# thetisproject/thetis

Hardware: AMD Instinct MI355X
Metric: DG element-updates/sec, 2D SWE DG-P1 SSPRK33 (higher is better)
Workload: dtype f64

## Files before the change

include/swe2d.h:

```cpp
#ifndef SWE2D_H
#define SWE2D_H

#include <stddef.h>
#include <stdint.h>

#ifdef __cplusplus
extern "C" {
#endif

#define SWE2D_ABI_VERSION 12
#define SWE2D_MAX_MARKERS 16

typedef enum {
    SWE2D_OK = 0,
    SWE2D_ERR_INVALID_ARGUMENT = -1,
    SWE2D_ERR_NO_DEVICE = -2,
    SWE2D_ERR_HIP = -3,
    SWE2D_ERR_UNSUPPORTED = -4,
    SWE2D_ERR_NOT_FINITE = -5
} swe2d_status;

#define SWE2D_BC_ELEV 1
#define SWE2D_BC_UV   2
#define SWE2D_BC_UN   4
#define SWE2D_BC_FLUX 8
#define SWE2D_BC_ELEV_FIELD 16
#define SWE2D_BC_UV_FIELD   32
#define SWE2D_BC_UN_FIELD   64
#define SWE2D_BC_FLUX_FIELD 128

typedef enum {
    SWE2D_FIELD_CORIOLIS = 0,
    SWE2D_FIELD_ATMOSPHERIC_PRESSURE = 1,
    SWE2D_FIELD_MOMENTUM_SOURCE = 2,
    SWE2D_FIELD_VOLUME_SOURCE = 3,
    SWE2D_FIELD_WIND_STRESS = 4,
    SWE2D_FIELD_LINEAR_DRAG = 5,
    SWE2D_FIELD_QUADRATIC_DRAG = 6,
    SWE2D_FIELD_MANNING_DRAG = 7,
    SWE2D_FIELD_NIKURADSE = 8,
    SWE2D_FIELD_COUNT = 9
} swe2d_field;

typedef enum {
    SWE2D_SCALAR_LINEAR_DRAG = 0,
    SWE2D_SCALAR_QUADRATIC_DRAG = 1,
    SWE2D_SCALAR_MANNING_DRAG = 2,
    SWE2D_SCALAR_NORM_SMOOTHER = 3,
    SWE2D_SCALAR_NIKURADSE = 4,
    SWE2D_SCALAR_COUNT = 5
} swe2d_scalar;

typedef enum {
    SWE2D_OPT_FUSED_STAGES = 0,
    SWE2D_OPT_FLOW = 1,
    SWE2D_OPT_FLOW_WD = 2,
    SWE2D_OPT_BND_INLINE = 3,
    SWE2D_OPT_LDSX = 4,
    SWE2D_OPT_ALTERNATE = 5,
    SWE2D_OPT_COMPACT_IDX = 6,
    SWE2D_OPT_VISC_FUSION = 7,
    SWE2D_OPT_WALL_FAST = 8,
    SWE2D_OPT_FLOW_POLL = 9,
    SWE2D_OPT_FLOW_CAPACITY = 10,
    SWE2D_OPT_FLOW_TIMEOUT_MS = 11,
    SWE2D_OPT_P2P_TIMEOUT_MS = 12,
    SWE2D_OPT_P2P_ZONE = 13,
    SWE2D_OPT_ROCTX = 14,
    SWE2D_OPT_COUNT = 15
} swe2d_option;

typedef struct {
    int32_t n_cells;
    int32_t n_owned;
    int32_t n_vertices;
    int32_t nodes_per_cell;
    const int32_t *cell_vertices;
    const double  *vertex_xy;
    const int32_t *cell_neighbours;
    const int8_t  *cell_neighbour_facets;
    const double  *bathymetry;
    const double  *boundary_len;
} swe2d_mesh;

typedef struct {
    double  g_grav;
    double  dt;
    int32_t use_nonlinear_equations;
    int32_t use_lax_friedrichs_velocity;
    double  lax_friedrichs_velocity_scaling_factor;
    int32_t device_id;
} swe2d_params;

typedef struct swe2d_handle swe2d_handle;

int  swe2d_abi_version(void);
int  swe2d_connectivity_info(swe2d_handle *h, int32_t out[2]);
int  swe2d_fused_pair_info(swe2d_handle *h, int32_t out[4]);
int  swe2d_fused_set_order(swe2d_handle *h, const int32_t *cells_in_tile_order);
int  swe2d_fused_triple_info(swe2d_handle *h, int32_t out[4]);
int  swe2d_fused_set_triple_tiles(swe2d_handle *h, const int32_t *cells_in_tile_order, const int32_t *tile_starts, int32_t n_starts);
int  swe2d_solve_step_cells(swe2d_handle *h, int32_t cell_end);
int  swe2d_fused_step_info(swe2d_handle *h, int32_t out[4]);
int  swe2d_device_count(void);

void swe2d_ssprk33_coefficients(double alpha0[3], double alpha_in[3], double beta[3]);

int  swe2d_create(const swe2d_mesh *mesh, const swe2d_params *params, swe2d_handle **out);
int  swe2d_set_general_quadrilaterals(swe2d_handle *h, int on);
void swe2d_destroy(swe2d_handle *h);
const char *swe2d_last_error(const swe2d_handle *h);
int  swe2d_set_option(swe2d_handle *h, int option, int value);
int  swe2d_get_option(swe2d_handle *h, int option, int *value);

int  swe2d_set_state(swe2d_handle *h, const double *uv, const double *eta);
int  swe2d_get_state(swe2d_handle *h, double *uv, double *eta);
int  swe2d_get_stage_state(swe2d_handle *h, int i_stage, double *uv, double *eta);
int  swe2d_state_snapshot(swe2d_handle *h, int restore);
#define SWE2D_SNAPSHOT_SLOTS 2
int  swe2d_state_snapshot_slot(swe2d_handle *h, int slot, int restore);

int  swe2d_set_dt(swe2d_handle *h, double dt);

int  swe2d_set_bc(swe2d_handle *h, int marker, int kind, const double values[5]);

int  swe2d_set_bc_field(swe2d_handle *h, int which, int marker, const double *nodal);
int  swe2d_set_bc_facets(swe2d_handle *h, int which, int32_t n_facets, const int32_t *cells, const int32_t *facets,
                         const double *values);

int  swe2d_set_boundary_drag(swe2d_handle *h, int marker, double drag_coefficient);

int  swe2d_set_field(swe2d_handle *h, int field, const double *nodal);
int  swe2d_set_field_vertex(swe2d_handle *h, int field, const double *vertex_values);
int  swe2d_set_scalar(swe2d_handle *h, int which, double value);

int  swe2d_set_wetting_and_drying(swe2d_handle *h, int enable, const double *alpha_vertex);

int  swe2d_advance(swe2d_handle *h, int n_steps);
int  swe2d_solve_stage(swe2d_handle *h, int i_stage);
int  swe2d_advance_forward_euler(swe2d_handle *h, int n_steps);
int  swe2d_advance_timed(swe2d_handle *h, int n_steps, int per_launch, float *ms_total, float *ms_kernel_avg);
int  swe2d_synchronize(swe2d_handle *h);

int  swe2d_tendency(swe2d_handle *h, double *k_uv, double *k_eta);

int  swe2d_diagnostics(swe2d_handle *h, double out[4]);
int  swe2d_diagnostics_limbs(swe2d_handle *h, int64_t limbs[18], double *min_depth);
double swe2d_sum_limbs_to_double(const int64_t limbs[6]);

int  swe2d_set_viscosity(swe2d_handle *h, int enable, const double *nu_vertex, double nu_const, double sipg_factor,
                         int use_grad_div_viscosity_term, int use_grad_depth_viscosity_term);

int  swe2d_tracer_add(swe2d_handle *h, int *tracer_id);
int  swe2d_tracer_set_options(swe2d_handle *h, int use_lax_friedrichs_tracer, double lax_friedrichs_tracer_scaling_factor,
                              double tracer_advective_velocity_factor);
int  swe2d_tracer_set_state(swe2d_handle *h, int tracer_id, const double *nodal);
int  swe2d_tracer_get_state(swe2d_handle *h, int tracer_id, double *nodal);
int  swe2d_tracer_set_bc(swe2d_handle *h, int tracer_id, int marker, int has_value, double value);
int  swe2d_tracer_set_bc_velocity(swe2d_handle *h, int tracer_id, int marker, int kind, double u, double v);
int  swe2d_tracer_set_bc_velocity_facets(swe2d_handle *h, int tracer_id, int marker, int kind, double elev, int32_t n_facets,
                                         const int32_t *cells, const int32_t *facets, const double *values);
int  swe2d_tracer_set_bc_field(swe2d_handle *h, int tracer_id, int marker, const double *nodal);
int  swe2d_tracer_set_bc_facets(swe2d_handle *h, int tracer_id, int32_t n_facets, const int32_t *cells, const int32_t *facets,
                                const double *values);
int  swe2d_tracer_set_source(swe2d_handle *h, int tracer_id, const double *nodal);
int  swe2d_tracer_set_conservative(swe2d_handle *h, int tracer_id, int use_conservative_form);
int  swe2d_tracer_set_diffusivity(swe2d_handle *h, int tracer_id, int enable, const double *mu_vertex, double mu_const,
                                  double sipg_factor_tracer);
#define SWE2D_DIFF_BC_NONE 0
#define SWE2D_DIFF_BC_DIFF_FLUX 1
#define SWE2D_DIFF_BC_UPWIND 2
#define SWE2D_DIFF_BC_GRAD_IN 3
#define SWE2D_DIFF_BC_VALUE_FIELD 4
int  swe2d_tracer_set_diffusion_bc(swe2d_handle *h, int tracer_id, int marker, int kind, double diff_flux);
int  swe2d_tracer_solve_stage(swe2d_handle *h, int tracer_id, int i_stage);
int  swe2d_tracer_tendency(swe2d_handle *h, int tracer_id, double *k_nodal);
int  swe2d_tracer_forward_euler(swe2d_handle *h, int tracer_id);
int  swe2d_tracer_solve_stage_cells(swe2d_handle *h, int tracer_id, int i_stage, int32_t cell_begin, int32_t cell_end);
int  swe2d_tracer_swap_buffers(swe2d_handle *h, int tracer_id);
int  swe2d_tracer_limit_cells(swe2d_handle *h, int tracer_id, int32_t cell_end);
int  swe2d_tracer_halo_pack(swe2d_handle *h, int tracer_id, int i_buffer, double *send_buf_dev);
int  swe2d_tracer_halo_unpack(swe2d_handle *h, int tracer_id, int i_buffer, const double *recv_buf_dev);
int  swe2d_limiter_setup(swe2d_handle *h, int32_t n_topo_vertices, const int32_t *cell_topo_vertices);
int  swe2d_tracer_limit(swe2d_handle *h, int tracer_id);
int  swe2d_tracer_diagnostics(swe2d_handle *h, int tracer_id, double out[4]);
int  swe2d_tracer_diagnostics_limbs(swe2d_handle *h, int tracer_id, int64_t limbs[12], double minmax[2]);
int  swe2d_advance_coupled(swe2d_handle *h, int n_steps, int tracer_only, int use_limiter);

int  swe2d_debug_calibration_copy(swe2d_handle *h, int n_times);

int  swe2d_halo_setup(swe2d_handle *h, int32_t n_send, const int32_t *send_cells, int32_t n_recv, const int32_t *recv_cells);
int  swe2d_halo_pack(swe2d_handle *h, int i_buffer, double *send_buf_dev);
int  swe2d_halo_unpack(swe2d_handle *h, int i_buffer, const double *recv_buf_dev);
#define SWE2D_IPC_HANDLE_BYTES 64
int  swe2d_p2p_create(swe2d_handle *h, int32_t n_channels, const int32_t *widths);
int  swe2d_p2p_export(swe2d_handle *h, void *ipc_handle_out, void **local_base, int32_t *zone_kind);
int  swe2d_p2p_open(swe2d_handle *h, const void *ipc_handle, void **remote_base);
int  swe2d_p2p_connect(swe2d_handle *h, int32_t n_peers, void *const *remote_base, const int32_t *send_offset,
                       const int32_t *send_count, const int32_t *remote_recv_offset, const int32_t *remote_flag_index,
                       const int32_t *remote_n_recv, int32_t n_from);
int  swe2d_p2p_push(swe2d_handle *h, int channel, int i_buffer);
int  swe2d_p2p_wait_unpack(swe2d_handle *h, int channel, int i_buffer);
int  swe2d_p2p_push_multi(swe2d_handle *h, int n, const int32_t *channels, const int32_t *i_buffers);
int  swe2d_p2p_wait_unpack_multi(swe2d_handle *h, int n, const int32_t *channels, const int32_t *i_buffers);
int  swe2d_set_exchange_stream(swe2d_handle *h, void *hip_stream);
int  swe2d_p2p_status(swe2d_handle *h, int64_t *epochs_sent, int64_t *epochs_received, int32_t *timeouts);
int  swe2d_solve_stage_cells(swe2d_handle *h, int i_stage, int32_t cell_begin, int32_t cell_end);
int  swe2d_solve_stage_pair_cells(swe2d_handle *h, int32_t cell_end_0, int32_t cell_end_1);
int  swe2d_forward_euler_cells(swe2d_handle *h, int32_t cell_begin, int32_t cell_end);
int  swe2d_swap_state_buffers(swe2d_handle *h);
int  swe2d_solve_flow(swe2d_handle *h, int32_t n_stages, const int32_t *cell_end);
int  swe2d_flow_supported(swe2d_handle *h);
int  swe2d_solve_flow_exchange(swe2d_handle *h, int32_t n_cycles, int32_t stages_per_cycle, const int32_t *cell_end);
int  swe2d_flow_prepare_exchange(swe2d_handle *h);
int  swe2d_flow_unpack_pending(swe2d_handle *h);
int  swe2d_flow_set_order(swe2d_handle *h, const int32_t *cells_in_flow_order);
int  swe2d_flow_status(swe2d_handle *h, int32_t *timeouts);
int  swe2d_debug_flow_poke(swe2d_handle *h, int32_t block, int32_t delta);
int  swe2d_debug_flow_delay(swe2d_handle *h, int32_t block, int32_t where, int32_t microseconds, int32_t every_nth_stage);
int  swe2d_debug_flow_tear(swe2d_handle *h, int32_t block, int32_t microseconds, int32_t every_nth_publish, int32_t across_ranks);
int  swe2d_set_stream(swe2d_handle *h, void *hip_stream);

// ... 38 lines not shown
```

thetis_amd/_lib.py:

```python
import ctypes
import os
import warnings

_HERE = os.path.dirname(os.path.abspath(__file__))
LIB_PATH = os.environ.get('THETIS_AMD_LIB') or os.path.join(_HERE, 'libswe2d_hip.so')

MAX_MARKERS = 16
BC_ELEV, BC_UV, BC_UN, BC_FLUX = 1, 2, 4, 8
BC_ELEV_FIELD, BC_UV_FIELD, BC_UN_FIELD, BC_FLUX_FIELD = 16, 32, 64, 128
FIELD_CORIOLIS, FIELD_ATMOSPHERIC_PRESSURE, FIELD_MOMENTUM_SOURCE, FIELD_VOLUME_SOURCE, FIELD_WIND_STRESS = 0, 1, 2, 3, 4
FIELD_LINEAR_DRAG, FIELD_QUADRATIC_DRAG, FIELD_MANNING_DRAG, FIELD_NIKURADSE = 5, 6, 7, 8
SCALAR_LINEAR_DRAG, SCALAR_QUADRATIC_DRAG, SCALAR_MANNING_DRAG, SCALAR_NORM_SMOOTHER, SCALAR_NIKURADSE = 0, 1, 2, 3, 4

IPC_HANDLE_BYTES = 64
SUM_LIMBS = 6
ABI_VERSION = 12
(OPT_FUSED_STAGES, OPT_FLOW, OPT_FLOW_WD, OPT_BND_INLINE, OPT_LDSX, OPT_ALTERNATE, OPT_COMPACT_IDX, OPT_VISC_FUSION, OPT_WALL_FAST,
 OPT_FLOW_POLL, OPT_FLOW_CAPACITY, OPT_FLOW_TIMEOUT_MS, OPT_P2P_TIMEOUT_MS, OPT_P2P_ZONE, OPT_ROCTX) = range(15)
OPT_COUNT = 15
SNAPSHOT_SLOTS = 2
MAX_FARMS, MAX_THRUST_TABLE = 8, 16
PROBE_UV, PROBE_ELEV = -1, -2
OK, ERR_INVALID_ARGUMENT, ERR_NO_DEVICE, ERR_HIP, ERR_UNSUPPORTED, ERR_NOT_FINITE = 0, -1, -2, -3, -4, -5

OPTION_ENV = {
    'THETIS_AMD_FUSE12': (OPT_FUSED_STAGES, int),
    'THETIS_AMD_FLOW': (OPT_FLOW, int),
    'THETIS_AMD_FLOW_WD': (OPT_FLOW_WD, int),
    'THETIS_AMD_BND_INLINE': (OPT_BND_INLINE, int),
    'THETIS_AMD_LDSX': (OPT_LDSX, int),
    'THETIS_AMD_ALTERNATE': (OPT_ALTERNATE, int),
    'THETIS_AMD_COMPACT_IDX': (OPT_COMPACT_IDX, int),
    'THETIS_AMD_NO_VISC_FUSION': (OPT_VISC_FUSION, lambda v: 0),
    'THETIS_AMD_WALL_FAST': (OPT_WALL_FAST, int),
    'THETIS_AMD_FLOW_POLL': (OPT_FLOW_POLL, int),
    'THETIS_AMD_FLOW_CAPACITY': (OPT_FLOW_CAPACITY, int),
    'THETIS_AMD_FLOW_TIMEOUT_S': (OPT_FLOW_TIMEOUT_MS, lambda v: max(1, int(round(1e3*float(v))))),
    'THETIS_AMD_P2P_TIMEOUT_S': (OPT_P2P_TIMEOUT_MS, lambda v: max(1, int(round(1e3*float(v))))),
    'THETIS_AMD_P2P_ZONE': (OPT_P2P_ZONE, lambda v: {'uncached': 1, 'finegrained': 2, 'device': 3}[v]),
    'THETIS_AMD_ROCTX': (OPT_ROCTX, int),
}


def options_from_environment():
    out = []
    for name, (opt, conv) in OPTION_ENV.items():
        v = os.environ.get(name)
        if v is not None and v != '':
            try:
                out.append((opt, int(conv(v))))
            except (ValueError, KeyError, TypeError) as e:
                warnings.warn('{}={!r} is not a valid value ({}: {}): the library\'s own rule applies'.format(name, v, type(e).__name__, e))
    return out


_dp = ctypes.POINTER(ctypes.c_double)
_ip = ctypes.POINTER(ctypes.c_int32)
_bp = ctypes.POINTER(ctypes.c_int8)


class Swe2dMesh(ctypes.Structure):
    _fields_ = [('n_cells', ctypes.c_int32), ('n_owned', ctypes.c_int32), ('n_vertices', ctypes.c_int32),
                ('nodes_per_cell', ctypes.c_int32), ('cell_vertices', _ip), ('vertex_xy', _dp),
                ('cell_neighbours', _ip), ('cell_neighbour_facets', _bp), ('bathymetry', _dp),
                ('boundary_len', _dp)]


class Swe2dParams(ctypes.Structure):
    _fields_ = [('g_grav', ctypes.c_double), ('dt', ctypes.c_double),
                ('use_nonlinear_equations', ctypes.c_int32), ('use_lax_friedrichs_velocity', ctypes.c_int32),
                ('lax_friedrichs_velocity_scaling_factor', ctypes.c_double), ('device_id', ctypes.c_int32)]


class TurbineParams(ctypes.Structure):
    _fields_ = [('thrust_area_const', ctypes.c_double), ('support_area', ctypes.c_double), ('rotor_area', ctypes.c_double),
                ('projected_diameter', ctypes.c_double), ('power_const', ctypes.c_double), ('rho0', ctypes.c_double),
                ('upwind_correction', ctypes.c_int32), ('n_table', ctypes.c_int32),
                ('speeds', ctypes.c_double*MAX_THRUST_TABLE), ('thrust', ctypes.c_double*MAX_THRUST_TABLE),
                ('power', ctypes.c_double*MAX_THRUST_TABLE)]


_H = ctypes.c_void_p
SYMBOLS = {
    'swe2d_abi_version': (ctypes.c_int, []),
    'swe2d_connectivity_info': (ctypes.c_int, [_H, ctypes.POINTER(ctypes.c_int32)]),
    'swe2d_fused_pair_info': (ctypes.c_int, [_H, ctypes.POINTER(ctypes.c_int32)]),
    'swe2d_fused_triple_info': (ctypes.c_int, [_H, ctypes.POINTER(ctypes.c_int32)]),
    'swe2d_fused_set_order': (ctypes.c_int, [_H, ctypes.POINTER(ctypes.c_int32)]),
    'swe2d_solve_step_cells': (ctypes.c_int, [_H, ctypes.c_int32]),
    'swe2d_fused_step_info': (ctypes.c_int, [_H, ctypes.POINTER(ctypes.c_int32)]),
    'swe2d_fused_set_triple_tiles': (ctypes.c_int, [_H, ctypes.POINTER(ctypes.c_int32), ctypes.POINTER(ctypes.c_int32), ctypes.c_int32]),
    'swe2d_solve_stage_pair_cells': (ctypes.c_int, [_H, ctypes.c_int32, ctypes.c_int32]),
    'swe2d_device_count': (ctypes.c_int, []),
    'swe2d_ssprk33_coefficients': (None, [_dp, _dp, _dp]),
    'swe2d_create': (ctypes.c_int, [ctypes.POINTER(Swe2dMesh), ctypes.POINTER(Swe2dParams), ctypes.POINTER(_H)]),
    'swe2d_destroy': (None, [_H]),
    'swe2d_last_error': (ctypes.c_char_p, [_H]),
    'swe2d_set_state': (ctypes.c_int, [_H, _dp, _dp]),
    'swe2d_get_state': (ctypes.c_int, [_H, _dp, _dp]),
    'swe2d_get_stage_state': (ctypes.c_int, [_H, ctypes.c_int, _dp, _dp]),
    'swe2d_state_snapshot': (ctypes.c_int, [_H, ctypes.c_int]),
    'swe2d_state_snapshot_slot': (ctypes.c_int, [_H, ctypes.c_int, ctypes.c_int]),
    'swe2d_set_option': (ctypes.c_int, [_H, ctypes.c_int, ctypes.c_int]),
    'swe2d_get_option': (ctypes.c_int, [_H, ctypes.c_int, ctypes.POINTER(ctypes.c_int)]),
    'swe2d_set_dt': (ctypes.c_int, [_H, ctypes.c_double]),
    'swe2d_set_bc': (ctypes.c_int, [_H, ctypes.c_int, ctypes.c_int, _dp]),
    'swe2d_set_bc_field': (ctypes.c_int, [_H, ctypes.c_int, ctypes.c_int, _dp]),
    'swe2d_set_bc_facets': (ctypes.c_int, [_H, ctypes.c_int, ctypes.c_int32, _ip, _ip, _dp]),
    'swe2d_set_boundary_drag': (ctypes.c_int, [_H, ctypes.c_int, ctypes.c_double]),
    'swe2d_set_field': (ctypes.c_int, [_H, ctypes.c_int, _dp]),
    'swe2d_set_field_vertex': (ctypes.c_int, [_H, ctypes.c_int, _dp]),
    'swe2d_set_scalar': (ctypes.c_int, [_H, ctypes.c_int, ctypes.c_double]),
    'swe2d_set_wetting_and_drying': (ctypes.c_int, [_H, ctypes.c_int, _dp]),
    'swe2d_set_viscosity': (ctypes.c_int, [_H, ctypes.c_int, _dp, ctypes.c_double, ctypes.c_double, ctypes.c_int, ctypes.c_int]),
    'swe2d_advance': (ctypes.c_int, [_H, ctypes.c_int]),
    'swe2d_solve_stage': (ctypes.c_int, [_H, ctypes.c_int]),
    'swe2d_advance_timed': (ctypes.c_int, [_H, ctypes.c_int, ctypes.c_int, ctypes.POINTER(ctypes.c_float),
                                           ctypes.POINTER(ctypes.c_float)]),
    'swe2d_synchronize': (ctypes.c_int, [_H]),
    'swe2d_tendency': (ctypes.c_int, [_H, _dp, _dp]),
    'swe2d_diagnostics': (ctypes.c_int, [_H, _dp]),
    'swe2d_diagnostics_limbs': (ctypes.c_int, [_H, ctypes.POINTER(ctypes.c_int64), _dp]),
    'swe2d_sum_limbs_to_double': (ctypes.c_double, [ctypes.POINTER(ctypes.c_int64)]),
    'swe2d_tracer_diagnostics_limbs': (ctypes.c_int, [_H, ctypes.c_int, ctypes.POINTER(ctypes.c_int64), _dp]),
    'swe2d_set_general_quadrilaterals': (ctypes.c_int, [_H, ctypes.c_int]),
    'swe2d_tracer_add': (ctypes.c_int, [_H, ctypes.POINTER(ctypes.c_int)]),
    'swe2d_tracer_set_options': (ctypes.c_int, [_H, ctypes.c_int, ctypes.c_double, ctypes.c_double]),
    'swe2d_tracer_set_state': (ctypes.c_int, [_H, ctypes.c_int, _dp]),
    'swe2d_tracer_get_state': (ctypes.c_int, [_H, ctypes.c_int, _dp]),
    'swe2d_tracer_set_bc': (ctypes.c_int, [_H, ctypes.c_int, ctypes.c_int, ctypes.c_int, ctypes.c_double]),
    'swe2d_tracer_set_bc_velocity': (ctypes.c_int, [_H, ctypes.c_int, ctypes.c_int, ctypes.c_int, ctypes.c_double, ctypes.c_double]),
    'swe2d_tracer_set_bc_velocity_facets': (ctypes.c_int, [_H, ctypes.c_int, ctypes.c_int, ctypes.c_int, ctypes.c_double, ctypes.c_int32,
                                                            _ip, _ip, _dp]),
    'swe2d_tracer_set_bc_field': (ctypes.c_int, [_H, ctypes.c_int, ctypes.c_int, _dp]),
    'swe2d_tracer_set_bc_facets': (ctypes.c_int, [_H, ctypes.c_int, ctypes.c_int32, _ip, _ip, _dp]),
    'swe2d_tracer_set_source': (ctypes.c_int, [_H, ctypes.c_int, _dp]),
    'swe2d_tracer_solve_stage_cells': (ctypes.c_int, [_H, ctypes.c_int, ctypes.c_int, ctypes.c_int32, ctypes.c_int32]),
    'swe2d_tracer_swap_buffers': (ctypes.c_int, [_H, ctypes.c_int]),
    'swe2d_tracer_limit_cells': (ctypes.c_int, [_H, ctypes.c_int, ctypes.c_int32]),
    'swe2d_tracer_halo_pack': (ctypes.c_int, [_H, ctypes.c_int, ctypes.c_int, ctypes.c_void_p]),
    'swe2d_tracer_halo_unpack': (ctypes.c_int, [_H, ctypes.c_int, ctypes.c_int, ctypes.c_void_p]),
    'swe2d_advance_forward_euler': (ctypes.c_int, [_H, ctypes.c_int]),
    'swe2d_tracer_forward_euler': (ctypes.c_int, [_H, ctypes.c_int]),
    'swe2d_tracer_set_conservative': (ctypes.c_int, [_H, ctypes.c_int, ctypes.c_int]),
    'swe2d_tracer_set_diffusivity': (ctypes.c_int, [_H, ctypes.c_int, ctypes.c_int, _dp, ctypes.c_double, ctypes.c_double]),
    'swe2d_tracer_set_diffusion_bc': (ctypes.c_int, [_H, ctypes.c_int, ctypes.c_int, ctypes.c_int, ctypes.c_double]),
    'swe2d_tracer_solve_stage': (ctypes.c_int, [_H, ctypes.c_int, ctypes.c_int]),
    'swe2d_tracer_tendency': (ctypes.c_int, [_H, ctypes.c_int, _dp]),
    'swe2d_limiter_setup': (ctypes.c_int, [_H, ctypes.c_int32, _ip]),
    'swe2d_tracer_limit': (ctypes.c_int, [_H, ctypes.c_int]),
    'swe2d_tracer_diagnostics': (ctypes.c_int, [_H, ctypes.c_int, _dp]),
    'swe2d_advance_coupled': (ctypes.c_int, [_H, ctypes.c_int, ctypes.c_int, ctypes.c_int]),
    'swe2d_debug_calibration_copy': (ctypes.c_int, [_H, ctypes.c_int]),
    'swe2d_halo_setup': (ctypes.c_int, [_H, ctypes.c_int32, _ip, ctypes.c_int32, _ip]),
    'swe2d_halo_pack': (ctypes.c_int, [_H, ctypes.c_int, ctypes.c_void_p]),
    'swe2d_halo_unpack': (ctypes.c_int, [_H, ctypes.c_int, ctypes.c_void_p]),
    'swe2d_p2p_create': (ctypes.c_int, [_H, ctypes.c_int32, _ip]),
    'swe2d_p2p_export': (ctypes.c_int, [_H, ctypes.c_void_p, ctypes.POINTER(ctypes.c_void_p), _ip]),
    'swe2d_p2p_open': (ctypes.c_int, [_H, ctypes.c_void_p, ctypes.POINTER(ctypes.c_void_p)]),
    'swe2d_p2p_connect': (ctypes.c_int, [_H, ctypes.c_int32, ctypes.POINTER(ctypes.c_void_p), _ip, _ip, _ip, _ip, _ip,
                                          ctypes.c_int32]),
    'swe2d_p2p_push': (ctypes.c_int, [_H, ctypes.c_int, ctypes.c_int]),
    'swe2d_p2p_wait_unpack': (ctypes.c_int, [_H, ctypes.c_int, ctypes.c_int]),
    'swe2d_p2p_push_multi': (ctypes.c_int, [_H, ctypes.c_int, _ip, _ip]),
    'swe2d_p2p_wait_unpack_multi': (ctypes.c_int, [_H, ctypes.c_int, _ip, _ip]),
    'swe2d_p2p_status': (ctypes.c_int, [_H, ctypes.POINTER(ctypes.c_int64), ctypes.POINTER(ctypes.c_int64), _ip]),
    'swe2d_solve_stage_cells': (ctypes.c_int, [_H, ctypes.c_int, ctypes.c_int32, ctypes.c_int32]),
    'swe2d_forward_euler_cells': (ctypes.c_int, [_H, ctypes.c_int32, ctypes.c_int32]),
    'swe2d_swap_state_buffers': (ctypes.c_int, [_H]),
    'swe2d_solve_flow': (ctypes.c_int, [_H, ctypes.c_int32, ctypes.POINTER(ctypes.c_int32)]),
    'swe2d_flow_supported': (ctypes.c_int, [_H]),
    'swe2d_flow_prepare_exchange': (ctypes.c_int, [_H]),
    'swe2d_flow_unpack_pending': (ctypes.c_int, [_H]),
    'swe2d_solve_flow_exchange': (ctypes.c_int, [_H, ctypes.c_int32, ctypes.c_int32, ctypes.POINTER(ctypes.c_int32)]),
    'swe2d_flow_set_order': (ctypes.c_int, [_H, ctypes.POINTER(ctypes.c_int32)]),
    'swe2d_flow_status': (ctypes.c_int, [_H, ctypes.POINTER(ctypes.c_int32)]),
    'swe2d_debug_flow_poke': (ctypes.c_int, [_H, ctypes.c_int32, ctypes.c_int32]),
    'swe2d_debug_flow_delay': (ctypes.c_int, [_H, ctypes.c_int32, ctypes.c_int32, ctypes.c_int32, ctypes.c_int32]),
    'swe2d_debug_flow_tear': (ctypes.c_int, [_H, ctypes.c_int32, ctypes.c_int32, ctypes.c_int32, ctypes.c_int32]),
    'swe2d_set_stream': (ctypes.c_int, [_H, ctypes.c_void_p]),
    'swe2d_set_exchange_stream': (ctypes.c_int, [_H, ctypes.c_void_p]),
    'swe2d_probe_create': (ctypes.c_int, [_H, ctypes.c_int32, _ip, _dp, ctypes.c_int32, _ip, ctypes.c_int32, _ip]),
    'swe2d_probe_width': (ctypes.c_int, [_H, ctypes.c_int32, _ip, _ip, _ip]),
    'swe2d_probe_append': (ctypes.c_int, [_H, ctypes.c_int32]),
    'swe2d_probe_read': (ctypes.c_int, [_H, ctypes.c_int32, _dp, _ip]),
    'swe2d_probe_eval': (ctypes.c_int, [_H, ctypes.c_int32, _dp]),
    'swe2d_probe_destroy': (ctypes.c_int, [_H, ctypes.c_int32]),
    'swe2d_turbine_farm_set': (ctypes.c_int, [_H, ctypes.c_int32, ctypes.POINTER(TurbineParams), _dp]),
    'swe2d_turbine_farm_clear': (ctypes.c_int, [_H, ctypes.c_int32]),
    'swe2d_turbine_power': (ctypes.c_int, [_H, _dp]),
    'swe2d_turbine_power_limbs': (ctypes.c_int, [_H, ctypes.POINTER(ctypes.c_int64)]),
    'swe2d_turbine_rows_reserve': (ctypes.c_int, [_H, ctypes.c_int32]),
    'swe2d_turbine_rows_append': (ctypes.c_int, [_H]),
# ... 46 lines not shown
```

thetis_amd/csrc/swe2d_api.hip:

```cpp
#include "swe2d_handle.h"
#include "swe2d_pick.h"

namespace swe2d_impl {

thread_local std::string g_create_error;
std::atomic<unsigned long long> g_next_uid{1ull};

extern const double kBeta[3] = {1.0, 0.25, 0.6666666666666666};
extern const double kAlpha0[3] = {1.0, 0.75, 0.33333333333333337};
extern const double kAlphaIn[3] = {0.0, 0.25, 0.6666666666666666};

int fail(Handle *h, int code, const std::string &msg)
{
    if (h) h->err = msg; else g_create_error = msg;
    return code;
}

bool stream_capturing(Handle *h, unsigned long long *id)
{
    hipStreamCaptureStatus cs = hipStreamCaptureStatusNone;
    unsigned long long cid = 0;
    const bool yes = h->stream && hipStreamGetCaptureInfo(h->stream, &cs, &cid) == hipSuccess && cs != hipStreamCaptureStatusNone;
    (void)hipGetLastError();
    if (id) *id = yes ? cid : 0;
// ... 91 lines not shown
        v.sipg = (h->npc == 4 ? 4.0 : 3.0)*h->sipg_factor;
        v.dt = h->par.dt; v.beta = beta;
        v.cell_begin = c0; v.cell_end = c1;
        v.grad_div = h->visc_grad_div; v.grad_depth = h->visc_grad_depth;
        v.nonlin = h->par.use_nonlinear_equations;
        v.wd = h->wd ? 1 : 0;
        v.valpha = h->valpha;
        v.eta = h->state[in] + (size_t)2*h->npc*h->stride;
        v.bc = h->bc;
        v.bc_elev_f = h->bc_field[0]; v.bc_uv_f = h->bc_field[1]; v.bc_un_f = h->bc_field[2]; v.bc_flux_f = h->bc_field[3];
        if (fused_visc) {
            bool any = false;
            for (int m = 0; m < SWE_MAX_MARKERS; m++) any = any || (h->bc.kind[m] & (SWE_BC_UN | SWE_BC_UV | SWE_BC_FLUX)) != 0;
            v.cell_list = h->bnd_cells; v.n_list = h->n_bnd;
            if (any && h->n_bnd > 0)
                hipLaunchKernelGGL((swe_sipg_kernel<2, true>), dim3((h->n_bnd + SWE_BLOCK - 1)/SWE_BLOCK), dim3(SWE_BLOCK), 0,
                                   h->stream, v);
        } else if (h->npc == 4 && !h->affine) hipLaunchKernelGGL((swe_sipg_kernel_quad<2, false>), dim3(grid), dim3(SWE_BLOCK), 0, h->stream, v);
        else if (h->npc == 4) hipLaunchKernelGGL(swe_sipg_kernel_quad<2>, dim3(grid), dim3(SWE_BLOCK), 0, h->stream, v);
        else hipLaunchKernelGGL(swe_sipg_kernel<2>, dim3(grid), dim3(SWE_BLOCK), 0, h->stream, v);
        HIP_TRY(h, hipGetLastError());
        if (h->wd && !(a0 == 0.0 && a1 == 0.0)) {
            if (h->npc == 4)
                hipLaunchKernelGGL(swe_wd_relax_kernel<4>, dim3((c1 - c0 + 255)/256), dim3(256), 0, h->stream, h->state[out], h->stride,
                                   h->cv, h->vh, h->valpha, h->par.g_grav, beta*h->par.dt, c0, c1);
            else
                hipLaunchKernelGGL(swe_wd_relax_kernel<3>, dim3((c1 - c0 + 255)/256), dim3(256), 0, h->stream, h->state[out], h->stride,
                                   h->cv, h->vh, h->valpha, h->par.g_grav, beta*h->par.dt, c0, c1);
            HIP_TRY(h, hipGetLastError());
        }
    }
    return SWE2D_OK;
}

int stage_on_range(Handle *h, int i_stage, int c0, int c1)
{
    switch (i_stage) {
    case 0: return launch_stage(h, 0, 0, 1, 0.0, 1.0, kBeta[0], c0, c1);
    case 1: return launch_stage(h, 1, 0, 2, kAlpha0[1], kAlphaIn[1], kBeta[1], c0, c1);
    case 2: return launch_stage(h, 2, 0, 0, kAlpha0[2], kAlphaIn[2], kBeta[2], c0, c1);
    default: return fail(h, SWE2D_ERR_INVALID_ARGUMENT, "i_stage must be 0, 1 or 2");
    }
}

int scatter_facet_values(Handle *h, double *planes, int n, const int32_t *cells, const int32_t *facets,
                                const double *values, int ncomp, int nval)
{
    if (n == 0) return SWE2D_OK;
    const size_t nv = (size_t)n*nval*ncomp;
    if (nv*sizeof(double) > (size_t)2*h->npc*h->n_cells*sizeof(double))
        return fail(h, SWE2D_ERR_INVALID_ARGUMENT, "more boundary facets than the staging buffer holds");
    int slot = -1;
    for (int i = 0; i < 8 && slot < 0; i++) {
        const Handle::FacetList &c = h->facet_lists[i];
        if ((int)c.cells.size() == n && std::memcmp(c.cells.data(), cells, (size_t)n*sizeof(int32_t)) == 0
            && std::memcmp(c.facets.data(), facets, (size_t)n*sizeof(int32_t)) == 0)
            slot = i;
    }
    const bool same = slot >= 0;
    if (!same) slot = (h->facet_list_next++) & 7;
    Handle::FacetList &fl = h->facet_lists[slot];
    if (!same) {
        for (int t = 0; t < n; t++)
            if (cells[t] < 0 || cells[t] >= h->n_cells || facets[t] < 0 || facets[t] >= h->npc)
                return fail(h, SWE2D_ERR_INVALID_ARGUMENT, "boundary facet list: cell or facet index out of range");
        HIP_TRY(h, hipStreamSynchronize(h->stream));
        if (fl.dev) { HIP_TRY(h, hipFree(fl.dev)); fl.dev = nullptr; }
        HIP_TRY(h, hipMalloc(&fl.dev, 2*(size_t)n*sizeof(int)));
        HIP_TRY(h, hipMemcpy(fl.dev, cells, (size_t)n*sizeof(int), hipMemcpyHostToDevice));
        HIP_TRY(h, hipMemcpy(fl.dev + n, facets, (size_t)n*sizeof(int), hipMemcpyHostToDevice));
        fl.cells.assign(cells, cells + n);
        fl.facets.assign(facets, facets + n);
    }
    double *dv = h->stage_uv;
    const int *dc = fl.dev, *df = fl.dev + n;
    HIP_TRY(h, hipMemcpyAsync(dv, values, nv*sizeof(double), hipMemcpyHostToDevice, h->stream));
    hipLaunchKernelGGL(swe_bc_facet_scatter, dim3(grid_for(n)), dim3(256), 0, h->stream, dv, planes, h->stride, dc, df, n, ncomp,
                       h->npc, nval);
    HIP_TRY(h, hipGetLastError());
    HIP_TRY(h, hipStreamSynchronize(h->stream));
    return SWE2D_OK;
}

int upload_vertex_coefficient(Handle *h, const double *vertex_values, double **dev)
{
    HIP_TRY(h, hipSetDevice(h->device));
    if (!vertex_values) {
        if (*dev) { HIP_TRY(h, hipStreamSynchronize(h->stream)); HIP_TRY(h, hipFree(*dev)); *dev = nullptr; }
        return SWE2D_OK;
    }
    for (int i = 0; i < h->n_vertices; i++)
        if (!(vertex_values[i] >= 0.0)) return fail(h, SWE2D_ERR_INVALID_ARGUMENT, "diffusion coefficient must be >= 0");
    if (!*dev) HIP_TRY(h, hipMalloc(dev, (size_t)h->n_vertices*sizeof(double)));
    HIP_TRY(h, hipMemcpyAsync(*dev, vertex_values, (size_t)h->n_vertices*sizeof(double), hipMemcpyHostToDevice, h->stream));
    HIP_TRY(h, hipStreamSynchronize(h->stream));
    return SWE2D_OK;
}

}

extern "C" {

int swe2d_abi_version(void) { return SWE2D_ABI_VERSION; }

static bool advance_takes_flow(Handle *h);
int swe2d_fused_pair_info(swe2d_handle *hh, int32_t out[4])
{
    Handle *h = H(hh);
    if (!h || !out) return fail(h, SWE2D_ERR_INVALID_ARGUMENT, "null argument");
    out[0] = out[1] = out[2] = 0; out[3] = h->n_cells;
    if (!fuse12_covers(h) || (h->n_owned == h->n_cells && advance_takes_flow(h))) return SWE2D_OK;
    HIP_TRY(h, hipSetDevice(h->device));
    if (int rc = fuse12_build(h)) return rc;
    if (h->npc == 4) { if (h->fuseq_tile) { out[0] = 1; out[1] = h->fuseq_n_tiles; out[2] = (int32_t)h->fuseq_ring_cells; } }
    else if (h->fuse_tile) { out[0] = 1; out[1] = h->fuse_n_tiles; out[2] = (int32_t)h->fuse_ring_cells; }
    return SWE2D_OK;
}

int swe2d_connectivity_info(swe2d_handle *hh, int32_t out[2])
{
    Handle *h = H(hh);
    if (!h || !out) return fail(h, SWE2D_ERR_INVALID_ARGUMENT, "null argument");
    const bool on = h->idxc && h->opt[SWE2D_OPT_COMPACT_IDX] != 0;
    out[0] = on ? 1 : 0;
    out[1] = on ? h->n_conn_escapes : 0;
    return SWE2D_OK;
}

int swe2d_device_count(void)
{
    int n = 0;
    if (hipGetDeviceCount(&n) != hipSuccess) return SWE2D_ERR_NO_DEVICE;
    return n;
}

void swe2d_ssprk33_coefficients(double alpha0[3], double alpha_in[3], double beta[3])
{
    const double a0[3] = {0.0, kAlpha0[1], kAlpha0[2]};
    const double ai[3] = {kAlpha0[0], kAlphaIn[1], kAlphaIn[2]};
    for (int i = 0; i < 3; i++) { alpha0[i] = a0[i]; alpha_in[i] = ai[i]; beta[i] = kBeta[i]; }
}

const char *swe2d_last_error(const swe2d_handle *h)
{
    return h ? H(h)->err.c_str() : g_create_error.c_str();
}

int swe2d_set_option(swe2d_handle *hh, int option, int value)
{
    Handle *h = H(hh);
    if (!h) return SWE2D_ERR_INVALID_ARGUMENT;
    if (option < 0 || option >= SWE2D_OPT_COUNT) return fail(h, SWE2D_ERR_INVALID_ARGUMENT, "swe2d_set_option: unknown option");
    if (value < -1) return fail(h, SWE2D_ERR_INVALID_ARGUMENT, "swe2d_set_option: value must be >= -1 (-1: the library's own rule)");
    h->opt[option] = value;
    if (option == SWE2D_OPT_FUSED_STAGES && h->fuse_state == -1) h->fuse_state = 0;
    if (option == SWE2D_OPT_FLOW_CAPACITY) h->flow_capacity = -1;
    return SWE2D_OK;
}

int swe2d_get_option(swe2d_handle *hh, int option, int *value)
{
    Handle *h = H(hh);
    if (!h || !value) return fail(h, SWE2D_ERR_INVALID_ARGUMENT, "null argument");
    if (option < 0 || option >= SWE2D_OPT_COUNT) return fail(h, SWE2D_ERR_INVALID_ARGUMENT, "swe2d_get_option: unknown option");
    *value = h->opt[option];
    return SWE2D_OK;
}

int swe2d_create(const swe2d_mesh *mesh, const swe2d_params *params, swe2d_handle **out)
{
    if (!mesh || !params || !out) return fail(nullptr, SWE2D_ERR_INVALID_ARGUMENT, "null argument");
    *out = nullptr;
    if (mesh->nodes_per_cell != 3 && mesh->nodes_per_cell != 4)
        return fail(nullptr, SWE2D_ERR_UNSUPPORTED, "nodes_per_cell must be 3 (triangles) or 4 (quadrilaterals)");
    if (mesh->n_cells <= 0 || mesh->n_owned <= 0 || mesh->n_owned > mesh->n_cells || mesh->n_vertices <= 0)
        return fail(nullptr, SWE2D_ERR_INVALID_ARGUMENT, "bad mesh sizes");
    if (mesh->n_cells >= (1 << 29))
        return fail(nullptr, SWE2D_ERR_UNSUPPORTED, "more than 2^29 cells per device");
    if (!mesh->cell_vertices || !mesh->vertex_xy || !mesh->cell_neighbours || !mesh->cell_neighbour_facets
        || !mesh->bathymetry)
        return fail(nullptr, SWE2D_ERR_INVALID_ARGUMENT, "null mesh array");
    if (!(params->dt > 0.0) || !(params->g_grav > 0.0))
        return fail(nullptr, SWE2D_ERR_INVALID_ARGUMENT, "dt and g_grav must be positive");
    if ((((size_t)mesh->n_cells + 255)/256*256)*(size_t)mesh->nodes_per_cell*sizeof(double) >= ((size_t)1 << 32)
        || (size_t)mesh->n_vertices*sizeof(double) >= ((size_t)1 << 32))
        return fail(nullptr, SWE2D_ERR_UNSUPPORTED,
                    "mesh too large for one device: nodes_per_cell*n_cells*8 bytes must stay below 4 GiB (partition it)");
    int ndev = 0;
    if (hipGetDeviceCount(&ndev) != hipSuccess || ndev <= 0)
        return fail(nullptr, SWE2D_ERR_NO_DEVICE, "no HIP device visible (this library has no CPU fallback)");
    if (params->device_id < 0 || params->device_id >= ndev)
        return fail(nullptr, SWE2D_ERR_INVALID_ARGUMENT, "device_id out of range");

    Handle *h = new (std::nothrow) Handle();
    if (!h) return fail(nullptr, SWE2D_ERR_INVALID_ARGUMENT, "out of host memory");
    h->device = params->device_id;
    h->par = *params;
    const int n = mesh->n_cells, nv = mesh->n_vertices;
    const int npc = mesh->nodes_per_cell;
    h->npc = npc;
    h->n_cells = n; h->n_owned = mesh->n_owned; h->n_interior = mesh->n_owned; h->n_vertices = nv;
    h->stride = ((size_t)n + 255)/256*256;

#define HIP_TRY_C(expr)                                                                                  \
    do {                                                                                                 \
        hipError_t e_ = (expr);                                                                          \
        if (e_ != hipSuccess) {                                                                          \
            (void)hipGetLastError();                                                                     \
            int rc_ = fail(nullptr, SWE2D_ERR_HIP, std::string(#expr) + ": " + hipGetErrorString(e_));   \
            swe2d_destroy(reinterpret_cast<swe2d_handle *>(h));                                          \
            return rc_;                                                                                  \
        }                                                                                                \
    } while (0)

    HIP_TRY_C(hipSetDevice(h->device));
    HIP_TRY_C(hipStreamCreateWithFlags(&h->my_stream, hipStreamNonBlocking));
    h->stream = h->my_stream; h->own_stream = true;
    HIP_TRY_C(hipEventCreate(&h->ev0));
    HIP_TRY_C(hipEventCreate(&h->ev1));
    const size_t S = h->stride;
    for (int b = 0; b < 3; b++) {
        HIP_TRY_C(hipMalloc(&h->state[b], 3*(size_t)npc*S*sizeof(double)));
        HIP_TRY_C(hipMemsetAsync(h->state[b], 0, 3*(size_t)npc*S*sizeof(double), h->stream));
    }
    HIP_TRY_C(hipMalloc(&h->nbr, (size_t)npc*S*sizeof(int)));
    HIP_TRY_C(hipMalloc(&h->cv, (size_t)npc*S*sizeof(int)));
    HIP_TRY_C(hipMalloc(&h->vx, (size_t)nv*sizeof(double)));
    HIP_TRY_C(hipMalloc(&h->vy, (size_t)nv*sizeof(double)));
    HIP_TRY_C(hipMalloc(&h->vh, (size_t)nv*sizeof(double)));
    HIP_TRY_C(hipMalloc(&h->stage_uv, 2*(size_t)npc*n*sizeof(double)));
    HIP_TRY_C(hipMalloc(&h->stage_eta, (size_t)npc*n*sizeof(double)));
    h->n_partial_blocks = (h->n_owned + SWE_BLOCK - 1)/SWE_BLOCK;
    HIP_TRY_C(hipMalloc(&h->partial, 4*(size_t)h->n_partial_blocks*sizeof(double)));
    HIP_TRY_C(hipMalloc(&h->diag_acc, SWE_DIAG_BUCKETS*SWE_DIAG_ACC*sizeof(unsigned long long)));

    std::vector<int> nbr((size_t)npc*S, 0), cv((size_t)npc*S, 0);
    std::vector<double> vx(nv), vy(nv), vh(nv);
    double blen[SWE2D_MAX_MARKERS];
    for (int m = 0; m < SWE2D_MAX_MARKERS; m++) blen[m] = 0.0;
    for (int i = 0; i < nv; i++) {
        vx[i] = mesh->vertex_xy[2*(size_t)i];
        vy[i] = mesh->vertex_xy[2*(size_t)i + 1];
        vh[i] = mesh->bathymetry[i];
    }
    h->host_cells.assign(mesh->cell_vertices, mesh->cell_vertices + (size_t)npc*n);
    h->host_nbr.assign(mesh->cell_neighbours, mesh->cell_neighbours + (size_t)npc*n);
    for (int k = 0; k < n; k++) {
        for (int f = 0; f < npc; f++) {
            const int vid = mesh->cell_vertices[(size_t)npc*k + f];
            if (vid < 0 || vid >= nv) {
                swe2d_destroy(reinterpret_cast<swe2d_handle *>(h));
                return fail(nullptr, SWE2D_ERR_INVALID_ARGUMENT, "cell_vertices entry out of range");
            }
            cv[(size_t)f*S + k] = vid;
            const int nb = mesh->cell_neighbours[(size_t)npc*k + f];
            int packed;
            if (nb >= 0) {
                const int f2 = mesh->cell_neighbour_facets[(size_t)npc*k + f];
                if (nb >= n || f2 < 0 || f2 >= npc) {
                    swe2d_destroy(reinterpret_cast<swe2d_handle *>(h));
                    return fail(nullptr, SWE2D_ERR_INVALID_ARGUMENT, "cell_neighbours entry out of range");
                }
                packed = (nb << 2) | f2;
            } else {
                const int marker = -nb;
                if (marker >= SWE2D_MAX_MARKERS && k < mesh->n_owned) {
                    swe2d_destroy(reinterpret_cast<swe2d_handle *>(h));
                    return fail(nullptr, SWE2D_ERR_UNSUPPORTED, "boundary marker >= SWE2D_MAX_MARKERS");
                }
                packed = -marker;
                if (k < mesh->n_owned && marker < SWE2D_MAX_MARKERS) {
                    const int va = mesh->cell_vertices[(size_t)npc*k + f], vb = mesh->cell_vertices[(size_t)npc*k + (f + 1) % npc];
                    blen[marker] += std::hypot(vx[vb] - vx[va], vy[vb] - vy[va]);
                }
            }
            nbr[(size_t)f*S + k] = packed;
        }
        const int a = mesh->cell_vertices[(size_t)npc*k], b = mesh->cell_vertices[(size_t)npc*k + 1],
                  c = mesh->cell_vertices[(size_t)npc*k + npc - 1];
        const double area2 = (vx[b] - vx[a])*(vy[c] - vy[a]) - (vx[c] - vx[a])*(vy[b] - vy[a]);
        if (!(area2 > 0.0)) {
            swe2d_destroy(reinterpret_cast<swe2d_handle *>(h));
            return fail(nullptr, SWE2D_ERR_INVALID_ARGUMENT, "cells must be counter-clockwise with positive area");
        }
        if (npc == 4) {
            const int d = mesh->cell_vertices[4*(size_t)k + 2];
            const double sx = vx[a] - vx[b] + vx[d] - vx[c], sy = vy[a] - vy[b] + vy[d] - vy[c];
            if (std::max(std::fabs(sx), std::fabs(sy)) > 1e-9*std::sqrt(area2)) {
                h->affine = false;
                h->affine_local = false;
                const double ax = vx[b] - vx[a], ay = vy[b] - vy[a], bx = vx[c] - vx[a], by = vy[c] - vy[a];
                const double d1 = ax*sy - ay*sx, d2 = sx*by - sy*bx;
                if (!(area2 + d1 > 0.0 && area2 + d2 > 0.0 && area2 + d1 + d2 > 0.0)) {
                    swe2d_destroy(reinterpret_cast<swe2d_handle *>(h));
                    return fail(nullptr, SWE2D_ERR_INVALID_ARGUMENT, "quadrilateral cells must be convex");
                }
            }
        }
    }
    if (mesh->n_owned != mesh->n_cells && !mesh->boundary_len) {
        swe2d_destroy(reinterpret_cast<swe2d_handle *>(h));
        return fail(nullptr, SWE2D_ERR_INVALID_ARGUMENT, "boundary_len is required for a partitioned mesh");
    }
    std::memset(&h->bc, 0, sizeof(h->bc));
    for (int m = 0; m < SWE2D_MAX_MARKERS; m++) h->bc.drag[m] = -1.0;
    for (int m = 0; m < SWE2D_MAX_MARKERS; m++) h->bc.len[m] = mesh->boundary_len ? mesh->boundary_len[m] : blen[m];
// ... 694 lines not shown
```

thetis_amd/csrc/swe2d_api_fuse.hip:

```cpp
#include "swe2d_handle.h"
#include "swe2d_fuse.h"

namespace swe2d_impl {

namespace {
typedef void (*fuse_kernel_t)(const SweFuseArgs);
template <bool SRC>
fuse_kernel_t pick_fuse_src(bool nl, bool lf)
{
    if (nl) return lf ? swe_fuse12_kernel<true, true, SRC> : swe_fuse12_kernel<true, false, SRC>;
    return lf ? swe_fuse12_kernel<false, true, SRC> : swe_fuse12_kernel<false, false, SRC>;
}
fuse_kernel_t pick_fuse_kernel(bool nl, bool lf, bool src) { return src ? pick_fuse_src<true>(nl, lf) : pick_fuse_src<false>(nl, lf); }
}

static bool fuse_applies(const Handle *h)
{
    if (h->opt[SWE2D_OPT_FUSED_STAGES] == 0) return false;
    if (h->opt[SWE2D_OPT_BND_INLINE] == 0) return false;
    if (h->n_farms > 0) return false;
    return !h->wd && !h->visc && !h->h_nbr.empty();
}

bool fuse12_covers(const Handle *h)
// ... 83 lines not shown
        h->fuse_state = -1; h->fuse_n_tiles = 0;
        return SWE2D_OK;
    }
    HIP_TRY(h, hipMalloc(&h->fuse_tile, tl.size()*sizeof(int2)));
    HIP_TRY(h, hipMalloc(&h->fuse_inner, inner.size()*sizeof(int)));
    HIP_TRY(h, hipMemcpy(h->fuse_tile, tl.data(), tl.size()*sizeof(int2), hipMemcpyHostToDevice));
    HIP_TRY(h, hipMemcpy(h->fuse_inner, inner.data(), inner.size()*sizeof(int), hipMemcpyHostToDevice));
    h->fuse_ring_cells = n_ring_total;
    return SWE2D_OK;
}

int launch_fuse12_quad(Handle *h, int cell_end);
int launch_fuse12(Handle *h, int cell_end)
{
    if (h->npc == 4) return launch_fuse12_quad(h, cell_end);
    if (int rc = fuse12_build(h)) return rc;
    if (!h->fuse_tile) return fail(h, SWE2D_ERR_UNSUPPORTED, "fused stage pair: no tile tables");
    SweFuseArgs q;
    fill_stage_args(h, q.st, 0, 0, 2, 0.0, 1.0, kBeta[0], 0, h->n_owned);
    q.st.idxc = h->opt[SWE2D_OPT_COMPACT_IDX] == 0 ? nullptr : h->idxc;
    q.tile = h->fuse_tile;
    q.n_inner = h->fuse_inner;
    q.n_tiles = h->fuse_n_tiles;
    q.cell_end = cell_end;
    q.beta1 = kBeta[0];
    q.a0_2 = kAlpha0[1]; q.a1_2 = kAlphaIn[1]; q.beta2 = kBeta[1];
    q.out = h->state[2];
    fuse_kernel_t kern = pick_fuse_kernel(h->par.use_nonlinear_equations != 0, h->par.use_lax_friedrichs_velocity != 0, has_sources(h));
    const int grid = ((h->fuse_n_tiles + 7)/8)*8;
    SWE_CHK_SYNC(h->stream);
    hipLaunchKernelGGL(kern, dim3(grid), dim3(SWE_FUSE_WG), 0, h->stream, q);
    HIP_TRY(h, hipGetLastError());
    stage_written(h, false, true);
    return SWE2D_OK;
}

int fuseq_build(Handle *h)
{
    if (h->fuseq_tile || h->fuse_state == -1) return SWE2D_OK;
    {
        hipStreamCaptureStatus cs = hipStreamCaptureStatusNone;
        if (hipStreamIsCapturing(h->stream, &cs) == hipSuccess && cs != hipStreamCaptureStatusNone) return SWE2D_OK;
        (void)hipGetLastError();
    }
    const int n = h->n_cells;
    const size_t S = h->stride;
    const int *nbr = h->h_nbr.data();
    const int *order = (int)h->fuse_order.size() == n ? h->fuse_order.data() : nullptr;
    std::vector<int4> tl;
    std::vector<int> inner, ring, cells;
    std::vector<int> state((size_t)n, 0), lane_of((size_t)n, -1);
    long long n_ring_total = 0;
    for (int pos = 0; pos < n;) {
        cells.clear(); ring.clear();
        int n_ring = 0;
        while (pos < n && (int)cells.size() < SWE_QFUSE_INNER) {
            const int kk = order ? order[pos] : pos;
            int delta = state[kk] == 2 ? -1 : 0;
            for (int f = 0; f < 4; f++) {
                const int code = nbr[(size_t)f*S + kk];
                if (code >= 0 && state[code >> 2] == 0) {
                    bool dup = false;
                    for (int g = 0; g < f; g++) dup = dup || (nbr[(size_t)g*S + kk] >= 0 && (nbr[(size_t)g*S + kk] >> 2) == (code >> 2));
                    if (!dup) delta++;
                }
            }
            if (!cells.empty() && n_ring + delta > SWE_QFUSE_RING) break;
            if (n_ring + delta > SWE_QFUSE_RING) return fail(h, SWE2D_ERR_UNSUPPORTED, "fused stage pair: a cell with more neighbours than a ring holds");
            if (state[kk] == 2) n_ring--;
            state[kk] = 1;
            cells.push_back(kk);
            for (int f = 0; f < 4; f++) {
                const int code = nbr[(size_t)f*S + kk];
                if (code >= 0 && state[code >> 2] == 0) { state[code >> 2] = 2; ring.push_back(code >> 2); n_ring++; }
            }
            pos++;
        }
        const int ni = (int)cells.size();
        for (int c : ring) if (state[c] == 2) cells.push_back(c);
        const int nt = (int)cells.size();
        if (nt - ni != n_ring || nt > SWE_FUSE_WG) return fail(h, SWE2D_ERR_UNSUPPORTED, "fused stage pair: tile bookkeeping");
        for (int l = 0; l < nt; l++) lane_of[cells[l]] = l;
        const size_t base = tl.size();
        tl.resize(base + SWE_FUSE_WG, int4{-1, 0, 0, 0});
        int n_out = 0;
        for (int l = 0; l < nt; l++) {
            const int c = cells[l];
            unsigned w[4];
            for (int f = 0; f < 4; f++) {
                const int code = nbr[(size_t)f*S + c];
                if (code < 0) w[f] = (unsigned)l;
                else if (state[code >> 2] != 0) w[f] = (unsigned)lane_of[code >> 2];
                else {
                    if (l < ni || n_out >= SWE_QFUSE_MAX_OUT) return fail(h, SWE2D_ERR_UNSUPPORTED, "fused stage pair: ring bookkeeping");
                    w[f] = 0x200u | (unsigned)n_out++;
                }
            }
            tl[base + l] = int4{c, (int)(w[0] | (w[1] << SWE_FUSE_FBITS) | (w[2] << (2*SWE_FUSE_FBITS))), (int)w[3], 0};
        }
        inner.push_back(ni);
        n_ring_total += nt - ni;
        for (int c : cells) { state[c] = 0; lane_of[c] = -1; }
    }
    h->fuseq_n_tiles = (int)inner.size();
    const bool forced = h->opt[SWE2D_OPT_FUSED_STAGES] == 1 || h->opt[SWE2D_OPT_FUSED_STAGES] == 3;
    if (!forced && (double)n/h->fuseq_n_tiles < 176.0) { h->fuse_state = -1; h->fuseq_n_tiles = 0; return SWE2D_OK; }
    HIP_TRY(h, hipMalloc(&h->fuseq_tile, tl.size()*sizeof(int4)));
    HIP_TRY(h, hipMalloc(&h->fuseq_inner, inner.size()*sizeof(int)));
    HIP_TRY(h, hipMemcpy(h->fuseq_tile, tl.data(), tl.size()*sizeof(int4), hipMemcpyHostToDevice));
    HIP_TRY(h, hipMemcpy(h->fuseq_inner, inner.data(), inner.size()*sizeof(int), hipMemcpyHostToDevice));
    h->fuseq_ring_cells = n_ring_total;
    return SWE2D_OK;
}

namespace {
typedef void (*fuseq_kernel_t)(const SweFuseQuadArgs);
template <bool SRC, bool AFFINE>
fuseq_kernel_t pick_fuseq_2(bool nl, bool lf)
{
    if (nl) return lf ? swe_fuse12_quad_kernel<true, true, SRC, AFFINE> : swe_fuse12_quad_kernel<true, false, SRC, AFFINE>;
    return lf ? swe_fuse12_quad_kernel<false, true, SRC, AFFINE> : swe_fuse12_quad_kernel<false, false, SRC, AFFINE>;
}
fuseq_kernel_t pick_fuseq_kernel(bool nl, bool lf, bool src, bool affine)
{
    if (affine) return src ? pick_fuseq_2<true, true>(nl, lf) : pick_fuseq_2<false, true>(nl, lf);
    return src ? pick_fuseq_2<true, false>(nl, lf) : pick_fuseq_2<false, false>(nl, lf);
}
}

int launch_fuse12_quad(Handle *h, int cell_end)
{
    if (int rc = fuseq_build(h)) return rc;
    if (!h->fuseq_tile) return fail(h, SWE2D_ERR_UNSUPPORTED, "fused stage pair: no tile tables");
    SweFuseQuadArgs q;
    fill_stage_args(h, q.st, 0, 0, 2, 0.0, 1.0, kBeta[0], 0, h->n_owned);
    q.tile = h->fuseq_tile;
    q.n_inner = h->fuseq_inner;
    q.n_tiles = h->fuseq_n_tiles;
    q.cell_end = cell_end;
    q.beta1 = kBeta[0];
    q.a0_2 = kAlpha0[1]; q.a1_2 = kAlphaIn[1]; q.beta2 = kBeta[1];
    q.out = h->state[2];
    fuseq_kernel_t kern = pick_fuseq_kernel(h->par.use_nonlinear_equations != 0, h->par.use_lax_friedrichs_velocity != 0, has_sources(h), h->affine);
    const int grid = ((h->fuseq_n_tiles + 7)/8)*8;
    SWE_CHK_SYNC(h->stream);
    hipLaunchKernelGGL(kern, dim3(grid), dim3(SWE_FUSE_WG), 0, h->stream, q);
    HIP_TRY(h, hipGetLastError());
    stage_written(h, false, true);
    return SWE2D_OK;
}

namespace {
typedef void (*fuse3_kernel_t)(const SweFuse3Args);
template <bool SRC>
fuse3_kernel_t pick_fuse3_src(bool nl, bool lf)
{
    if (nl) return lf ? swe_fuse123_kernel<true, true, SRC> : swe_fuse123_kernel<true, false, SRC>;
    return lf ? swe_fuse123_kernel<false, true, SRC> : swe_fuse123_kernel<false, false, SRC>;
}
fuse3_kernel_t pick_fuse3_kernel(bool nl, bool lf, bool src) { return src ? pick_fuse3_src<true>(nl, lf) : pick_fuse3_src<false>(nl, lf); }
}

int fuse123_build(Handle *h)
{
    if (h->fuse3_tile || stream_capturing(h)) return SWE2D_OK;
    const int n = h->n_cells;
    const size_t S = h->stride;
    const int *nbr = h->h_nbr.data();
    const int *order = (int)h->fuse3_order.size() == n ? h->fuse3_order.data() : ((int)h->fuse_order.size() == n ? h->fuse_order.data() : nullptr);
    const unsigned char *start = (int)h->fuse3_start.size() == n ? h->fuse3_start.data() : nullptr;
    std::vector<int2> tl, cnt;
    std::vector<unsigned char> state((size_t)n, 0);
    std::vector<int> lane_of((size_t)n, -1), touched, inner;
    std::vector<std::pair<int, unsigned char>> undo;
    int count[4] = {0, 0, 0, 0};
    long long r1_total = 0, r2_total = 0;
    auto set = [&](int c, unsigned char ns) {
        undo.push_back({c, state[c]});
        if (state[c] == 0) touched.push_back(c);
        count[state[c]]--; state[c] = ns; count[ns]++;
    };
    for (int pos = 0; pos < n;) {
        inner.clear(); touched.clear();
        count[1] = count[2] = count[3] = 0;
        while (pos < n) {
            if (start && start[pos] && !inner.empty()) break;
            const int kk = order ? order[pos] : pos;
            undo.clear();
            const size_t touched_before = touched.size();
            set(kk, 1);
            for (int f = 0; f < 3; f++) {
                const int code = nbr[(size_t)f*S + kk];
                if (code < 0) continue;
                const int c1 = code >> 2;
                if (state[c1] == 0 || state[c1] == 3) {
                    set(c1, 2);
                    for (int g = 0; g < 3; g++) {
                        const int code2 = nbr[(size_t)g*S + c1];
                        if (code2 >= 0 && state[code2 >> 2] == 0) set(code2 >> 2, 3);
                    }
                }
            }
            if (count[1] + count[2] + count[3] > SWE_FUSE_WG || 2*count[3] > SWE_FUSE3_MAX_OUT) {
                if (inner.empty()) return fail(h, SWE2D_ERR_UNSUPPORTED, "fused stages: a cell whose two rings do not fit a tile");
                for (size_t i = undo.size(); i-- > 0;) { count[state[undo[i].first]]--; state[undo[i].first] = undo[i].second; count[undo[i].second]++; }
                touched.resize(touched_before);
                break;
            }
            inner.push_back(kk);
            pos++;
        }
        std::vector<int> cells(inner);
        for (int want = 2; want <= 3; want++)
            for (int c : touched) if (state[c] == want) cells.push_back(c);
        const int ni = (int)inner.size(), nm = ni + count[2], nt = (int)cells.size();
        if (nt != count[1] + count[2] + count[3] || ni != count[1] || nt > SWE_FUSE_WG) return fail(h, SWE2D_ERR_UNSUPPORTED, "fused stages: tile bookkeeping");
        for (int l = 0; l < nt; l++) lane_of[cells[l]] = l;
        const size_t base = tl.size();
        tl.resize(base + SWE_FUSE_WG, int2{-1, 0});
        int n_out = 0;
        for (int l = 0; l < nt; l++) {
            const int c = cells[l];
            unsigned w = 0u;
            for (int f = 0; f < 3; f++) {
                const int code = nbr[(size_t)f*S + c];
                unsigned field;
                if (code < 0) field = (unsigned)l;
                else if (state[code >> 2] != 0) field = (unsigned)lane_of[code >> 2];
                else {
                    if (l < nm || n_out >= SWE_FUSE3_MAX_OUT) return fail(h, SWE2D_ERR_UNSUPPORTED, "fused stages: ring bookkeeping");
                    field = 0x200u | (unsigned)n_out++;
                }
                w |= field << (SWE_FUSE_FBITS*f);
            }
            tl[base + l] = int2{c, (int)w};
        }
        cnt.push_back(int2{ni, nm});
        r1_total += count[2]; r2_total += count[3];
        for (int c : cells) { state[c] = 0; lane_of[c] = -1; }
    }
    h->fuse3_n_tiles = (int)cnt.size();
    HIP_TRY(h, hipMalloc(&h->fuse3_tile, tl.size()*sizeof(int2)));
    HIP_TRY(h, hipMalloc(&h->fuse3_cnt, cnt.size()*sizeof(int2)));
    HIP_TRY(h, hipMemcpy(h->fuse3_tile, tl.data(), tl.size()*sizeof(int2), hipMemcpyHostToDevice));
    HIP_TRY(h, hipMemcpy(h->fuse3_cnt, cnt.data(), cnt.size()*sizeof(int2), hipMemcpyHostToDevice));
    h->fuse3_ring1 = r1_total; h->fuse3_ring2 = r2_total;
    return SWE2D_OK;
}

int launch_fuse123(Handle *h, int cell_end)
{
    if (int rc = capture_parity_check(h)) return rc;
    if (int rc = fuse123_build(h)) return rc;
    if (!h->fuse3_tile) return fail(h, SWE2D_ERR_UNSUPPORTED, "fused stages: no tile tables (not built inside a stream capture)");
    SweFuse3Args q;
    fill_stage_args(h, q.st, 0, 0, 1, 0.0, 1.0, kBeta[0], 0, h->n_owned);
    q.st.idxc = h->opt[SWE2D_OPT_COMPACT_IDX] == 0 ? nullptr : h->idxc;
    q.tile = h->fuse3_tile;
    q.counts = h->fuse3_cnt;
    q.n_tiles = h->fuse3_n_tiles;
    q.cell_end = cell_end;
    for (int s = 0; s < 3; s++) { q.a0[s] = s ? kAlpha0[s] : 0.0; q.a1[s] = s ? kAlphaIn[s] : 1.0; q.beta[s] = kBeta[s]; }
    q.out = h->state[1];
    fuse3_kernel_t kern = pick_fuse3_kernel(h->par.use_nonlinear_equations != 0, h->par.use_lax_friedrichs_velocity != 0, has_sources(h));
    const int grid = ((h->fuse3_n_tiles + 7)/8)*8;
    SWE_CHK_SYNC(h->stream);
    hipLaunchKernelGGL(kern, dim3(grid), dim3(SWE_FUSE_WG), 0, h->stream, q);
    HIP_TRY(h, hipGetLastError());
    std::swap(h->state[0], h->state[1]);
    h->stage_valid[0] = h->stage_valid[1] = false;
    unsigned long long id = 0;
    if (stream_capturing(h, &id)) {
        if (id != h->capture_id) { h->capture_id = id; h->capture_swaps = 0; }
        h->capture_swaps++;
    }
    return SWE2D_OK;
}

int capture_parity_check(Handle *h)
{
    if (h->capture_swaps == 0 && h->capture_odd == 0) return SWE2D_OK;
    unsigned long long id = 0;
    const bool capturing = stream_capturing(h, &id);
    if (h->capture_swaps) {
        if (capturing && id == h->capture_id) return SWE2D_OK;
        if (h->capture_swaps & 1) { std::swap(h->state[0], h->state[1]); h->capture_odd++; }
        h->capture_swaps = 0;
    }
    if (capturing || h->capture_odd == 0) return SWE2D_OK;
    const int odd = h->capture_odd;
    h->capture_odd = 0;
    return fail(h, SWE2D_ERR_UNSUPPORTED, std::to_string(odd) + " stream capture(s) recorded an odd number of swe2d_solve_step_cells launches: "
                "such a graph ends on the other state buffer than it began on and cannot be replayed (the state is the one from before the "
                "capture); capture an even number per sequence");
}

bool fuse123_wanted(const Handle *h)
{
    const int mode = h->opt[SWE2D_OPT_FUSED_STAGES];
    const bool patches = (int)h->fuse3_start.size() == h->n_cells;
    const int from = patches ? 131073 : 2500000;
    if (h->npc != 3 || !fuse_applies(h) || h->idx4 == nullptr || h->n_owned != h->n_cells) return false;
    return mode == 3 ? h->n_cells >= 64 : (mode == -1 && h->n_cells >= from && !has_sources(h));
}

int step_swe(Handle *h)
{
    if (fuse123_wanted(h)) {
        if (!stream_capturing(h)) return launch_fuse123(h, h->n_owned);
    }
    if (fuse12_covers(h)) { if (int rc = fuse12_build(h)) return rc; }
    if (fuse12_covers(h) && (h->npc == 4 ? h->fuseq_tile != nullptr : h->fuse_tile != nullptr)) {
        if (int rc = launch_fuse12(h, h->n_owned)) return rc;
        return stage_on_range(h, 2, 0, h->n_owned);
    }
    for (int s = 0; s < 3; s++)
        if (int rc = stage_on_range(h, s, 0, h->n_owned)) return rc;
    return SWE2D_OK;
}

}

extern "C" {

int swe2d_fused_set_order(swe2d_handle *hh, const int32_t *cells_in_tile_order)
{
    Handle *h = H(hh);
    if (!h) return SWE2D_ERR_INVALID_ARGUMENT;
    HIP_TRY(h, hipSetDevice(h->device));
    std::vector<int> order;
    if (cells_in_tile_order) {
        std::vector<char> seen((size_t)h->n_cells, 0);
        for (int i = 0; i < h->n_cells; i++) {
            const int c = cells_in_tile_order[i];
            if (c < 0 || c >= h->n_cells || seen[c]) return fail(h, SWE2D_ERR_INVALID_ARGUMENT, "fused stages: the tile order is not a permutation of the cells");
            seen[c] = 1;
        }
        order.assign(cells_in_tile_order, cells_in_tile_order + h->n_cells);
    }
    HIP_TRY(h, hipStreamSynchronize(h->stream));
    if (h->fuse_tile) { (void)hipFree(h->fuse_tile); h->fuse_tile = nullptr; }
    if (h->fuse_inner) { (void)hipFree(h->fuse_inner); h->fuse_inner = nullptr; }
    if (h->fuseq_tile) { (void)hipFree(h->fuseq_tile); h->fuseq_tile = nullptr; }
    if (h->fuseq_inner) { (void)hipFree(h->fuseq_inner); h->fuseq_inner = nullptr; }
    h->fuseq_n_tiles = 0;
    if (h->fuse3_tile) { (void)hipFree(h->fuse3_tile); h->fuse3_tile = nullptr; }
    if (h->fuse3_cnt) { (void)hipFree(h->fuse3_cnt); h->fuse3_cnt = nullptr; }
    h->fuse3_n_tiles = 0;
    h->fuse_n_tiles = 0; h->fuse_ring_cells = 0;
    if (h->fuse_state == -1) h->fuse_state = 0;
    h->fuse_order.swap(order);
    return SWE2D_OK;
}

int swe2d_fused_set_triple_tiles(swe2d_handle *hh, const int32_t *cells_in_tile_order, const int32_t *tile_starts, int32_t n_starts)
{
    Handle *h = H(hh);
    if (!h) return SWE2D_ERR_INVALID_ARGUMENT;
    HIP_TRY(h, hipSetDevice(h->device));
    std::vector<int> order;
    std::vector<unsigned char> start;
    if (cells_in_tile_order) {
        std::vector<char> seen((size_t)h->n_cells, 0);
        for (int i = 0; i < h->n_cells; i++) {
            const int c = cells_in_tile_order[i];
            if (c < 0 || c >= h->n_cells || seen[c]) return fail(h, SWE2D_ERR_INVALID_ARGUMENT, "fused stages: the tile order is not a permutation of the cells");
            seen[c] = 1;
        }
        order.assign(cells_in_tile_order, cells_in_tile_order + h->n_cells);
    }
    if (n_starts < 0 || (n_starts > 0 && !tile_starts)) return fail(h, SWE2D_ERR_INVALID_ARGUMENT, "fused stages: tile starts");
    if (n_starts > 0) {
        start.assign((size_t)h->n_cells, 0);
        for (int i = 0; i < n_starts; i++) {
            if (tile_starts[i] < 0 || tile_starts[i] >= h->n_cells) return fail(h, SWE2D_ERR_INVALID_ARGUMENT, "fused stages: a tile start outside the cells");
            start[tile_starts[i]] = 1;
        }
    }
    HIP_TRY(h, hipStreamSynchronize(h->stream));
    if (h->fuse3_tile) { (void)hipFree(h->fuse3_tile); h->fuse3_tile = nullptr; }
    if (h->fuse3_cnt) { (void)hipFree(h->fuse3_cnt); h->fuse3_cnt = nullptr; }
    h->fuse3_n_tiles = 0;
    h->fuse3_order.swap(order);
    h->fuse3_start.swap(start);
    return SWE2D_OK;
}

int swe2d_fused_triple_info(swe2d_handle *hh, int32_t out[4])
{
    Handle *h = H(hh);
    if (!h || !out) return fail(h, SWE2D_ERR_INVALID_ARGUMENT, "null argument");
    out[0] = out[1] = out[2] = out[3] = 0;
    if (!fuse123_wanted(h)) return SWE2D_OK;
    HIP_TRY(h, hipSetDevice(h->device));
    if (int rc = fuse123_build(h)) return rc;
    if (!h->fuse3_tile) return SWE2D_OK;
    out[0] = 1; out[1] = h->fuse3_n_tiles; out[2] = (int32_t)h->fuse3_ring1; out[3] = (int32_t)h->fuse3_ring2;
    return SWE2D_OK;
}

static bool fuse123_partition_ok(const Handle *h)
{
    const int mode = h->opt[SWE2D_OPT_FUSED_STAGES];
    if (h->npc != 3 || !fuse_applies(h) || h->idx4 == nullptr || mode == 2 || mode == 1) return false;
    return mode == 3 || !has_sources(h);
}

int swe2d_fused_step_info(swe2d_handle *hh, int32_t out[4])
{
    Handle *h = H(hh);
    if (!h || !out) return fail(h, SWE2D_ERR_INVALID_ARGUMENT, "null argument");
    out[0] = out[1] = out[2] = out[3] = 0;
    const int mode = h->opt[SWE2D_OPT_FUSED_STAGES];
    if (!fuse123_partition_ok(h)) return SWE2D_OK;
    if (mode != 3 && ((int)h->fuse3_start.size() != h->n_cells || h->n_cells <= 131072)) return SWE2D_OK;
    HIP_TRY(h, hipSetDevice(h->device));
    if (int rc = fuse123_build(h)) return rc;
    if (!h->fuse3_tile) return SWE2D_OK;
    out[0] = 1; out[1] = h->fuse3_n_tiles; out[2] = (int32_t)h->fuse3_ring1; out[3] = (int32_t)h->fuse3_ring2;
    return SWE2D_OK;
// ... 31 lines not shown
```

thetis_amd/csrc/swe2d_flow.h:

```cpp
#pragma once
#include "swe2d_kernels.h"
#include "swe2d_p2p.h"

#ifndef SWE_FLOW_OCCUPANCY
#define SWE_FLOW_OCCUPANCY __attribute__((amdgpu_waves_per_eu(2, 2)))
#endif
#define SWE_FLOW_MAX_STAGES 384
#define SWE_FLOW_MAX_CYCLES 64
#ifndef SWE_FLOW_FLAG_STRIDE
#define SWE_FLOW_FLAG_STRIDE 16
#endif
#define SWE_FLOW_SLOT_BYTES 128
#define SWE_FLOW_DIV6(t_) ((int)(((unsigned)(t_)*43691u) >> 18))
#ifndef SWE_FLOW_POLL_SLEEP
#define SWE_FLOW_POLL_SLEEP 2
#endif
#ifndef SWE_FLOW_NTR_SRC
#define SWE_FLOW_NTR_SRC 3
#endif
#ifndef SWE_FLOW_WALLFAST_SRC
#define SWE_FLOW_WALLFAST_SRC true
#endif
#ifndef SWE_FLOW_RX
#define SWE_FLOW_RX 3
// ... 2 lines not shown

typedef unsigned int swe_u32x4 __attribute__((ext_vector_type(4)));
#define SWE_FLOW_NOWHERE 0x80000000u
#define SWE_FLOW_XG (9*SWE_BLOCK)
#define SWE_FLOW_LDS_DOUBLES (SWE_FLOW_XG + 6*SWE_FLOW_MAX_RIM)
#ifdef SWE_RANGE_CHECK
__device__ __forceinline__ unsigned swe_lds_index_chk(unsigned i, unsigned n, int line)
{
    if (i < n) return i;
    if (atomicAdd(&swe_chk_report[0], 1ull) == 0ull) { swe_chk_report[1] = 0x1d5000000000ull | i; swe_chk_report[2] = (unsigned long long)line; }
    return 0u;
}
#define SWE_LDSI(i, n) swe_lds_index_chk((unsigned)(i), (unsigned)(n), __LINE__)
#else
#define SWE_LDSI(i, n) (i)
#endif

#ifdef SWE_FLOW_DELAY
__device__ int swe_flow_delay[4] = {-1, 0, 0, 1};
#define SWE_FLOW_DELAY_AT(w) do {                                                                                            \
        if (swe_flow_delay[0] == lb && (swe_flow_delay[1] & (w)) && (swe_flow_delay[3] <= 1 || (s % swe_flow_delay[3]) == 0)) {    \
            const unsigned long long t0_ = wall_clock64();                                                                   \
            while (wall_clock64() - t0_ < (unsigned long long)swe_flow_delay[2]) __builtin_amdgcn_s_sleep(64);                \
        }                                                                                                                    \
    } while (0)
#else
#define SWE_FLOW_DELAY_AT(w) do { } while (0)
#endif

struct SweFlowArgs {
    SweStageArgs st;
    double *buf[3];
    unsigned *flag;
    unsigned *status;
    const int *fcell;
    const int4 *xo4;
    const int2 *xo2;
    const int2 *xblk;
    const int *xsrc;
    void *ex;
    unsigned parity_bytes;
    int n_blocks;
    int n_stages;
    int cell_end[SWE_FLOW_MAX_STAGES];
    double a0[3], a1[3], beta[3];
    unsigned long long timeout_ticks;
    int n_cycles, stages_per_cycle;
    const int2 *xsend;
    const int *xrecv;
    unsigned *xtick;
    SweP2pCounters *xctr;
    int x_n_peers;
    int x_off[SWE_P2P_MAX_PEERS];
    void *x_rdata[SWE_P2P_MAX_PEERS];
    unsigned x_rbytes[SWE_P2P_MAX_PEERS];
    unsigned x_rslot[SWE_P2P_MAX_PEERS];
    void *x_zone;
    unsigned x_zbytes, x_slot;
    unsigned long long x_timeout;
};

__device__ __forceinline__ unsigned swe_flow_check_word(unsigned lo, unsigned hi, unsigned tag) { return tag ^ lo ^ hi; }
#ifdef SWE_FLOW_TEAR
__device__ int swe_flow_tear[4] = {-1, 0, 1, 0};
__device__ __forceinline__ void swe_flow_put_torn(__amdgpu_buffer_rsrc_t r, unsigned off, swe_u32x4 g, int aux_sys, int ticks)
{
    const swe_u32x2 hi2 = {g.z, g.w}, lo2 = {g.x, g.y};
    if (aux_sys) __builtin_amdgcn_raw_buffer_store_b64(hi2, r, off + 8u, 0, 17); else __builtin_amdgcn_raw_buffer_store_b64(hi2, r, off + 8u, 0, 16);
    asm volatile("s_waitcnt vmcnt(0)" ::: "memory");
    const unsigned long long t0 = wall_clock64();
    while (wall_clock64() - t0 < (unsigned long long)ticks) __builtin_amdgcn_s_sleep(16);
    if (aux_sys) __builtin_amdgcn_raw_buffer_store_b64(lo2, r, off, 0, 17); else __builtin_amdgcn_raw_buffer_store_b64(lo2, r, off, 0, 16);
}
#define SWE_FLOW_TORN(lb_, pc_, sys_) ((swe_flow_tear[0] == (lb_) || swe_flow_tear[0] == -2) && swe_flow_tear[1] > 0 \
                                       && ((pc_) % (swe_flow_tear[2] < 1 ? 1 : swe_flow_tear[2])) == 0 && (!(sys_) || swe_flow_tear[3]))
#endif
__device__ __forceinline__ void swe_flow_put(__amdgpu_buffer_rsrc_t r, unsigned off, double x, unsigned tag, bool torn = false)
{
    const swe_u32x2 xb = __builtin_bit_cast(swe_u32x2, x);
    const swe_u32x4 g = {xb.x, xb.y, tag, swe_flow_check_word(xb.x, xb.y, tag)};
#ifdef SWE_FLOW_TEAR
    if (torn) { swe_flow_put_torn(r, off, g, 0, swe_flow_tear[1]); return; }
#endif
    (void)torn;
    __builtin_amdgcn_raw_buffer_store_b128(g, r, off, 0, 16);
}
__device__ __forceinline__ swe_u32x4 swe_flow_get(__amdgpu_buffer_rsrc_t r, unsigned off)
{
    return __builtin_amdgcn_raw_buffer_load_b128(r, off, 0, 16);
}
__device__ __forceinline__ void swe_flow_put_sys(__amdgpu_buffer_rsrc_t r, unsigned off, double x, unsigned tag, bool torn = false)
{
    const swe_u32x2 xb = __builtin_bit_cast(swe_u32x2, x);
    const swe_u32x4 g = {xb.x, xb.y, tag, swe_flow_check_word(xb.x, xb.y, tag)};
#ifdef SWE_FLOW_TEAR
    if (torn) { swe_flow_put_torn(r, off, g, 1, swe_flow_tear[1]); return; }
#endif
    (void)torn;
    __builtin_amdgcn_raw_buffer_store_b128(g, r, off, 0, 17);
}
__device__ __forceinline__ swe_u32x4 swe_flow_get_sys(__amdgpu_buffer_rsrc_t r, unsigned off)
{
    return __builtin_amdgcn_raw_buffer_load_b128(r, off, 0, 17);
}
__device__ __forceinline__ double swe_flow_val(swe_u32x4 g)
{
    const swe_u32x2 xb = {g.x, g.y};
    return __builtin_bit_cast(double, xb);
}
__device__ __forceinline__ bool swe_flow_arrived(swe_u32x4 g, unsigned need)
{
#ifdef SWE_FLOW_NOCHECK
    return (int)(g.z - need) >= 0;
#else
    return (int)(g.z - need) >= 0 && g.w == swe_flow_check_word(g.x, g.y, g.z);
#endif
}

template <bool NONLIN, bool WD = false>
__device__ __forceinline__ void swe_flow_rhs_cell(const SweStageArgs &p, const double u[3], const double v[3], const double e[3],
                                                  const double h[3], const double nx[3], const double ny[3], double bu[3], double bv[3],
                                                  double be[3], const double *Dn = nullptr)
{
#pragma clang fp contract(off)
    const double g = p.g;
    double H[3], gxs[3], gys[3];
#pragma unroll
    for (int i = 0; i < 3; i++) {
        H[i] = WD ? Dn[i] : (NONLIN ? h[i] + e[i] : h[i]);
        gxs[i] = -0.5*nx[(i + 1) % 3];
        gys[i] = -0.5*ny[(i + 1) % 3];
    }
    const double ge3 = g*(e[0] + e[1] + e[2])*(1.0/3.0);
    const double SHu = swe_int2(H, u)*(1.0/12.0), SHv = swe_int2(H, v)*(1.0/12.0);
#pragma unroll
    for (int i = 0; i < 3; i++) {
        bu[i] = gxs[i]*ge3;
        bv[i] = gys[i]*ge3;
        be[i] = swe_dot2(gxs[i], SHu, gys[i], SHv);
    }
    if (NONLIN) {
        const double Suu = swe_int2(u, u)*(1.0/12.0), Suv = swe_int2(u, v)*(1.0/12.0), Svv = swe_int2(v, v)*(1.0/12.0);
        const double D12 = fma(gys[2], v[2], fma(gys[1], v[1], fma(gys[0], v[0],
                           fma(gxs[2], u[2], fma(gxs[1], u[1], gxs[0]*u[0])))))*(1.0/12.0);
        const double us = u[0] + u[1] + u[2], vs = v[0] + v[1] + v[2];
#pragma unroll
        for (int i = 0; i < 3; i++) {
            bu[i] = fma(gys[i], Suv, fma(gxs[i], Suu, fma(D12, us + u[i], bu[i])));
            bv[i] = fma(gys[i], Svv, fma(gxs[i], Suv, fma(D12, vs + v[i], bv[i])));
        }
    }
}

template <bool NONLIN, bool LF, bool SRC, int NTR, bool WD = false, int XG = SWE_FLOW_XG, int PLANE = SWE_BLOCK, int NLDS = SWE_FLOW_LDS_DOUBLES>
__device__ __forceinline__ void swe_flow_rhs_facets(const SweStageArgs &p, int k, const double u[3], const double v[3], const double e[3],
                                                    const double h[3], const double *lds, const unsigned tr[3][NTR], int bmarkers,
                                                    const double nx[3], const double ny[3], double twoA, double bu[3], double bv[3],
                                                    double be[3], const double *Dn = nullptr, const double *al = nullptr)
{
#pragma clang fp contract(off)
    const double g = p.g;
#pragma unroll
    for (int f = 0; f < 3; f++) {
        const int a = f, b = (f + 1) % 3;
        const bool bnd = ((bmarkers >> (8*f)) & 0xff) != 0;
        const unsigned ab0 = tr[f][0] & 0xffffu, aa0 = tr[f][0] >> 16;
        const unsigned step = ab0 >= (unsigned)XG ? 1u : (unsigned)(3*PLANE);
        const unsigned ab1 = NTR == 3 ? tr[f][NTR - 2] & 0xffffu : ab0 + step, aa1 = NTR == 3 ? tr[f][NTR - 2] >> 16 : aa0 + step;
        const unsigned ab2 = NTR == 3 ? tr[f][NTR - 1] & 0xffffu : ab0 + 2u*step, aa2 = NTR == 3 ? tr[f][NTR - 1] >> 16 : aa0 + 2u*step;
        const double unb = lds[SWE_LDSI(ab0, NLDS)], una = lds[SWE_LDSI(aa0, NLDS)];
        const double vnb = lds[SWE_LDSI(ab1, NLDS)], vna = lds[SWE_LDSI(aa1, NLDS)];
        const double enb = lds[SWE_LDSI(ab2, NLDS)], ena = lds[SWE_LDSI(aa2, NLDS)];
        const double nxs = nx[f], nys = ny[f];
        double Lf, rLf;
        swe_sqrt_rsqrt(swe_dot2(nxs, nxs, nys, nys), Lf, rLf);
        double Fau, Fbu, Fav, Fbv, Fae, Fbe;
        if constexpr (WD) {
            const double ena_ = swe_wd_eta(ena, h[a], al[a]), enb_ = swe_wd_eta(enb, h[b], al[b]);
            swe_facet_flux<NONLIN, LF, true>(g, p.sigma_lf, u[a], u[b], v[a], v[b], e[a], e[b], h[a], h[b], Dn[a], Dn[b], una, unb, vna, vnb,
                                             ena_, enb_, ena, enb, nxs, nys, Lf, rLf, Fau, Fbu, Fav, Fbv, Fae, Fbe);
        } else
        swe_facet_flux<NONLIN, LF, false>(g, p.sigma_lf, u[a], u[b], v[a], v[b], e[a], e[b], h[a], h[b], 0.0, 0.0, una, unb, vna, vnb, ena, enb,
                                          0.0, 0.0, nxs, nys, Lf, rLf, Fau, Fbu, Fav, Fbv, Fae, Fbe);
        if (bnd) { Fau = 0.0; Fbu = 0.0; Fav = 0.0; Fbv = 0.0; Fae = 0.0; Fbe = 0.0; }
        bu[a] = fma(-0.5, Fau, bu[a]); bu[b] = fma(-0.5, Fbu, bu[b]);
        bv[a] = fma(-0.5, Fav, bv[a]); bv[b] = fma(-0.5, Fbv, bv[b]);
        be[a] = fma(-0.5, Fae, be[a]); be[b] = fma(-0.5, Fbe, be[b]);
    }
    if (SRC) {
        double H[3], gxs[3], gys[3];
#pragma unroll
        for (int i = 0; i < 3; i++) {
            H[i] = WD ? Dn[i] : (NONLIN ? h[i] + e[i] : h[i]);
            gxs[i] = -0.5*nx[(i + 1) % 3];
            gys[i] = -0.5*ny[(i + 1) % 3];
        }
        swe_source_terms(p, k, p.stride, twoA, u, v, H, gxs, gys, bu, bv, be);
    }
}

template <bool NONLIN, bool LF, bool WALLFAST, bool WD = false>
__device__ __forceinline__ void swe_flow_finish(const SweStageArgs &p, int k, double beta, const double u[3], const double v[3],
                                                const double e[3], const double h[3], const double nx[3], const double ny[3],
                                                double twoA, int bmarkers, int bkind1, const double bu[3], const double bv[3], const double be[3],
                                                const double wu[3], const double wv[3], const double we[3], double ou[3],
                                                double ov[3], double oe[3], const double *Dn = nullptr, const double *al = nullptr)
{
#pragma clang fp contract(off)
    const double s = 6.0*p.dt*beta*swe_rcp(twoA);
    const double su = bu[0] + bu[1] + bu[2], sv = bv[0] + bv[1] + bv[2], se = be[0] + be[1] + be[2];
#pragma unroll
    for (int i = 0; i < 3; i++) {
        ou[i] = fma(s, fma(4.0, bu[i], -su), wu[i]);
        ov[i] = fma(s, fma(4.0, bv[i], -sv), wv[i]);
        oe[i] = fma(s, fma(4.0, be[i], -se), we[i]);
    }
    if (bmarkers != 0) {
        const double sfac = 6.0*p.dt*beta*swe_rcp(fma(-ny[0], -nx[2], -(nx[0]*ny[2])));
        int rem = ((bmarkers & 0xff) ? 1 : 0) | ((bmarkers & 0xff00) ? 2 : 0) | ((bmarkers & 0xff0000) ? 4 : 0);
        int kind_next = bkind1;
        const double u_0 = u[0], u_1 = u[1], u_2 = u[2], v_0 = v[0], v_1 = v[1], v_2 = v[2], e_0 = e[0], e_1 = e[1], e_2 = e[2];
        const double h_0 = h[0], h_1 = h[1], h_2 = h[2], nx_0 = nx[0], nx_1 = nx[1], nx_2 = nx[2], ny_0 = ny[0], ny_1 = ny[1], ny_2 = ny[2];
        const double D_0 = WD ? Dn[0] : 0.0, D_1 = WD ? Dn[1] : 0.0, D_2 = WD ? Dn[2] : 0.0;
        const double al_0 = WD ? al[0] : 0.0, al_1 = WD ? al[1] : 0.0, al_2 = WD ? al[2] : 0.0;
#define SWE_SEL3(x, i) ((i) == 0 ? x##_0 : ((i) == 1 ? x##_1 : x##_2))
#pragma unroll 1
        while (rem) {
            const int f = (rem & 1) ? 0 : ((rem & 2) ? 1 : 2);
            rem &= rem - 1;
            const int a = f, b = (f == 2) ? 0 : f + 1;
            const double nxs = SWE_SEL3(nx, f), nys = SWE_SEL3(ny, f);
            double Lf, rLf;
            swe_sqrt_rsqrt(swe_dot2(nxs, nxs, nys, nys), Lf, rLf);
            double Fau = 0.0, Fbu = 0.0, Fav = 0.0, Fbv = 0.0, Fae = 0.0, Fbe = 0.0;
            const double Ha_ = WD ? SWE_SEL3(D, a) : (!NONLIN ? SWE_SEL3(h, a) : SWE_SEL3(h, a) + SWE_SEL3(e, a));
            const double Hb_ = WD ? SWE_SEL3(D, b) : (!NONLIN ? SWE_SEL3(h, b) : SWE_SEL3(h, b) + SWE_SEL3(e, b));
            swe_boundary_facet<NONLIN, LF, WD, WALLFAST>(p, (bmarkers >> (8*f)) & 0xff, k, a, b, SWE_SEL3(u, a), SWE_SEL3(u, b), SWE_SEL3(v, a),
                                                  SWE_SEL3(v, b), SWE_SEL3(e, a), SWE_SEL3(e, b), SWE_SEL3(h, a), SWE_SEL3(h, b),
                                                  Ha_, Hb_, WD ? SWE_SEL3(al, a) : 0.0, WD ? SWE_SEL3(al, b) : 0.0, nxs, nys, Lf, rLf, Fau, Fbu, Fav,
                                                  Fbv, Fae, Fbe, kind_next);
            kind_next = -1;
            const double dau = -0.5*Fau, dbu = -0.5*Fbu, dav = -0.5*Fav, dbv = -0.5*Fbv, dae = -0.5*Fae, dbe = -0.5*Fbe;
#pragma unroll
            for (int i = 0; i < 3; i++) {
                const double wa = (i == a) ? 3.0 : -1.0, wb = (i == b) ? 3.0 : -1.0;
                ou[i] = fma(sfac, fma(wa, dau, wb*dbu), ou[i]);
                ov[i] = fma(sfac, fma(wa, dav, wb*dbv), ov[i]);
                oe[i] = fma(sfac, fma(wa, dae, wb*dbe), oe[i]);
            }
        }
#undef SWE_SEL3
    }
    if constexpr (WD) swe_wd_finish<3>(p.g, beta*p.dt, h, al, ou, ov, oe, !p.wd_skip_relax);
}

#ifdef SWE_WAVE_TIMING
#ifndef SWE_FLOW_TS_STAGE
#define SWE_FLOW_TS_STAGE 7
#endif
#define SWE_FT(i) do { if (s == SWE_FLOW_TS_STAGE && lane == 0 && lb < SWE_WT_MAX) swe_wave_ts[i][lb] = wall_clock64(); } while (0)
#else
#define SWE_FT(i)
#endif


template <bool NONLIN, bool LF, bool SRC, bool FX, int POLL = 6, bool WD = false>
__global__ __launch_bounds__(SWE_BLOCK) SWE_FLOW_OCCUPANCY void swe_flow_kernel(const SweFlowArgs q)
{
#pragma clang fp contract(off)
    __shared__ double lds[SWE_FLOW_LDS_DOUBLES];
    __shared__ int xsrc[SWE_FLOW_MAX_RIM];
    __shared__ int lact[SWE_BLOCK];
    __shared__ unsigned lrec[SWE_BLOCK];
    __shared__ int lpeer[SWE_BLOCK];
    __shared__ unsigned char lpub[SWE_FLOW_MAX_RIM];
    __shared__ double lu0[9][SWE_BLOCK];
    const SweStageArgs &p = q.st;
    const int lb = swe_logical_block(blockIdx.x, gridDim.x);
    if (lb >= q.n_blocks) return;
    const int lane = (int)threadIdx.x;
    const int kcode = q.fcell[lb*SWE_BLOCK + lane];
    const bool real = kcode >= 0;
    const int k = real ? kcode : -1 - kcode;
    const size_t S = p.stride;
    const unsigned S8 = (unsigned)S*8u;
    unsigned *const myflag = q.flag + (size_t)lb*SWE_FLOW_FLAG_STRIDE;
    const unsigned base = *myflag;
    const unsigned fin = base + (unsigned)q.n_stages;
    if (!FX && !__any(real && k < q.cell_end[0])) {
        if (lane == 0) *myflag = fin;
        return;
    }
    const unsigned k8 = (unsigned)k*8u;
    const __amdgpu_buffer_rsrc_t rex = __builtin_amdgcn_make_buffer_rsrc(q.ex, 0, 3*q.parity_bytes, 0x00020000);
    const int2 myslots = q.xblk[lb];
    const int nrim = myslots.y;
    for (int i = lane; i < nrim; i += SWE_BLOCK) xsrc[SWE_LDSI(i, SWE_FLOW_MAX_RIM)] = q.xsrc[myslots.x + i];

    int bmarkers, bkind1 = 0;
    constexpr int NTR = WD ? 1 : SWE_FLOW_NTR_SRC;
    unsigned tr[3][NTR];
    int xown[3];
    double h[3], nx[3], ny[3], al[3] = {0.0, 0.0, 0.0};
    double u[3], v[3], e[3];
    {
        const int4 q4 = p.idx4[k];
        const int2 q2 = p.idx2[k];
        const int4 x4 = q.xo4[lb*SWE_BLOCK + lane];
        const int2 x2 = q.xo2[lb*SWE_BLOCK + lane];
        const int nb[3] = {q4.x, q4.y, q4.z};
        const int vid[3] = {q4.w, q2.x, q2.y};
        const int xin[3] = {x4.w, x2.x, x2.y};
        xown[0] = x4.x; xown[1] = x4.y; xown[2] = x4.z;
        bmarkers = (nb[0] < 0 ? -nb[0] : 0) | (nb[1] < 0 ? (-nb[1]) << 8 : 0) | (nb[2] < 0 ? (-nb[2]) << 16 : 0);
        if (bmarkers != 0) {
            const int m1 = (bmarkers & 0xff) ? (bmarkers & 0xff) : ((bmarkers & 0xff00) ? ((bmarkers >> 8) & 0xff) : (bmarkers >> 16));
            bkind1 = m1 < SWE_MAX_MARKERS ? p.bc.kind[m1] : 0;
        }
        const swe_rsrc_t gu = swe_rsrc(q.buf[0]), gv = swe_rsrc(q.buf[0] + 3*S), ge = swe_rsrc(q.buf[0] + 6*S);
#pragma unroll
        for (int i = 0; i < 3; i++) {
            u[i] = swe_ld(gu, k8, i*S8);
            v[i] = swe_ld(gv, k8, i*S8);
            e[i] = swe_ld(ge, k8, i*S8);
        }
        double r0[3][6];
#pragma unroll
        for (int f = 0; f < 3; f++) {
            const int nbf = nb[f];
            const bool rim = xown[f] >= 0;
            const bool inw = nbf >= 0 && !rim;
            const int ls = rim ? lane : xin[f];
            const int f2 = inw ? (nbf & 3) : f, f2a = f2 == 2 ? 0 : f2 + 1;
#pragma unroll
            for (int c = 0; c < NTR; c++) {
                const unsigned ab = rim ? (unsigned)(SWE_FLOW_XG + 6*xin[f] + c) : (unsigned)((3*c + f2)*SWE_BLOCK + ls);
                const unsigned aa = rim ? (unsigned)(SWE_FLOW_XG + 6*xin[f] + 3 + c) : (unsigned)((3*c + f2a)*SWE_BLOCK + ls);
                tr[f][c] = ab | (aa << 16);
            }
            if (!FX) {
                const int code = rim ? nbf : ((k << 2) | f);
                const unsigned kn8 = (unsigned)(code >> 2)*8u;
                const int g2 = code & 3;
                const unsigned ob = kn8 + (g2 == 0 ? 0u : (g2 == 1 ? S8 : 2u*S8));
                const unsigned oa = kn8 + (g2 == 0 ? S8 : (g2 == 1 ? 2u*S8 : 0u));
                r0[f][0] = swe_ld(gu, ob, 0); r0[f][1] = swe_ld(gv, ob, 0); r0[f][2] = swe_ld(ge, ob, 0);
                r0[f][3] = swe_ld(gu, oa, 0); r0[f][4] = swe_ld(gv, oa, 0); r0[f][5] = swe_ld(ge, oa, 0);
            }
        }
        double px[3], py[3];
        const swe_rsrc_t rvx = swe_rsrc(p.vx), rvy = swe_rsrc(p.vy), rvh = swe_rsrc(p.vh);
#pragma unroll
        for (int i = 0; i < 3; i++) {
            const unsigned v8 = (unsigned)vid[i]*8u;
            px[i] = swe_ld(rvx, v8, 0);
            py[i] = swe_ld(rvy, v8, 0);
            h[i] = swe_ld(rvh, v8, 0);
            if (WD) al[i] = swe_ld(swe_rsrc(p.valpha), v8, 0);
        }
#pragma unroll
        for (int f = 0; f < 3; f++) {
            const int b = (f + 1) % 3;
// ... 392 lines not shown
```

thetis_amd/csrc/swe2d_fuse.h:

```cpp
#pragma once
#include "swe2d_kernels.h"
#include "swe2d_flow.h"

#ifndef SWE_FUSE_WG
#define SWE_FUSE_WG 256
#endif
#ifndef SWE_FUSE_MIN_WG
#define SWE_FUSE_MIN_WG 3
#endif
#ifndef SWE_FUSE_INNER
#define SWE_FUSE_INNER 192
#endif
#define SWE_FUSE_FBITS 10
#define SWE_FUSE_RING (SWE_FUSE_WG - SWE_FUSE_INNER)
#define SWE_FUSE_XG (9*SWE_FUSE_WG)
#define SWE_FUSE_MAX_OUT (2*SWE_FUSE_RING)
#define SWE_FUSE_LDS (SWE_FUSE_XG + 6*SWE_FUSE_MAX_OUT)

struct SweFuseArgs {
    SweStageArgs st;
    const int2 *tile;
    const int *n_inner;
    int n_tiles;
    int cell_end;
    double beta1;
    double a0_2, a1_2, beta2;
    double *out;
};

template <bool NONLIN, bool LF, bool SRC = false>
__global__ __launch_bounds__(SWE_FUSE_WG, SWE_FUSE_MIN_WG) void swe_fuse12_kernel(const SweFuseArgs q)
{
#pragma clang fp contract(off)
    __shared__ double lds[SWE_FUSE_LDS];
    __shared__ double lw[9][SWE_FUSE_INNER];
    const SweStageArgs &p = q.st;
    const int tile = swe_logical_block(blockIdx.x, gridDim.x);
    if (tile >= q.n_tiles) return;
    const int lane = (int)threadIdx.x;
    const int2 tl = q.tile[(size_t)tile*SWE_FUSE_WG + lane];
    const bool real = tl.x >= 0;
    const int k = real ? tl.x : 0;
    const int n_inner = q.n_inner[tile];
    const size_t S = p.stride;
    const unsigned S8 = (unsigned)S*8u, k8 = (unsigned)k*8u;

    int bmarkers = 0, bkind1 = 0;
    unsigned tr[3][1];
    double h[3], nx[3], ny[3], u[3], v[3], e[3];
    if (real) {
        int nb[3], vid[3];
        swe_conn_load(p.idxc, p.idx4, p.idx2, k, nb, vid);
        bmarkers = (nb[0] < 0 ? -nb[0] : 0) | (nb[1] < 0 ? (-nb[1]) << 8 : 0) | (nb[2] < 0 ? (-nb[2]) << 16 : 0);
        if (bmarkers != 0) {
            const int m1 = (bmarkers & 0xff) ? (bmarkers & 0xff) : ((bmarkers & 0xff00) ? ((bmarkers >> 8) & 0xff) : (bmarkers >> 16));
            bkind1 = m1 < SWE_MAX_MARKERS ? p.bc.kind[m1] : 0;
        }
        const swe_rsrc_t gu = swe_rsrc(p.uin), gv = swe_rsrc(p.uin + 3*S), ge = swe_rsrc(p.uin + 6*S);
#pragma unroll
        for (int i = 0; i < 3; i++) {
            u[i] = swe_ld(gu, k8, i*S8);
            v[i] = swe_ld(gv, k8, i*S8);
            e[i] = swe_ld(ge, k8, i*S8);
        }
        double r0[3][6];
        bool outside[3];
#pragma unroll
        for (int f = 0; f < 3; f++) {
            const int nbf = nb[f];
            const unsigned w = ((unsigned)tl.y >> (SWE_FUSE_FBITS*f)) & 0x3ffu;
            outside[f] = (w & 0x200u) != 0u;
            const unsigned at = w & 0x1ffu;
            const int f2 = nbf >= 0 ? (nbf & 3) : f, f2a = f2 == 2 ? 0 : f2 + 1;
            {
                const unsigned ab = outside[f] ? (unsigned)(SWE_FUSE_XG + 6*at) : (unsigned)(f2*SWE_FUSE_WG + at);
                const unsigned aa = outside[f] ? (unsigned)(SWE_FUSE_XG + 6*at + 3) : (unsigned)(f2a*SWE_FUSE_WG + at);
                tr[f][0] = ab | (aa << 16);
            }
            const int code = outside[f] ? nbf : ((k << 2) | f);
            const unsigned kn8 = (unsigned)(code >> 2)*8u;
            const int g2 = code & 3;
            const unsigned ob = kn8 + (g2 == 0 ? 0u : (g2 == 1 ? S8 : 2u*S8));
            const unsigned oa = kn8 + (g2 == 0 ? S8 : (g2 == 1 ? 2u*S8 : 0u));
            r0[f][0] = swe_ld(gu, ob, 0); r0[f][1] = swe_ld(gv, ob, 0); r0[f][2] = swe_ld(ge, ob, 0);
            r0[f][3] = swe_ld(gu, oa, 0); r0[f][4] = swe_ld(gv, oa, 0); r0[f][5] = swe_ld(ge, oa, 0);
        }
        double px[3], py[3];
        const swe_rsrc_t rvx = swe_rsrc(p.vx), rvy = swe_rsrc(p.vy), rvh = swe_rsrc(p.vh);
#pragma unroll
        for (int i = 0; i < 3; i++) {
            const unsigned v8 = (unsigned)vid[i]*8u;
            px[i] = swe_ld(rvx, v8, 0);
            py[i] = swe_ld(rvy, v8, 0);
            h[i] = swe_ld(rvh, v8, 0);
        }
#pragma unroll
        for (int f = 0; f < 3; f++) {
            const int b = (f + 1) % 3;
            nx[f] = py[b] - py[f];
            ny[f] = px[f] - px[b];
        }
#pragma unroll
        for (int i = 0; i < 3; i++) { lds[i*SWE_FUSE_WG + lane] = u[i]; lds[(3 + i)*SWE_FUSE_WG + lane] = v[i]; lds[(6 + i)*SWE_FUSE_WG + lane] = e[i]; }
#pragma unroll
        for (int f = 0; f < 3; f++) {
            if (outside[f]) {
                const unsigned at = ((unsigned)tl.y >> (SWE_FUSE_FBITS*f)) & 0x1ffu;
#pragma unroll
                for (int j = 0; j < 6; j++) lds[SWE_LDSI(SWE_FUSE_XG + 6*at + j, SWE_FUSE_LDS)] = r0[f][j];
            }
        }
    }
    __syncthreads();
    double o1u[3], o1v[3], o1e[3];
    double twoA = 0.0;
    if (real) {
        twoA = fma(nx[0], ny[1], -(ny[0]*nx[1]));
        double bu[3], bv[3], be[3], wu[3], wv[3], we[3];
        swe_flow_rhs_cell<NONLIN>(p, u, v, e, h, nx, ny, bu, bv, be);
        swe_flow_rhs_facets<NONLIN, LF, SRC, 1, false, SWE_FUSE_XG, SWE_FUSE_WG, SWE_FUSE_LDS>(p, k, u, v, e, h, lds, tr, bmarkers, nx, ny, twoA, bu, bv, be);
#pragma unroll
        for (int i = 0; i < 3; i++) { wu[i] = 1.0*u[i]; wv[i] = 1.0*v[i]; we[i] = 1.0*e[i]; }
        swe_flow_finish<NONLIN, LF, true>(p, k, q.beta1, u, v, e, h, nx, ny, twoA, bmarkers, bkind1, bu, bv, be, wu, wv, we, o1u, o1v, o1e);
    }
    __syncthreads();
    if (real) {
#pragma unroll
        for (int i = 0; i < 3; i++) { lds[i*SWE_FUSE_WG + lane] = o1u[i]; lds[(3 + i)*SWE_FUSE_WG + lane] = o1v[i]; lds[(6 + i)*SWE_FUSE_WG + lane] = o1e[i]; }
    }
    const bool act2 = lane < n_inner && k < q.cell_end;
    if (act2) {
#pragma unroll
        for (int i = 0; i < 3; i++) {
            lw[i][lane] = fma(q.a0_2, u[i], q.a1_2*o1u[i]);
            lw[3 + i][lane] = fma(q.a0_2, v[i], q.a1_2*o1v[i]);
            lw[6 + i][lane] = fma(q.a0_2, e[i], q.a1_2*o1e[i]);
        }
    }
    __syncthreads();
    if (act2) {
#pragma unroll
        for (int i = 0; i < 3; i++) asm volatile("" : "+v"(nx[i]), "+v"(ny[i]), "+v"(h[i]));
#pragma unroll
        for (int f = 0; f < 3; f++) asm volatile("" : "+v"(tr[f][0]));
        asm volatile("" : "+v"(bmarkers), "+v"(twoA));
        double bu[3], bv[3], be[3], wu[3], wv[3], we[3], ou[3], ov[3], oe[3];
        swe_flow_rhs_cell<NONLIN>(p, o1u, o1v, o1e, h, nx, ny, bu, bv, be);
        swe_flow_rhs_facets<NONLIN, LF, SRC, 1, false, SWE_FUSE_XG, SWE_FUSE_WG, SWE_FUSE_LDS>(p, k, o1u, o1v, o1e, h, lds, tr, bmarkers, nx, ny, twoA, bu, bv, be);
#pragma unroll
        for (int i = 0; i < 3; i++) { wu[i] = lw[i][lane]; wv[i] = lw[3 + i][lane]; we[i] = lw[6 + i][lane]; }
        swe_flow_finish<NONLIN, LF, true>(p, k, q.beta2, o1u, o1v, o1e, h, nx, ny, twoA, bmarkers, bkind1, bu, bv, be, wu, wv, we, ou, ov, oe);
        const swe_rsrc_t gou = swe_rsrc(q.out), gov = swe_rsrc(q.out + 3*S), goe = swe_rsrc(q.out + 6*S);
#pragma unroll
        for (int i = 0; i < 3; i++) {
            swe_st(gou, k8, i*S8, ou[i]);
            swe_st(gov, k8, i*S8, ov[i]);
            swe_st(goe, k8, i*S8, oe[i]);
        }
    }
}

#define SWE_FUSE3_XG (18*SWE_FUSE_WG)
#ifndef SWE_FUSE3_MAX_OUT
#define SWE_FUSE3_MAX_OUT 224
#endif
#define SWE_FUSE3_LDS (SWE_FUSE3_XG + 6*SWE_FUSE3_MAX_OUT)
#ifndef SWE_FUSE3_SRC_MIN_WG
#define SWE_FUSE3_SRC_MIN_WG 2
#endif

struct SweFuse3Args {
    SweStageArgs st;
    const int2 *tile;
    const int2 *counts;
    int n_tiles;
    int cell_end;
    double a0[3], a1[3], beta[3];
    double *out;
};

template <bool NONLIN, bool LF, bool SRC = false>
__global__ __launch_bounds__(SWE_FUSE_WG, SRC ? SWE_FUSE3_SRC_MIN_WG : SWE_FUSE_MIN_WG) void swe_fuse123_kernel(const SweFuse3Args q)
{
#pragma clang fp contract(off)
    __shared__ double lds[SWE_FUSE3_LDS];
    const SweStageArgs &p = q.st;
    const int tile = swe_logical_block(blockIdx.x, gridDim.x);
    if (tile >= q.n_tiles) return;
    const int lane = (int)threadIdx.x;
    const int2 tl = q.tile[(size_t)tile*SWE_FUSE_WG + lane];
    const bool real = tl.x >= 0;
    const int k = real ? tl.x : 0;
    const int2 cnt = q.counts[tile];
    const size_t S = p.stride;
    const unsigned S8 = (unsigned)S*8u, k8 = (unsigned)k*8u;
    double *const P1 = lds + 9*SWE_FUSE_WG;

    int bmarkers = 0, bkind1 = 0;
    unsigned tr[3][1];
    double h[3], nx[3], ny[3], u[3], v[3], e[3];
    if (real) {
        int nb[3], vid[3];
        swe_conn_load(p.idxc, p.idx4, p.idx2, k, nb, vid);
        bmarkers = (nb[0] < 0 ? -nb[0] : 0) | (nb[1] < 0 ? (-nb[1]) << 8 : 0) | (nb[2] < 0 ? (-nb[2]) << 16 : 0);
        if (bmarkers != 0) {
            const int m1 = (bmarkers & 0xff) ? (bmarkers & 0xff) : ((bmarkers & 0xff00) ? ((bmarkers >> 8) & 0xff) : (bmarkers >> 16));
            bkind1 = m1 < SWE_MAX_MARKERS ? p.bc.kind[m1] : 0;
        }
        const swe_rsrc_t gu = swe_rsrc(p.uin), gv = swe_rsrc(p.uin + 3*S), ge = swe_rsrc(p.uin + 6*S);
#pragma unroll
        for (int i = 0; i < 3; i++) {
            u[i] = swe_ld(gu, k8, i*S8);
            v[i] = swe_ld(gv, k8, i*S8);
            e[i] = swe_ld(ge, k8, i*S8);
        }
        double r0[3][6];
        bool outside[3];
#pragma unroll
        for (int f = 0; f < 3; f++) {
            const int nbf = nb[f];
            const unsigned w = ((unsigned)tl.y >> (SWE_FUSE_FBITS*f)) & 0x3ffu;
            outside[f] = (w & 0x200u) != 0u;
            const unsigned at = w & 0x1ffu;
            const int f2 = nbf >= 0 ? (nbf & 3) : f, f2a = f2 == 2 ? 0 : f2 + 1;
            {
                const unsigned ab = outside[f] ? (unsigned)(SWE_FUSE3_XG + 6*at) : (unsigned)(f2*SWE_FUSE_WG + at);
                const unsigned aa = outside[f] ? (unsigned)(SWE_FUSE3_XG + 6*at + 3) : (unsigned)(f2a*SWE_FUSE_WG + at);
                tr[f][0] = ab | (aa << 16);
            }
            const int code = outside[f] ? nbf : ((k << 2) | f);
            const unsigned kn8 = (unsigned)(code >> 2)*8u;
            const int g2 = code & 3;
            const unsigned ob = kn8 + (g2 == 0 ? 0u : (g2 == 1 ? S8 : 2u*S8));
            const unsigned oa = kn8 + (g2 == 0 ? S8 : (g2 == 1 ? 2u*S8 : 0u));
            r0[f][0] = swe_ld(gu, ob, 0); r0[f][1] = swe_ld(gv, ob, 0); r0[f][2] = swe_ld(ge, ob, 0);
            r0[f][3] = swe_ld(gu, oa, 0); r0[f][4] = swe_ld(gv, oa, 0); r0[f][5] = swe_ld(ge, oa, 0);
        }
        double px[3], py[3];
        const swe_rsrc_t rvx = swe_rsrc(p.vx), rvy = swe_rsrc(p.vy), rvh = swe_rsrc(p.vh);
#pragma unroll
        for (int i = 0; i < 3; i++) {
            const unsigned v8 = (unsigned)vid[i]*8u;
            px[i] = swe_ld(rvx, v8, 0);
            py[i] = swe_ld(rvy, v8, 0);
            h[i] = swe_ld(rvh, v8, 0);
        }
#pragma unroll
        for (int f = 0; f < 3; f++) {
            const int b = (f + 1) % 3;
            nx[f] = py[b] - py[f];
            ny[f] = px[f] - px[b];
        }
#pragma unroll
        for (int i = 0; i < 3; i++) { lds[i*SWE_FUSE_WG + lane] = u[i]; lds[(3 + i)*SWE_FUSE_WG + lane] = v[i]; lds[(6 + i)*SWE_FUSE_WG + lane] = e[i]; }
#pragma unroll
        for (int f = 0; f < 3; f++) {
            if (outside[f]) {
                const unsigned at = ((unsigned)tl.y >> (SWE_FUSE_FBITS*f)) & 0x1ffu;
#pragma unroll
                for (int j = 0; j < 6; j++) lds[SWE_LDSI(SWE_FUSE3_XG + 6*at + j, SWE_FUSE3_LDS)] = r0[f][j];
            }
        }
    }
    __syncthreads();
    double twoA = 0.0;
    if (real) {
        twoA = fma(nx[0], ny[1], -(ny[0]*nx[1]));
        double bu[3], bv[3], be[3], wu[3], wv[3], we[3], ou[3], ov[3], oe[3];
        swe_flow_rhs_cell<NONLIN>(p, u, v, e, h, nx, ny, bu, bv, be);
        swe_flow_rhs_facets<NONLIN, LF, SRC, 1, false, SWE_FUSE3_XG, SWE_FUSE_WG, SWE_FUSE3_LDS>(p, k, u, v, e, h, lds, tr, bmarkers, nx, ny, twoA, bu, bv, be);
#pragma unroll
        for (int i = 0; i < 3; i++) { wu[i] = 1.0*u[i]; wv[i] = 1.0*v[i]; we[i] = 1.0*e[i]; }
        swe_flow_finish<NONLIN, LF, true>(p, k, q.beta[0], u, v, e, h, nx, ny, twoA, bmarkers, bkind1, bu, bv, be, wu, wv, we, ou, ov, oe);
#pragma unroll
        for (int i = 0; i < 3; i++) { u[i] = ou[i]; v[i] = ov[i]; e[i] = oe[i]; }
#pragma unroll
        for (int i = 0; i < 3; i++) { P1[i*SWE_FUSE_WG + lane] = u[i]; P1[(3 + i)*SWE_FUSE_WG + lane] = v[i]; P1[(6 + i)*SWE_FUSE_WG + lane] = e[i]; }
    }
    __syncthreads();
#pragma unroll 1
    for (int s = 1; s < 3; s++) {
        const bool act = lane < (s == 1 ? cnt.y : cnt.x) && (s == 1 || k < q.cell_end);
        double ou[3], ov[3], oe[3];
        if (act) {
#pragma unroll
            for (int i = 0; i < 3; i++) asm volatile("" : "+v"(nx[i]), "+v"(ny[i]), "+v"(h[i]));
#pragma unroll
            for (int f = 0; f < 3; f++) asm volatile("" : "+v"(tr[f][0]));
            asm volatile("" : "+v"(bmarkers), "+v"(twoA));
            double bu[3], bv[3], be[3], wu[3], wv[3], we[3];
            swe_flow_rhs_cell<NONLIN>(p, u, v, e, h, nx, ny, bu, bv, be);
            swe_flow_rhs_facets<NONLIN, LF, SRC, 1, false, SWE_FUSE3_XG, SWE_FUSE_WG, 9*SWE_FUSE_WG>(p, k, u, v, e, h, P1, tr, bmarkers, nx, ny, twoA, bu, bv, be);
            const double a0 = q.a0[s], a1 = q.a1[s];
#pragma unroll
            for (int i = 0; i < 3; i++) {
                wu[i] = fma(a0, lds[i*SWE_FUSE_WG + lane], a1*u[i]);
                wv[i] = fma(a0, lds[(3 + i)*SWE_FUSE_WG + lane], a1*v[i]);
                we[i] = fma(a0, lds[(6 + i)*SWE_FUSE_WG + lane], a1*e[i]);
            }
            swe_flow_finish<NONLIN, LF, true>(p, k, q.beta[s], u, v, e, h, nx, ny, twoA, bmarkers, bkind1, bu, bv, be, wu, wv, we, ou, ov, oe);
        }
        if (s == 1) {
            __syncthreads();
            if (act) {
#pragma unroll
                for (int i = 0; i < 3; i++) { P1[i*SWE_FUSE_WG + lane] = ou[i]; P1[(3 + i)*SWE_FUSE_WG + lane] = ov[i]; P1[(6 + i)*SWE_FUSE_WG + lane] = oe[i]; }
#pragma unroll
                for (int i = 0; i < 3; i++) { u[i] = ou[i]; v[i] = ov[i]; e[i] = oe[i]; }
            }
            __syncthreads();
        } else if (act) {
            const swe_rsrc_t gou = swe_rsrc(q.out), gov = swe_rsrc(q.out + 3*S), goe = swe_rsrc(q.out + 6*S);
#pragma unroll
            for (int i = 0; i < 3; i++) {
                swe_st(gou, k8, i*S8, ou[i]);
                swe_st(gov, k8, i*S8, ov[i]);
                swe_st(goe, k8, i*S8, oe[i]);
            }
        }
    }
}


#define SWE_QFUSE_INNER 192
#define SWE_QFUSE_RING (SWE_FUSE_WG - SWE_QFUSE_INNER)
#define SWE_QFUSE_XG (12*SWE_FUSE_WG)
#define SWE_QFUSE_MAX_OUT (3*SWE_QFUSE_RING)
#define SWE_QFUSE_LDS (SWE_QFUSE_XG + 6*SWE_QFUSE_MAX_OUT)

struct SweFuseQuadArgs {
    SweStageArgs st;
    const int4 *tile;
    const int *n_inner;
    int n_tiles;
    int cell_end;
    double beta1, a0_2, a1_2, beta2;
    double *out;
};

template <bool NONLIN, bool LF, bool SRC, bool AFFINE>
__global__ __launch_bounds__(SWE_FUSE_WG, SWE_FUSE_MIN_WG) void swe_fuse12_quad_kernel(const SweFuseQuadArgs q)
{
#pragma clang fp contract(off)
    __shared__ double lds[SWE_QFUSE_LDS];
    __shared__ double lu0[12*SWE_QFUSE_INNER];
    const SweStageArgs &p = q.st;
    const int tile = swe_logical_block(blockIdx.x, gridDim.x);
    if (tile >= q.n_tiles) return;
    const int lane = (int)threadIdx.x;
    const int4 tl = q.tile[(size_t)tile*SWE_FUSE_WG + lane];
    const bool real = tl.x >= 0;
    const int k = real ? tl.x : 0;
    const int n_inner = q.n_inner[tile];
    const size_t S = p.stride;
    const unsigned S8 = (unsigned)S*8u, k8 = (unsigned)k*8u, S4 = (unsigned)S*4u, k4 = (unsigned)k*4u;

    unsigned tr[4] = {0u, 0u, 0u, 0u}, bmarkers = 0u;
    int nb[4] = {-1, -1, -1, -1}, vid[4] = {0, 0, 0, 0};
    double u[4], v[4], e[4];
    if (real) {
#pragma unroll
        for (int i = 0; i < 4; i++) {
            nb[i] = swe_ldi(swe_rsrc(p.nbr), k4, i*S4);
            vid[i] = swe_ldi(swe_rsrc(p.cv), k4, i*S4);
        }
        const swe_rsrc_t gu = swe_rsrc(p.uin), gv = swe_rsrc(p.uin + 4*S), ge = swe_rsrc(p.uin + 8*S);
#pragma unroll
        for (int i = 0; i < 4; i++) {
            u[i] = swe_ld(gu, k8, i*S8);
            v[i] = swe_ld(gv, k8, i*S8);
            e[i] = swe_ld(ge, k8, i*S8);
        }
        bmarkers = (nb[0] < 0 ? (unsigned)(-nb[0]) : 0u) | (nb[1] < 0 ? (unsigned)(-nb[1]) << 8 : 0u) |
                   (nb[2] < 0 ? (unsigned)(-nb[2]) << 16 : 0u) | (nb[3] < 0 ? (unsigned)(-nb[3]) << 24 : 0u);
        double r0[4][6];
        bool outside[4];
#pragma unroll
        for (int f = 0; f < 4; f++) {
            const int nbf = nb[f];
            const unsigned w = f < 3 ? (((unsigned)tl.y >> (SWE_FUSE_FBITS*f)) & 0x3ffu) : ((unsigned)tl.z & 0x3ffu);
            outside[f] = (w & 0x200u) != 0u;
            const unsigned at = w & 0x1ffu;
            const int f2 = nbf >= 0 ? (nbf & 3) : f, na = (f2 + 1) & 3;
            const unsigned ab = outside[f] ? (unsigned)(SWE_QFUSE_XG + 6*at) : (unsigned)(f2*SWE_FUSE_WG + at);
            const unsigned aa = outside[f] ? (unsigned)(SWE_QFUSE_XG + 6*at + 3) : (unsigned)(na*SWE_FUSE_WG + at);
            tr[f] = ab | (aa << 16);
            const int code = outside[f] ? nbf : ((k << 2) | f);
            const unsigned kn8 = (unsigned)(code >> 2)*8u;
            const int g2 = code & 3, ga = (g2 + 1) & 3;
            const unsigned ob = kn8 + ((g2 & 1) ? S8 : 0u) + ((g2 & 2) ? 2u*S8 : 0u);
            const unsigned oa = kn8 + ((ga & 1) ? S8 : 0u) + ((ga & 2) ? 2u*S8 : 0u);
            r0[f][0] = swe_ld(gu, ob, 0); r0[f][1] = swe_ld(gv, ob, 0); r0[f][2] = swe_ld(ge, ob, 0);
            r0[f][3] = swe_ld(gu, oa, 0); r0[f][4] = swe_ld(gv, oa, 0); r0[f][5] = swe_ld(ge, oa, 0);
        }
#pragma unroll
        for (int i = 0; i < 4; i++) { lds[i*SWE_FUSE_WG + lane] = u[i]; lds[(4 + i)*SWE_FUSE_WG + lane] = v[i]; lds[(8 + i)*SWE_FUSE_WG + lane] = e[i]; }
#pragma unroll
        for (int f = 0; f < 4; f++) {
            if (outside[f]) {
                const unsigned at = (f < 3 ? ((unsigned)tl.y >> (SWE_FUSE_FBITS*f)) : (unsigned)tl.z) & 0x1ffu;
#pragma unroll
                for (int j = 0; j < 6; j++) lds[SWE_LDSI(SWE_QFUSE_XG + 6*at + j, SWE_QFUSE_LDS)] = r0[f][j];
            }
        }
    }
    __syncthreads();
#define SWE_QFUSE_TRACES(una, unb, vna, vnb, ena, enb) \
    _Pragma("unroll") \
    for (int f = 0; f < 4; f++) { \
        const unsigned ab = tr[f] & 0xffffu, aa = tr[f] >> 16; \
        const unsigned step = ab >= (unsigned)SWE_QFUSE_XG ? 1u : (unsigned)(4*SWE_FUSE_WG); \
        unb[f] = lds[SWE_LDSI(ab, SWE_QFUSE_LDS)]; vnb[f] = lds[SWE_LDSI(ab + step, SWE_QFUSE_LDS)]; enb[f] = lds[SWE_LDSI(ab + 2u*step, SWE_QFUSE_LDS)]; \
        una[f] = lds[SWE_LDSI(aa, SWE_QFUSE_LDS)]; vna[f] = lds[SWE_LDSI(aa + step, SWE_QFUSE_LDS)]; ena[f] = lds[SWE_LDSI(aa + 2u*step, SWE_QFUSE_LDS)]; \
    }
    double o1u[4], o1v[4], o1e[4];
    if (real) {
        double una[4], unb[4], vna[4], vnb[4], ena[4], enb[4];
        SWE_QFUSE_TRACES(una, unb, vna, vnb, ena, enb)
        swe_quad_stage_cell<NONLIN, LF, false, SRC, false, AFFINE, true>(p, k, k8, S8, nb, vid, bmarkers, u, v, e, una, unb, vna, vnb, ena, enb,
                                                                        0.0, 1.0, q.beta1, lds, SWE_FUSE_WG, lane, nullptr, 0, o1u, o1v, o1e);
    }
    __syncthreads();
    const bool act2 = lane < n_inner && k < q.cell_end;
    if (real) {
#pragma unroll
        for (int i = 0; i < 4; i++) { lds[i*SWE_FUSE_WG + lane] = o1u[i]; lds[(4 + i)*SWE_FUSE_WG + lane] = o1v[i]; lds[(8 + i)*SWE_FUSE_WG + lane] = o1e[i]; }
    }
    if (act2) {
#pragma unroll
        for (int i = 0; i < 4; i++) { lu0[i*SWE_QFUSE_INNER + lane] = u[i]; lu0[(4 + i)*SWE_QFUSE_INNER + lane] = v[i]; lu0[(8 + i)*SWE_QFUSE_INNER + lane] = e[i]; }
    }
    __syncthreads();
    if (act2) {
#pragma unroll
        for (int f = 0; f < 4; f++) asm volatile("" : "+v"(tr[f]));
        asm volatile("" : "+v"(bmarkers));
        double una[4], unb[4], vna[4], vnb[4], ena[4], enb[4], ou[4], ov[4], oe[4];
        SWE_QFUSE_TRACES(una, unb, vna, vnb, ena, enb)
        swe_quad_stage_cell<NONLIN, LF, true, SRC, false, AFFINE, true>(p, k, k8, S8, nb, vid, bmarkers, o1u, o1v, o1e, una, unb, vna, vnb, ena, enb,
                                                                       q.a0_2, q.a1_2, q.beta2, lds, SWE_FUSE_WG, lane, lu0, SWE_QFUSE_INNER, ou, ov, oe);
        const swe_rsrc_t gou = swe_rsrc(q.out), gov = swe_rsrc(q.out + 4*S), goe = swe_rsrc(q.out + 8*S);
#pragma unroll
        for (int i = 0; i < 4; i++) {
            swe_st(gou, k8, i*S8, ou[i]);
            swe_st(gov, k8, i*S8, ov[i]);
            swe_st(goe, k8, i*S8, oe[i]);
        }
    }
#undef SWE_QFUSE_TRACES
}
```

thetis_amd/csrc/swe2d_handle.h:

```cpp
#pragma once
#include "../../include/swe2d.h"
#include "swe2d_kernels.h"
#include "swe2d_sipg.h"
#include "swe2d_flow.h"
#include "swe2d_p2p.h"

#include <dlfcn.h>
#include <unistd.h>

#include <algorithm>
#include <cmath>
#include <cstdio>
#include <cstdlib>
#include <cstring>
#include <new>
#include <string>
#include <vector>
#include <atomic>
#include <mutex>

static_assert(SWE2D_MAX_MARKERS == SWE_MAX_MARKERS, "marker table size mismatch");
static_assert(SWE2D_MAX_FARMS == SWE_MAX_FARMS && SWE2D_MAX_THRUST_TABLE == SWE_MAX_THRUST_TABLE, "turbine farm table size mismatch");

#ifdef SWE_RANGE_CHECK
#include <map>
#include <mutex>
namespace {
std::mutex g_chk_mutex;
std::map<unsigned long long, unsigned long long> g_chk_allocs;
bool g_chk_dirty = true;
unsigned long long g_chk_launches = 0;
void swe_chk_upload_locked()
{
    static SweChkTable t;
    t.n = 0;
    for (auto &kv : g_chk_allocs) if (t.n < SWE_CHK_MAX) { t.lo[t.n] = kv.first; t.hi[t.n] = kv.second; t.n++; }
    (void)hipDeviceSynchronize();
    (void)hipMemcpyToSymbol(HIP_SYMBOL(swe_chk_tab), &t, sizeof(t));
    g_chk_dirty = false;
}
hipError_t swe_chk_malloc(void **p, size_t n)
{
    const hipError_t e = hipMalloc(p, n);
    if (e == hipSuccess && *p) {
        std::lock_guard<std::mutex> lock(g_chk_mutex);
        const char *st = getenv("THETIS_AMD_RANGE_SELFTEST");
        g_chk_allocs[(unsigned long long)*p] = (unsigned long long)*p + ((st && atoi(st)) ? n/2 : n);
        swe_chk_upload_locked();
    }
    return e;
}
template <class T> hipError_t swe_chk_malloc(T **p, size_t n) { return swe_chk_malloc((void **)p, n); }
hipError_t swe_chk_free(void *p)
{
    { std::lock_guard<std::mutex> lock(g_chk_mutex); g_chk_allocs.erase((unsigned long long)p); g_chk_dirty = true; }
    return hipFree(p);
}
void swe_chk_sync(hipStream_t stream)
{
    std::lock_guard<std::mutex> lock(g_chk_mutex);
    g_chk_launches++;
    if (!g_chk_dirty) return;
    hipStreamCaptureStatus cs = hipStreamCaptureStatusNone;
    if (stream && hipStreamIsCapturing(stream, &cs) == hipSuccess && cs != hipStreamCaptureStatusNone) return;
    swe_chk_upload_locked();
}
}
#define hipMalloc(p, n) swe_chk_malloc(p, n)
#define hipFree(p) swe_chk_free(p)
#define SWE_CHK_SYNC(stream) swe_chk_sync(stream)
extern "C" int swe2d_debug_range_report(unsigned long long out[5])
{
    std::lock_guard<std::mutex> lock(g_chk_mutex);
    (void)hipDeviceSynchronize();
    if (hipMemcpyFromSymbol(out, HIP_SYMBOL(swe_chk_report), 4*sizeof(unsigned long long)) != hipSuccess) return 1;
    out[3] = g_chk_launches;
    out[4] = g_chk_allocs.size();
    return 0;
}
#else
#define SWE_CHK_SYNC(stream) ((void)0)
#endif

namespace swe2d_impl {

extern thread_local std::string g_create_error;

extern const double kBeta[3], kAlpha0[3], kAlphaIn[3];

extern std::atomic<unsigned long long> g_next_uid;

struct Handle {
    unsigned long long uid = g_next_uid.fetch_add(1ull);
    int device = 0;
    hipStream_t stream = nullptr;
    bool own_stream = false;
    hipStream_t my_stream = nullptr;
    hipStream_t xstream = nullptr;
    int n_cells = 0, n_owned = 0, n_interior = 0, n_vertices = 0;
    int npc = 3;
    bool affine = true;
    bool affine_local = true;
    size_t stride = 0;
    double *state[3] = {nullptr, nullptr, nullptr};
    int *nbr = nullptr, *cv = nullptr;
    struct FacetList { std::vector<int32_t> cells, facets; int *dev = nullptr; };
    FacetList facet_lists[8];
    int facet_list_next = 0;
    int4 *opp4 = nullptr;
    int *bnd_cells = nullptr;
    int n_bnd = 0;
    int opt[SWE2D_OPT_COUNT];
    Handle() { for (int i = 0; i < SWE2D_OPT_COUNT; i++) opt[i] = -1; }
    bool stage_valid[2] = {false, false};
    int capture_swaps = 0;
    unsigned long long capture_id = 0;
    int capture_odd = 0;
    int4 *idx4 = nullptr;
    int2 *idx2 = nullptr;
    int4 *idxc = nullptr;
    int2 *fuse_tile = nullptr;
    int *fuse_inner = nullptr;
    int fuse_n_tiles = 0;
    int fuse_state = 0;
    long long fuse_ring_cells = 0;
    int4 *fuseq_tile = nullptr;
    int *fuseq_inner = nullptr;
    int fuseq_n_tiles = 0;
    long long fuseq_ring_cells = 0;
    int2 *fuse3_tile = nullptr, *fuse3_cnt = nullptr;
    int fuse3_n_tiles = 0;
    long long fuse3_ring1 = 0, fuse3_ring2 = 0;
    std::vector<int> fuse_order;
    std::vector<int> fuse3_order;
    std::vector<unsigned char> fuse3_start;
    int n_conn_escapes = 0;
    std::vector<int> h_nbr;
    unsigned *flow_flag = nullptr, *flow_status = nullptr;
    int4 *flow_xo4 = nullptr;
    int2 *flow_xo2 = nullptr;
    int2 *flow_xblk = nullptr;
    int *flow_xsrc = nullptr;
    std::vector<int> h_send, h_recv;
    std::vector<int> flow_fpos;
    int2 *flow_xsend = nullptr;
    int *flow_xrecv = nullptr;
    unsigned *flow_xtick = nullptr;
    int flow_push_blocks = 0, flow_recv_blocks = 0;
    bool flow_x_ready = false;
    int *flow_cell = nullptr;
    unsigned flow_parity_bytes = 0;
    void *flow_ex = nullptr;
    size_t flow_ex_bytes = 0;
    int flow_blocks = 0;
    int flow_capacity = -1;
    int flow_max_rim = 0;
    int launch_parity = 0;
    bool flow_used = false;
    double *vx = nullptr, *vy = nullptr, *vh = nullptr;
    double *bc_field[4] = {nullptr, nullptr, nullptr, nullptr};
    double *valpha = nullptr;
    bool wd = false;
    bool state_holds_D = false;
    struct Snapshot { void *data = nullptr; size_t bytes = 0; bool holds_D = false; };
    Snapshot snapshot[SWE2D_SNAPSHOT_SLOTS];
    bool visc = false;
    double *nu_v = nullptr;
    double nu_const = 0.0, sipg_factor = 1.0;
    int visc_grad_div = 0, visc_grad_depth = 1;
    double *field[SWE2D_FIELD_COUNT] = {nullptr, nullptr, nullptr, nullptr, nullptr, nullptr, nullptr, nullptr, nullptr};
    double scalar[SWE2D_SCALAR_COUNT] = {-1.0, -1.0, -1.0, 0.0, -1.0};
    double *stage_uv = nullptr, *stage_eta = nullptr;
    double *partial = nullptr;
    int n_partial_blocks = 0;
    unsigned long long *diag_acc = nullptr;
    int *send_cells = nullptr, *recv_cells = nullptr;
    int n_send = 0, n_recv = 0;
    struct P2p {
        void *zone = nullptr;
        size_t zone_bytes = 0;
        int zone_kind = 0;
        int n_channels = 0;
        int width[SWE_P2P_MAX_CHANNELS] = {0};
        SweP2pCounters *ctr = nullptr;
        std::vector<void *> opened;
        int n_peers = 0, n_from = 0;
        int off[SWE_P2P_MAX_PEERS], cnt[SWE_P2P_MAX_PEERS], remote_off[SWE_P2P_MAX_PEERS], remote_flag[SWE_P2P_MAX_PEERS],
            remote_n_recv[SWE_P2P_MAX_PEERS];
        char *remote_base[SWE_P2P_MAX_PEERS];
    } p2p;
    struct Tracer {
        double *buf[3] = {nullptr, nullptr, nullptr};
        double *source = nullptr;
        bool conservative = false;
        double *bc_value_f = nullptr;
        int bc_vel_kind[SWE_MAX_MARKERS];
        double bc_u[SWE_MAX_MARKERS], bc_v[SWE_MAX_MARKERS];
        double *bc_vel_f = nullptr;
        int bc_vel_field[SWE_MAX_MARKERS];
        int bc_has_value[SWE_MAX_MARKERS];
        double bc_value[SWE_MAX_MARKERS];
        bool diff = false;
        double *mu_v = nullptr;
        double mu_const = 0.0, sipg_factor = 1.0;
        int bc_diff_kind[SWE_MAX_MARKERS];
        double bc_diff_flux[SWE_MAX_MARKERS];
    };
    std::vector<Tracer> tracers;
    int tracer_use_lf = 0;
    double tracer_lf_factor = 1.0, tracer_vel_factor = 1.0;
    std::vector<int> host_cells;
    std::vector<int> host_nbr;
    int lim_nv = 0;
    int *lim_v2c_off = nullptr, *lim_v2c_cell = nullptr, *lim_vbf_off = nullptr, *lim_vbf_facet = nullptr, *lim_tv = nullptr;
    double *lim_mean = nullptr, *lim_qmin = nullptr, *lim_qmax = nullptr;
    struct Probe {
        bool live = false;
        int n_points = 0, width = 0, capacity = 0, rows = 0;
        int *cell = nullptr;
        double *weight = nullptr;
        double *out = nullptr;
        std::vector<int> fields;
    };
    std::vector<Probe> probes;
    struct Farm {
        bool live = false;
        swe2d_turbine_params par{};
        double *density = nullptr;
        int *cells = nullptr;
        int n_list = 0;
    };
    Farm farms[SWE2D_MAX_FARMS];
    int n_farms = 0;
    SweFarmTable *farm_table = nullptr;
    int farm_blocks = 0;
    unsigned long long *farm_rows = nullptr;
    int farm_rows_cap = 0, farm_rows_n = 0;
    swe2d_params par{};
    SweBcTable bc{};
    hipEvent_t ev0 = nullptr, ev1 = nullptr;
    std::string err;
};

inline Handle *H(swe2d_handle *h) { return reinterpret_cast<Handle *>(h); }
inline const Handle *H(const swe2d_handle *h) { return reinterpret_cast<const Handle *>(h); }

int fail(Handle *h, int code, const std::string &msg);

#define HIP_TRY(h, expr)                                                                         \
    do {                                                                                         \
        hipError_t e_ = (expr);                                                                  \
        if (e_ != hipSuccess) {                                                                  \
             \
            (void)hipGetLastError();                                                             \
            return fail(h, SWE2D_ERR_HIP, std::string(#expr) + ": " + hipGetErrorString(e_));     \
        }                                                                                        \
    } while (0)

struct RoctxRange {
    typedef int (*push_t)(const char *);
    typedef int (*pop_t)();
    static void resolve(push_t &push, pop_t &pop)
    {
        static bool done = false;
        static push_t p_push = nullptr;
        static pop_t p_pop = nullptr;
        if (!done) {
            done = true;
            {
                for (const char *name : {"librocprofiler-sdk-roctx.so", "libroctx64.so"}) {
                    if (void *lib = dlopen(name, RTLD_NOW | RTLD_GLOBAL)) {
                        p_push = reinterpret_cast<push_t>(dlsym(lib, "roctxRangePushA"));
                        p_pop = reinterpret_cast<pop_t>(dlsym(lib, "roctxRangePop"));
                        if (p_push && p_pop) break;
                        p_push = nullptr; p_pop = nullptr;
                    }
                }
            }
        }
        push = p_push; pop = p_pop;
    }
    pop_t pop_ = nullptr;
    RoctxRange(const Handle *h, const char *name);
    ~RoctxRange() { if (pop_) pop_(); }
};
inline RoctxRange::RoctxRange(const Handle *h, const char *name)
{
    if (!h || h->opt[SWE2D_OPT_ROCTX] <= 0) return;
    push_t push;
    resolve(push, pop_);
    if (push) push(name); else pop_ = nullptr;
}


inline bool has_sources(const Handle *h)
{
    for (int i = 0; i < SWE2D_FIELD_COUNT; i++) if (h->field[i]) return true;
    if (h->n_farms > 0) return true;
    return h->scalar[SWE2D_SCALAR_LINEAR_DRAG] >= 0 || h->scalar[SWE2D_SCALAR_QUADRATIC_DRAG] >= 0
           || h->scalar[SWE2D_SCALAR_MANNING_DRAG] >= 0 || h->scalar[SWE2D_SCALAR_NIKURADSE] >= 0;
}

inline int grid_for(int n) { return (n + 255)/256; }

inline bool opt_on(const Handle *h, int o) { return h->opt[o] != 0; }
inline double opt_seconds(const Handle *h, int o, double dflt) { return h->opt[o] > 0 ? 1e-3*h->opt[o] : dflt; }

inline bool conn_pays(const Handle *h, int n_cells_of_launch, bool arithmetic_bound)
{
    const int o = h->opt[SWE2D_OPT_COMPACT_IDX];
    return h->idxc && o != 0 && (o == 2 || (n_cells_of_launch >= 250000 && !arithmetic_bound));
}
bool fuse12_covers(const Handle *h);
int fuse12_build(Handle *h);
int launch_fuse12(Handle *h, int cell_end);
bool fuse123_wanted(const Handle *h);
int fuse123_build(Handle *h);
int launch_fuse123(Handle *h, int cell_end);
int capture_parity_check(Handle *h);
bool stream_capturing(Handle *h, unsigned long long *id = nullptr);
void stage_written(Handle *h, bool s0, bool s1);
int step_swe(Handle *h);
void fill_stage_args(Handle *h, SweStageArgs &a, int in, int u0, int out, double a0, double a1, double beta, int c0, int c1);
int launch_stage(Handle *h, int in, int u0, int out, double a0, double a1, double beta, int c0, int c1);
int stage_on_range(Handle *h, int i_stage, int c0, int c1);
int scatter_facet_values(Handle *h, double *planes, int n, const int32_t *cells, const int32_t *facets,
                         const double *values, int ncomp, int nval);
int upload_vertex_coefficient(Handle *h, const double *vertex_values, double **dev);
int flow_build(Handle *h, const int32_t *order);
bool flow_kernel_covers(const Handle *h);
int flow_capacity(Handle *h);
int flow_build_exchange(Handle *h);
int launch_flow(Handle *h, int n_stages, const int32_t *cell_end, int n_cycles = 0);
int flow_check(Handle *h);
size_t p2p_channel_offset(const int *width, int c, int n_recv);
void probe_free_all(Handle *h);
void farm_free_all(Handle *h);

}
using namespace swe2d_impl;
```

thetis_amd/device.py:

```python
import ctypes
import os
import numpy as np

from . import _lib, ordering

__all__ = ['Swe2dDevice']

_dp = ctypes.POINTER(ctypes.c_double)


def _ptr(a):
    return a.ctypes.data_as(_dp)


def _iptr(a):
    return a.ctypes.data_as(ctypes.POINTER(ctypes.c_int32))


class FacetValues(object):

    def __init__(self, values):
        self.values = np.asarray(values, dtype=np.float64)


class Swe2dDevice(object):
    def __init__(self, mesh, bathymetry_vertex, dt, g_grav=9.81, use_nonlinear_equations=True,
                 use_lax_friedrichs_velocity=True, lax_friedrichs_velocity_scaling_factor=1.0,
                 device_id=0, n_owned=None, boundary_len=None, reorder='auto', ranges=None):
        self.lib = _lib.load()
        self.n_cells = int(mesh.cells.shape[0])
        self.npc = int(mesh.cells.shape[1])
        self.n_owned = self.n_cells if n_owned is None else int(n_owned)
        c = np.ascontiguousarray
        cells0 = np.asarray(mesh.cells)
        xy0 = np.asarray(mesh.vertex_xy, dtype=np.float64)
        nbr0 = np.asarray(mesh.cell_nbr)
        nbf0 = np.asarray(mesh.cell_nbr_facet)
        bath0 = np.asarray(bathymetry_vertex, dtype=np.float64)
        if bath0.shape != (xy0.shape[0],):
            raise ValueError('bathymetry must have one value per vertex')
        markers = sorted(int(m) for m in np.unique(-nbr0[nbr0 < 0])) if (nbr0 < 0).any() else []
        if len(markers) >= _lib.MAX_MARKERS:
            raise NotImplementedError('more than {:d} distinct boundary markers'.format(_lib.MAX_MARKERS - 1))
        self._marker_slot = {m: i + 1 for i, m in enumerate(markers)}
        if markers and markers != list(range(1, len(markers) + 1)):
            lut = np.zeros(max(markers) + 1, dtype=np.int64)
            for m, sl in self._marker_slot.items():
                lut[m] = sl
            nbr0 = np.where(nbr0 < 0, -lut[np.where(nbr0 < 0, -nbr0, 0)], nbr0)
        self._caller_nbr = np.array(nbr0)
        if boundary_len is not None:
            boundary_len = {self._marker_slot[m]: v for m, v in boundary_len.items() if m in self._marker_slot}
        self.perm = None
        self._vperm = None
        if reorder is not None:
            if isinstance(reorder, str):
                if reorder not in ('hilbert', 'auto'):
                    raise ValueError('unknown reorder {!r}'.format(reorder))
                cen = xy0[cells0].mean(axis=1)
                bounds = [0] + [int(b) for b in (ranges or (self.n_owned,))] + [self.n_cells]
                bounds = sorted(set(bounds))
                perm = np.arange(self.n_cells)
                for a, b in zip(bounds[:-1], bounds[1:]):
                    if b - a > 1 and a < self.n_owned:
                        if reorder == 'auto':
                            perm[a:b] = a + ordering.auto_cell_order(mesh, a, b)
                        else:
                            perm[a:b] = a + ordering.hilbert_cell_order(cen[a:b])
            else:
                perm = np.asarray(reorder, dtype=np.int64)
                assert sorted(perm) == list(range(self.n_cells))
            inv = np.empty_like(perm)
            inv[perm] = np.arange(self.n_cells)
            self.perm, self.inv_perm = perm, inv
            cells0 = cells0[perm]
            nb = nbr0[perm].astype(np.int64)
            pos = nb >= 0
            nb[pos] = inv[nb[pos]]
            nbr0 = nb
            nbf0 = nbf0[perm]
            vperm = ordering.first_touch_vertex_order(cells0)
            vinv = np.full(xy0.shape[0], -1, dtype=np.int64)
            vinv[vperm] = np.arange(len(vperm))
            cells0 = vinv[cells0]
            xy0 = xy0[vperm]
            bath0 = bath0[vperm]
            self._vperm = vperm
        self._topo_cells = None
        self._limiter_ready = False
        topo = getattr(mesh, 'topo_vertex', None)
        if topo is not None and not np.array_equal(np.asarray(topo), np.arange(len(topo))):
            tc = np.asarray(topo)[np.asarray(mesh.cells)]
            if self.perm is not None:
                tc = tc[self.perm]
            _, tc = np.unique(tc, return_inverse=True)
            self._topo_cells = tc.reshape(-1, self.npc)
        self._keep = [c(cells0, dtype=np.int32), c(xy0, dtype=np.float64),
                      c(nbr0, dtype=np.int32), c(nbf0, dtype=np.int8), c(bath0, dtype=np.float64)]
        cells, xy, nbr, nbf, bath = self._keep
        m = _lib.Swe2dMesh()
        m.n_cells = self.n_cells
        m.n_owned = self.n_owned
        m.n_vertices = xy.shape[0]
        m.nodes_per_cell = self.npc
        m.cell_vertices = cells.ctypes.data_as(ctypes.POINTER(ctypes.c_int32))
        m.vertex_xy = _ptr(xy)
        m.cell_neighbours = nbr.ctypes.data_as(ctypes.POINTER(ctypes.c_int32))
        m.cell_neighbour_facets = nbf.ctypes.data_as(ctypes.POINTER(ctypes.c_int8))
        m.bathymetry = _ptr(bath)
        if boundary_len is not None:
            bl = np.zeros(_lib.MAX_MARKERS)
            for k, v in boundary_len.items():
                if 0 < k < _lib.MAX_MARKERS:
                    bl[k] = v
            self._keep.append(bl)
            m.boundary_len = _ptr(bl)
        p = _lib.Swe2dParams()
        p.g_grav = g_grav
        p.dt = dt
        p.use_nonlinear_equations = int(bool(use_nonlinear_equations))
        p.use_lax_friedrichs_velocity = int(bool(use_lax_friedrichs_velocity))
        p.lax_friedrichs_velocity_scaling_factor = float(lax_friedrichs_velocity_scaling_factor)
        p.device_id = device_id
        self.h = ctypes.c_void_p()
        _lib.check(self.lib.swe2d_create(ctypes.byref(m), ctypes.byref(p), ctypes.byref(self.h)))
        for opt, value in _lib.options_from_environment():
            self.set_option(opt, value)
        if (self.npc == 3 and isinstance(reorder, str) and self.n_owned == self.n_cells and 64 < self.n_cells <= 196608
                and os.environ.get('THETIS_AMD_FLOW_BLOCKS', '1') != '0'):
            self.flow_set_order(ordering.flow_block_order(mesh))
        tt = ordering.triple_tile_shape() if self.npc == 3 else None
        if (self.npc == 3 and isinstance(reorder, str) and self.n_owned == self.n_cells and getattr(mesh, 'structured', False)
                and self.n_cells > 131072 and tt is not None):
            self.fused_set_triple_tiles(*ordering.triple_tile_order(mesh, *tt))
        if self.npc == 4 and not getattr(mesh, 'affine', True):
            self._ck(self.lib.swe2d_set_general_quadrilaterals(self.h, 1))

    def close(self):
        if getattr(self, 'h', None) is not None and self.h:
            self.lib.swe2d_destroy(self.h)
            self.h = None

    def __del__(self):
        try:
            self.close()
        except Exception:
            pass

    def _ck(self, rc):
        _lib.check(rc, self.h)

    def set_state(self, uv, eta):
        uv = np.asarray(uv, dtype=np.float64).reshape(self.n_cells, self.npc, 2)
        eta = np.asarray(eta, dtype=np.float64).reshape(self.n_cells, self.npc)
        if self.perm is not None:
            uv, eta = uv[self.perm], eta[self.perm]
        uv, eta = np.ascontiguousarray(uv), np.ascontiguousarray(eta)
        self._ck(self.lib.swe2d_set_state(self.h, _ptr(uv), _ptr(eta)))

    def get_state(self, i_stage=2):
        uv = np.empty((self.n_cells, self.npc, 2))
        eta = np.empty((self.n_cells, self.npc))
        self._ck(self.lib.swe2d_get_stage_state(self.h, int(i_stage), _ptr(uv), _ptr(eta)))
        if self.perm is not None:
            uv, eta = uv[self.inv_perm], eta[self.inv_perm]
        return uv, eta

    def snapshot(self, slot=0):
        self._ck(self.lib.swe2d_state_snapshot_slot(self.h, int(slot), 0))

    def restore(self, slot=0):
        self._ck(self.lib.swe2d_state_snapshot_slot(self.h, int(slot), 1))

    def set_option(self, option, value):
        self._ck(self.lib.swe2d_set_option(self.h, int(option), -1 if value is None else int(value)))

    def get_option(self, option):
        v = ctypes.c_int(0)
        self._ck(self.lib.swe2d_get_option(self.h, int(option), ctypes.byref(v)))
        return v.value

    def set_dt(self, dt):
        self._ck(self.lib.swe2d_set_dt(self.h, float(dt)))

    def _slot(self, marker):
        try:
            return self._marker_slot[int(marker)]
        except KeyError:
            raise KeyError('the mesh has no boundary with marker {:}'.format(marker))

    def set_bc(self, marker, funcs):
        marker = self._slot(marker)
        kind = 0
        vals = np.zeros(5)
        is_field = lambda v: isinstance(v, FacetValues) or (isinstance(v, np.ndarray) and v.ndim >= 2)
        for key, value in (funcs or {}).items():
            if key == 'elev':
                kind |= _lib.BC_ELEV
                if is_field(value):
                    kind |= _lib.BC_ELEV_FIELD
                    self._set_bc_function(0, marker, value)
                else:
                    vals[0] = float(value)
            elif key == 'uv':
                kind |= _lib.BC_UV
                if is_field(value):
                    kind |= _lib.BC_UV_FIELD
                    self._set_bc_function(1, marker, value)
                else:
                    vals[1], vals[2] = float(value[0]), float(value[1])
            elif key == 'un':
                kind |= _lib.BC_UN
                if is_field(value):
                    kind |= _lib.BC_UN_FIELD
                    self._set_bc_function(2, marker, value)
                else:
                    vals[3] = float(value)
            elif key == 'flux':
                kind |= _lib.BC_FLUX
                if is_field(value):
                    kind |= _lib.BC_FLUX_FIELD
                    self._set_bc_function(3, marker, value)
                else:
                    vals[4] = float(value)
            elif key == 'drag':
                pass
            else:
                raise Exception('Invalid boundary tag "{:}" specified on boundary {:}'.format(key, marker))
        self._ck(self.lib.swe2d_set_bc(self.h, int(marker), kind, _ptr(vals)))
        drag = (funcs or {}).get('drag')
        self._ck(self.lib.swe2d_set_boundary_drag(self.h, int(marker), -1.0 if drag is None else float(drag)))

    def set_wetting_and_drying(self, alpha):
        if alpha is None:
            self._ck(self.lib.swe2d_set_wetting_and_drying(self.h, 0, None))
            return
        nv = self._keep[1].shape[0]
        a = np.asarray(alpha, dtype=np.float64)
        if a.ndim == 0:
            a = np.full(nv, float(a))
        elif self._vperm is not None:
            a = a[self._vperm]
        a = np.ascontiguousarray(a)
        assert a.shape == (nv,), 'alpha must be a constant or have one value per vertex'
        self._ck(self.lib.swe2d_set_wetting_and_drying(self.h, 1, _ptr(a)))

    def _vertex_coefficient(self, value):
        a = np.asarray(value, dtype=np.float64)
        if a.ndim == 0:
            return None, float(a)
        nv = self._keep[1].shape[0]
        if self._vperm is not None:
            a = a[self._vperm]
        a = np.ascontiguousarray(a)
        assert a.shape == (nv,), 'coefficient must be a constant or have one value per vertex'
        return a, 0.0

    def set_viscosity(self, nu, sipg_factor=1.0, use_grad_div_viscosity_term=False, use_grad_depth_viscosity_term=True):
        if nu is None:
            self._ck(self.lib.swe2d_set_viscosity(self.h, 0, None, 0.0, 1.0, 0, 0))
            return
        arr, const = self._vertex_coefficient(nu)
        self._ck(self.lib.swe2d_set_viscosity(self.h, 1, None if arr is None else _ptr(arr), const, float(sipg_factor),
                                              int(bool(use_grad_div_viscosity_term)), int(bool(use_grad_depth_viscosity_term))))

    def tracer_set_conservative(self, tracer_id, use_conservative_form=True):
        self._ck(self.lib.swe2d_tracer_set_conservative(self.h, int(tracer_id), int(bool(use_conservative_form))))

    def tracer_set_diffusivity(self, tracer_id, mu, sipg_factor_tracer=1.0):
        if mu is None:
            self._ck(self.lib.swe2d_tracer_set_diffusivity(self.h, int(tracer_id), 0, None, 0.0, 1.0))
            return
        arr, const = self._vertex_coefficient(mu)
        self._ck(self.lib.swe2d_tracer_set_diffusivity(self.h, int(tracer_id), 1, None if arr is None else _ptr(arr), const,
                                                       float(sipg_factor_tracer)))

    def tracer_set_diffusion_bc(self, tracer_id, marker, kind, diff_flux=0.0):
        self._ck(self.lib.swe2d_tracer_set_diffusion_bc(self.h, int(tracer_id), self._slot(marker), int(kind), float(diff_flux)))

    def _set_bc_function(self, which, slot, value):
        if isinstance(value, FacetValues):
            self.set_bc_facets(which, slot, value.values)
        else:
            self.set_bc_field(which, slot, value)

    def facet_node_values(self, marker, function_values, cells_of_vertices=None):
        cells, facets = self.boundary_facets(self._slot(marker))
        nxt = (facets + 1) % self.npc
        d = np.asarray(function_values)
        if cells_of_vertices is None:
            return FacetValues(np.stack([d[cells, facets], d[cells, nxt]], axis=1))
        cv = np.asarray(cells_of_vertices)
        return FacetValues(np.stack([d[cv[cells, facets]], d[cv[cells, nxt]]], axis=1))

    def boundary_facets(self, slot):
        cache = self.__dict__.setdefault('_bnd_facets', {})
        if slot not in cache:
            c, f = np.nonzero(self._caller_nbr == -int(slot))
            cache[slot] = (np.ascontiguousarray(c.astype(np.int32)), np.ascontiguousarray(f.astype(np.int32)))
        return cache[slot]

    def _device_cells(self, cells):
        cache = self.__dict__.setdefault('_device_cell_lists', {})
        key = id(cells)
        if key not in cache:
            cache[key] = (cells, np.ascontiguousarray((cells if self.perm is None else self.inv_perm[cells]).astype(np.int32)))
        return cache[key][1]

    def set_bc_facets(self, which, slot, values):
        cells, facets = self.boundary_facets(slot)
        v = np.ascontiguousarray(np.asarray(values, dtype=np.float64).reshape((len(cells), 2, 2) if which == 1 else (len(cells), 2)))
        self._ck(self.lib.swe2d_set_bc_facets(self.h, int(which), len(cells), _iptr(self._device_cells(cells)), _iptr(facets),
                                              _ptr(v)))

    def tracer_set_bc_facets(self, tid, slot, values):
        cells, facets = self.boundary_facets(slot)
        v = np.ascontiguousarray(np.asarray(values, dtype=np.float64).reshape(len(cells), self.npc))
        self._ck(self.lib.swe2d_tracer_set_bc_facets(self.h, int(tid), len(cells), _iptr(self._device_cells(cells)),
                                                     _iptr(facets), _ptr(v)))
        self._ck(self.lib.swe2d_tracer_set_bc(self.h, int(tid), int(slot), 2, 0.0))

    def set_bc_field(self, which, slot, nodal):
        shape = (self.n_cells, self.npc, 2) if which == 1 else (self.n_cells, self.npc)
        a = np.asarray(nodal, dtype=np.float64).reshape(shape)
        if self.perm is not None:
            a = a[self.perm]
        a = np.ascontiguousarray(a)
        self._ck(self.lib.swe2d_set_bc_field(self.h, int(which), int(slot), _ptr(a)))

    def set_field(self, field, nodal):
        if nodal is None:
            self._ck(self.lib.swe2d_set_field(self.h, field, None))
            return
        vec = field in (_lib.FIELD_MOMENTUM_SOURCE, _lib.FIELD_WIND_STRESS)
        shape = (self.n_cells, self.npc, 2) if vec else (self.n_cells, self.npc)
        a = np.broadcast_to(np.asarray(nodal, dtype=np.float64), shape)
        if self.perm is not None:
            a = a[self.perm]
        a = np.ascontiguousarray(a)
        self._ck(self.lib.swe2d_set_field(self.h, field, _ptr(a)))

    def set_field_vertex(self, field, vertex_values):
        vec = field in (_lib.FIELD_MOMENTUM_SOURCE, _lib.FIELD_WIND_STRESS)
        nv = self._keep[1].shape[0]
        a = np.asarray(vertex_values, dtype=np.float64).reshape((nv, 2) if vec else (nv,))
        if self._vperm is not None:
            a = a[self._vperm]
        a = np.ascontiguousarray(a)
        self._ck(self.lib.swe2d_set_field_vertex(self.h, field, _ptr(a)))

    def set_scalar(self, which, value):
        self._ck(self.lib.swe2d_set_scalar(self.h, which, -1.0 if value is None else float(value)))

    def advance(self, n_steps=1):
        self._ck(self.lib.swe2d_advance(self.h, int(n_steps)))

    def solve_stage(self, i_stage):
        self._ck(self.lib.swe2d_solve_stage(self.h, int(i_stage)))

    def advance_forward_euler(self, n_steps=1):
        self._ck(self.lib.swe2d_advance_forward_euler(self.h, int(n_steps)))

    def tracer_forward_euler(self, tid):
        self._ck(self.lib.swe2d_tracer_forward_euler(self.h, int(tid)))

    def solve_stage_cells(self, i_stage, cell_begin, cell_end):
        self._ck(self.lib.swe2d_solve_stage_cells(self.h, int(i_stage), int(cell_begin), int(cell_end)))

    def solve_stage_pair_cells(self, cell_end_0, cell_end_1):
        self._ck(self.lib.swe2d_solve_stage_pair_cells(self.h, int(cell_end_0), int(cell_end_1)))

    def solve_step_cells(self, cell_end):
        self._ck(self.lib.swe2d_solve_step_cells(self.h, int(cell_end)))

    def fused_step_info(self):
        out = (ctypes.c_int32*4)()
        self._ck(self.lib.swe2d_fused_step_info(self.h, out))
        return bool(out[0]), int(out[1]), int(out[2]), int(out[3])

    def fused_set_order(self, cells_in_tile_order):
        if cells_in_tile_order is None:
            self._ck(self.lib.swe2d_fused_set_order(self.h, None))
            return
        order = np.asarray(cells_in_tile_order, dtype=np.int64)
        if self.perm is not None:
            order = self.inv_perm[order]
        order = np.ascontiguousarray(order, dtype=np.int32)
        self._ck(self.lib.swe2d_fused_set_order(self.h, _iptr(order)))

    def fused_set_triple_tiles(self, cells_in_tile_order, tile_starts=None):
        if cells_in_tile_order is None:
            self._ck(self.lib.swe2d_fused_set_triple_tiles(self.h, None, None, 0))
            return
        order = np.asarray(cells_in_tile_order, dtype=np.int64)
        if self.perm is not None:
            order = self.inv_perm[order]
        order = np.ascontiguousarray(order, dtype=np.int32)
        starts = np.ascontiguousarray(np.zeros(0) if tile_starts is None else tile_starts, dtype=np.int32)
        self._ck(self.lib.swe2d_fused_set_triple_tiles(self.h, _iptr(order), _iptr(starts) if len(starts) else None, len(starts)))

    def forward_euler_cells(self, cell_begin, cell_end):
        self._ck(self.lib.swe2d_forward_euler_cells(self.h, int(cell_begin), int(cell_end)))

    def swap_state_buffers(self):
        self._ck(self.lib.swe2d_swap_state_buffers(self.h))

    def solve_flow(self, cell_ends):
        ends = np.ascontiguousarray(cell_ends, dtype=np.int32)
        self._ck(self.lib.swe2d_solve_flow(self.h, int(len(ends)), _iptr(ends)))

    def solve_flow_exchange(self, n_cycles, cell_ends):
        ends = np.ascontiguousarray(cell_ends, dtype=np.int32)
        self._ck(self.lib.swe2d_solve_flow_exchange(self.h, int(n_cycles), int(len(ends)), _iptr(ends)))

    def flow_unpack_pending(self):
        self._ck(self.lib.swe2d_flow_unpack_pending(self.h))

    def flow_prepare_exchange(self):
        self._ck(self.lib.swe2d_flow_prepare_exchange(self.h))

    def flow_set_order(self, cells_in_flow_order):
        order = np.asarray(cells_in_flow_order, dtype=np.int64)
        if self.perm is not None:
            order = self.inv_perm[order]
        order = np.ascontiguousarray(order, dtype=np.int32)
        self._ck(self.lib.swe2d_flow_set_order(self.h, _iptr(order)))

    def flow_supported(self):
        return int(self.lib.swe2d_flow_supported(self.h))

    def connectivity_info(self):
        out = (ctypes.c_int32*2)()
        self._ck(self.lib.swe2d_connectivity_info(self.h, out))
        return int(out[0]), int(out[1])

    def fused_pair_info(self):
        out = (ctypes.c_int32*4)()
        self._ck(self.lib.swe2d_fused_pair_info(self.h, out))
        return bool(out[0]), int(out[1]), int(out[2]), int(out[3])

    def fused_triple_info(self):
        out = (ctypes.c_int32*4)()
        self._ck(self.lib.swe2d_fused_triple_info(self.h, out))
        return bool(out[0]), int(out[1]), int(out[2]), int(out[3])

    def flow_timeouts(self):
        n = ctypes.c_int32()
        self._ck(self.lib.swe2d_flow_status(self.h, ctypes.byref(n)))
        return n.value

    def advance_timed(self, n_steps, per_launch=False):
        tot = ctypes.c_float()
        avg = ctypes.c_float()
        self._ck(self.lib.swe2d_advance_timed(self.h, int(n_steps), int(per_launch), ctypes.byref(tot), ctypes.byref(avg)))
        return tot.value, avg.value

    def synchronize(self):
        self._ck(self.lib.swe2d_synchronize(self.h))

    def tendency(self):
        ku = np.empty((self.n_cells, self.npc, 2))
        ke = np.empty((self.n_cells, self.npc))
        self._ck(self.lib.swe2d_tendency(self.h, _ptr(ku), _ptr(ke)))
        if self.perm is not None:
            ku, ke = ku[self.inv_perm], ke[self.inv_perm]
        return ku, ke

    def diagnostics(self):
        out = np.empty(4)
        self._ck(self.lib.swe2d_diagnostics(self.h, _ptr(out)))
        return out

    def diagnostics_limbs(self):
        limbs = np.zeros(3*_lib.SUM_LIMBS, dtype=np.int64)
        lo = ctypes.c_double()
        self._ck(self.lib.swe2d_diagnostics_limbs(self.h, limbs.ctypes.data_as(ctypes.POINTER(ctypes.c_int64)), ctypes.byref(lo)))
        return limbs.reshape(3, _lib.SUM_LIMBS), float(lo.value)

    def tracer_diagnostics_limbs(self, tid):
        limbs = np.zeros(2*_lib.SUM_LIMBS, dtype=np.int64)
        mm = np.empty(2)
        self._ck(self.lib.swe2d_tracer_diagnostics_limbs(self.h, int(tid), limbs.ctypes.data_as(ctypes.POINTER(ctypes.c_int64)), _ptr(mm)))
        return limbs.reshape(2, _lib.SUM_LIMBS), mm

    def limbs_to_double(self, limbs):
        a = np.ascontiguousarray(limbs, dtype=np.int64).reshape(_lib.SUM_LIMBS)
        return float(self.lib.swe2d_sum_limbs_to_double(a.ctypes.data_as(ctypes.POINTER(ctypes.c_int64))))

    _PROBE_FIELDS = {'uv': _lib.PROBE_UV, 'elev': _lib.PROBE_ELEV}

    def probe_create(self, cells, weights, fields, capacity=0):
        cells = np.asarray(cells, dtype=np.int64).reshape(-1)
        dev = np.ascontiguousarray((cells if self.perm is None else self.inv_perm[cells]).astype(np.int32))
        w = np.ascontiguousarray(np.asarray(weights, dtype=np.float64).reshape(len(cells), self.npc))
        codes = np.ascontiguousarray([self._PROBE_FIELDS[f] if isinstance(f, str) else int(f) for f in fields], dtype=np.int32)
        pid = ctypes.c_int32()
        self._ck(self.lib.swe2d_probe_create(self.h, len(dev), _iptr(dev), _ptr(w), len(codes), _iptr(codes), int(capacity),
                                             ctypes.byref(pid)))
        return pid.value

    def probe_shape(self, pid):
        m, w, c = ctypes.c_int32(), ctypes.c_int32(), ctypes.c_int32()
        self._ck(self.lib.swe2d_probe_width(self.h, int(pid), ctypes.byref(m), ctypes.byref(w), ctypes.byref(c)))
        return m.value, w.value, c.value

    def probe_append(self, pid):
        if pid == self.TURBINE_ROWS:
            return self.turbine_rows_append()
        self._ck(self.lib.swe2d_probe_append(self.h, int(pid)))

    def probe_read(self, pid):
        if pid == self.TURBINE_ROWS:
            return self.turbine_rows_read()
        m, w, c = self.probe_shape(pid)
        out = np.empty((max(c, 1), m, w))
        n = ctypes.c_int32()
        self._ck(self.lib.swe2d_probe_read(self.h, int(pid), _ptr(out), ctypes.byref(n)))
        return out[:n.value].copy()

    def probe_eval(self, pid):
        m, w, _ = self.probe_shape(pid)
        out = np.empty((m, w))
        self._ck(self.lib.swe2d_probe_eval(self.h, int(pid), _ptr(out)))
        return out

    def probe_destroy(self, pid):
        self._ck(self.lib.swe2d_probe_destroy(self.h, int(pid)))

    TURBINE_ROWS = -100

    def turbine_farm_set(self, farm, params, density_nodal):
        d = self._nodal_in(density_nodal)
        self._ck(self.lib.swe2d_turbine_farm_set(self.h, int(farm), ctypes.byref(params), _ptr(d)))

    def turbine_farm_clear(self, farm):
        self._ck(self.lib.swe2d_turbine_farm_clear(self.h, int(farm)))

    def turbine_power(self):
        out = np.zeros(_lib.MAX_FARMS)
        self._ck(self.lib.swe2d_turbine_power(self.h, _ptr(out)))
        return out

# ... 193 lines not shown
```

thetis_amd/distributed.py:

```python
import os

import numpy as np

from .partition import build_partition, strip_owner

__all__ = ['HaloExchanger', 'P2PHalo', 'DistributedSwe2d', 'state_digest']
_TEST_FAILED_ONCE = []


class HaloExchanger(object):

    def __init__(self, part, device, host_staged=False, width=None, group=None):
        import torch
        self.part = part
        self.group = group
        self.w = w = 3*int(part.cells.shape[1]) if width is None else int(width)
        self.send_buf = torch.zeros(max(1, len(part.send_cells))*w, dtype=torch.float64, device=device)
        self.recv_buf = torch.zeros(max(1, len(part.recv_cells))*w, dtype=torch.float64, device=device)
        self.host_staged = host_staged
        if host_staged:
            self._send_h = torch.zeros_like(self.send_buf, device='cpu')
            self._recv_h = torch.zeros_like(self.recv_buf, device='cpu')

    def start(self):
# ... 77 lines not shown
        return self.dev.p2p_status(self.n_channels)[2]


def coupled_halo_depth(exchange_every, use_limiter, stages_per_step=3):
    sps = int(stages_per_step)
    return (sps + 1 if use_limiter else sps)*int(exchange_every) + sps


def coupled_cycle_schedule(part, n_steps, n_tracers, use_limiter, tracer_only=False, stages_per_step=3):
    sps = int(stages_per_step)
    depth = coupled_halo_depth(n_steps, use_limiter, sps)
    if depth > len(part.layer_sizes):
        raise ValueError('a coupled cycle of {:d} steps needs {:d} ghost layers, the partition has {:d}'.format(
            n_steps, depth, len(part.layer_sizes)))
    v_swe = v_t = depth
    ops = []
    for k in range(n_steps):
        if not tracer_only:
            for g in range(sps):
                v_swe -= 1
                ops.append(('swe', g, part.layer_end(v_swe)))
            if k == n_steps - 1:
                ops.append(('swe_done',))
        v_in = min(v_t, v_swe)
        for i in range(n_tracers):
            for g in range(sps):
                ops.append(('tracer', i, g, part.layer_end(v_in - 1 - g)))
        v_t = v_in - sps
        if use_limiter:
            v_t -= 1
            for i in range(n_tracers):
                ops.append(('limit', i, part.layer_end(v_t)))
    assert v_t >= 0 and v_swe >= 0
    return ops


class DistributedSwe2d(object):

    def __init__(self, mesh, bathymetry_vertex, dt, rank, world_size, device_id, owner=None, host_staged=False,
                 n_tracers=0, use_limiter=True, tracer_only=False, exchange_every=1, overlap_stages=0,
                 graph_mode=None, stepper='SSPRK33', exchange=None, split_last_stage=True, group=None, partition=None,
                 combined_exchange=False, flow=None, flow_exchange=None, device_cls=None, **opts):
        import torch
        from .device import Swe2dDevice
        device_cls = Swe2dDevice if device_cls is None else device_cls
        self._on_gpu = not getattr(device_cls, 'is_host', False)
        self.rank, self.world = rank, world_size
        self.group = group
        if partition is None:
            owner = strip_owner(mesh, world_size) if owner is None else owner
        self.use_limiter = bool(use_limiter) and n_tracers > 0
        self.tracer_only = bool(tracer_only)
        if stepper not in ('SSPRK33', 'ForwardEuler'):
            raise ValueError("stepper must be 'SSPRK33' or 'ForwardEuler'")
        self.stages_per_step = 3 if stepper == 'SSPRK33' else 1
        if self.stages_per_step == 1 and int(overlap_stages) > 0:
            raise ValueError('ForwardEuler on partitions: no overlap_stages')
        self.exchange_every = m = int(exchange_every)
        self.overlap_stages = int(overlap_stages)
        if m < 1:
            raise ValueError('exchange_every must be >= 1')
        self.coupled_cycles = n_tracers > 0 and (m > 1 or bool(combined_exchange) or self.stages_per_step == 1)
        if self.overlap_stages > 0 and n_tracers > 0 and (not self.coupled_cycles or tracer_only):
            raise ValueError('overlap_stages on coupled runs needs the combined exchange (exchange_every > 1 or '
                             'combined_exchange=True) and a shallow water step to overlap with (not tracer_only)')
        if not 0 <= self.overlap_stages <= 3*m - 1:
            raise ValueError('overlap_stages must be in 0 .. 3*exchange_every - 1')
        self.exchange = exchange or ('host' if host_staged else 'rccl')
        if self.exchange not in ('p2p', 'rccl', 'host'):
            raise ValueError("exchange must be 'p2p', 'rccl' or 'host'")
        self.split_last_stage = bool(split_last_stage)
        if not self.split_last_stage and self.overlap_stages:
            raise ValueError('overlap_stages needs split_last_stage')
        if partition is not None:
            self.part = partition
        elif self.coupled_cycles:
            self.part = build_partition(mesh, owner, rank, halo_depth=coupled_halo_depth(m, self.use_limiter, self.stages_per_step),
                                        adjacency='vertex' if self.use_limiter else 'facet')
        elif self.stages_per_step == 1:
            self.part = build_partition(mesh, owner, rank, halo_depth=m)
        elif m > 1:
            self.part = build_partition(mesh, owner, rank, halo_depth=3*m)
        elif self.use_limiter:
            self.part = build_partition(mesh, owner, rank, halo_depth=4, adjacency='vertex')
        else:
            self.part = build_partition(mesh, owner, rank)
        p = self.part
        if self._on_gpu:
            torch.cuda.set_device(device_id)
            self.torch_device = torch.device('cuda', device_id)
        else:
            self.torch_device = torch.device('cpu')
            if self.exchange != 'host':
                raise ValueError("a host stand-in device exchanges through host memory: exchange='host'")
        self._flow_request = flow
        ve = opts.pop('verify_every', None)
        self._verify_every = int(ve if ve is not None else os.environ.get('THETIS_AMD_VERIFY_EVERY', '0') or 0)
        self._v_snapshot, self._v_steps = None, 0
        self._replaying = False
        self._distrust = 0
        self.verify_report = {'windows': 0, 'mismatches': 0, 'bad_ranks': []}
        self._host_halos = {}
        self._flowx_request = flow_exchange
        self._flow_now = None
        self._flowx_now = False
        self._flow_epoch, self._decided_epoch = 0, None
        self._no_exchange = False
        self._shared_device = None
        self.dev = None
        self.tids = []
        self.halo = self.thalo = self.p2p = None
        try:
            self._build_handle(device_cls, p, bathymetry_vertex, dt, device_id, n_tracers, opts)
            local_error = None
        except Exception as e:
            if self.exchange != 'p2p' or world_size == 1:
                raise
            local_error = '{:}: {:}'.format(type(e).__name__, (str(e).strip().splitlines() or [''])[0])
        if self.exchange == 'p2p':
            try:
                self.p2p = P2PHalo(self.dev, p, rank, world_size, n_tracers=n_tracers, group=group, local_error=local_error)
            except Exception:
                if self.dev is not None:
                    self.dev.close()
                raise
        else:
            staged = self.exchange == 'host' and self._on_gpu
            self.halo = HaloExchanger(p, self.torch_device, host_staged=staged, group=group)
            self.thalo = HaloExchanger(p, self.torch_device, host_staged=staged, width=p.cells.shape[1], group=group) if n_tracers else None
        self._finish_init(graph_mode)

    def _build_handle(self, device_cls, p, bathymetry_vertex, dt, device_id, n_tracers, opts):
        flow = self._flow_request
        if os.environ.get('THETIS_AMD_TEST_FAIL_HANDLE_RANK') == str(self.rank) and not _TEST_FAILED_ONCE:
            _TEST_FAILED_ONCE.append(1)
            raise RuntimeError('THETIS_AMD_TEST_FAIL_HANDLE_RANK')
        self.dev = device_cls(p, np.asarray(bathymetry_vertex)[p.vertex_global], dt, device_id=device_id,
                              n_owned=p.n_owned, boundary_len=p.boundary_len, ranges=p.reorder_ranges(), **opts)
        self.dev.halo_setup(p.send_cells, p.recv_cells)
        if os.environ.get('THETIS_AMD_TEST_TEAR'):
            us, ev = (int(v) for v in os.environ['THETIS_AMD_TEST_TEAR'].split(':'))
            if self.dev.lib.swe2d_debug_flow_tear(self.dev.h, -2, us, ev, 1) != 0:
                raise RuntimeError('THETIS_AMD_TEST_TEAR needs the -DSWE_FLOW_TEAR build of the library')
        if flow is not False and self.dev.npc == 3 and self._on_gpu:
            from . import ordering
            blocks = os.environ.get('THETIS_AMD_FLOW_BLOCKS', '1') != '0'
            self.dev.flow_set_order((ordering.flow_block_order if blocks else ordering.auto_cell_order)(p, 0, p.num_cells))
        if self.dev.npc == 3 and self._on_gpu:
            from . import ordering
            order = ordering.fused_tile_order(p)
            if order is not None:
                self.dev.fused_set_order(order)
            self.dev.fused_pair_info()
            tt = ordering.triple_tile_shape()
            tiles = ordering.triple_tile_order(p, *tt) if tt is not None else None
            if tiles is not None:
                self.dev.fused_set_triple_tiles(*tiles)
            self.dev.fused_step_info()
        self._ranges = [p.stage_range(i) for i in range(3)]
        self.tids = [self.dev.add_tracer() for _ in range(n_tracers)]

    def _finish_init(self, graph_mode):
        import torch
        self.xstream = None
        if self._on_gpu:
            self.stream = torch.cuda.Stream(device=self.torch_device)
            self.dev.set_stream(self.stream.cuda_stream)
            if self.p2p is not None and os.environ.get('THETIS_AMD_P2P_SIDE_STREAM', '0') == '1':
                self.xstream = torch.cuda.Stream(device=self.torch_device)
                self.dev.set_exchange_stream(self.xstream.cuda_stream)
                self._ev_fork = torch.cuda.Event()
                self._ev_join = torch.cuda.Event()
                self._ev_pushed = torch.cuda.Event()
        else:
            self.stream = None
        self.graph = None
        self.graph_steps = 0
        self.graph_mode = graph_mode or os.environ.get('THETIS_AMD_GRAPH_MODE', 'cycle')
        if self.stages_per_step == 1:
            self.graph_mode = 'none'
        if self.graph_mode not in ('cycle', 'full', 'none'):
            raise ValueError("graph_mode / THETIS_AMD_GRAPH_MODE must be 'cycle', 'full' or 'none'")
        if self.exchange == 'host' and self.graph_mode == 'full':
            self.graph_mode = 'cycle'
        if not self._on_gpu:
            self.graph_mode = 'none'
        self._cycle_graphs = {}

    def close(self):
        self.dev.close()

    def _flow_local(self):
        if self._flow_request is False or os.environ.get('THETIS_AMD_FLOW') == '0' or not self._on_gpu or self._distrust:
            return False
        plain = (self.stages_per_step == 3 and not self.tids and not self.tracer_only and self.overlap_stages == 0
                 and 3*self.exchange_every <= 384)
        if not plain or not self.dev.flow_supported():
            if self._flow_request is True:
                raise ValueError('flow=True: the flow kernel covers SSPRK33 shallow-water-only runs on triangles without wetting-drying, '
                                 'viscosity and overlap_stages, on partitions whose 64-cell blocks are all resident at once')
            return False
        return True

    def _ranks_share_a_device(self):
        if self._shared_device is None:
            import socket
            import torch
            import torch.distributed as dist
            prop = torch.cuda.get_device_properties(self.torch_device)
            ident = (socket.gethostname(), str(getattr(prop, 'uuid', '')), getattr(prop, 'pci_bus_id', -1),
                     getattr(prop, 'pci_device_id', -1), getattr(prop, 'pci_domain_id', -1),
                     os.environ.get('HIP_VISIBLE_DEVICES', os.environ.get('ROCR_VISIBLE_DEVICES', '')), self.torch_device.index)
            everyone = [None]*self.world
            dist.all_gather_object(everyone, ident, group=self.group)
            self._shared_device = len(set(everyone)) < len(everyone)
        return self._shared_device

    def _flowx_local(self):
        if self.p2p is None or self._flowx_request is False or os.environ.get('THETIS_AMD_FLOWX') == '0':
            return False
        if self.dev.flow_supported() not in (1, 2):
            return False
        sc = np.asarray(self.part.send_cells)
        return not len(sc) or int(np.bincount(sc).max()) <= 2

    def _decide_flow(self):
        import torch.distributed as dist
        if self._flow_request is False or self.world == 1:
            self._flow_now = self._flow_local()
            self._flowx_now = self._flow_now and self._flowx_local()
            return self._flow_now
        if self._flow_request is True:
            if self._flow_now is None:
                try:
                    ok = self._flow_local()
                except ValueError:
                    ok = False
                okx = ok and self._flowx_local()
                both = self._all_reduce([1.0 if ok else 0.0, 1.0 if okx else 0.0], dist.ReduceOp.MIN)
                if both[0] < 0.5:
                    raise ValueError('flow=True: the flow kernel does not cover the partition of every rank (rank {:d}: {:})'.format(
                        self.rank, 'covered' if ok else 'not covered'))
                if self._flowx_request is True and both[1] < 0.5:
                    raise ValueError('flow_exchange=True: the exchange inside the flow launches needs the peer-to-peer transport and '
                                     'cells that go to at most two peers, on every rank (rank {:d}: {:})'.format(
                                         self.rank, 'possible' if okx else 'not possible'))
                self._flow_now, self._flowx_now = True, bool(both[1] > 0.5)
            return self._flow_now
        if self._decided_epoch == self._flow_epoch and self._flow_now is not None:
            return self._flow_now
        shared = self._ranks_share_a_device()
        ok = self._flow_local() and not shared
        okx = ok and self._flowx_local()
        both = self._all_reduce([1.0 if ok else 0.0, 1.0 if okx else 0.0], dist.ReduceOp.MIN)
        self._flow_now, self._flowx_now = bool(both[0] > 0.5), bool(both[1] > 0.5)
        self._decided_epoch = self._flow_epoch
        return self._flow_now

    def config_changed(self):
        self._flow_epoch += 1

    @property
    def flow(self):
        if self._replaying or self._distrust:
            return False
        return self._flow_local() if self._flow_now is None else self._flow_now

    @property
    def flow_exchange(self):
        if self._no_exchange or self._replaying or self._distrust:
            return False
        if self._flow_now is None:
            return self._flow_local() and self._flowx_local()
        return bool(self._flow_now and self._flowx_now)

    def _steps_flow_exchange(self, n_steps, graphed):
        dev, p, m = self.dev, self.part, self.exchange_every
        if graphed:
            dev.flow_prepare_exchange()
        full, rem = divmod(n_steps, m)
        per_launch = max(1, min(64, 384//(3*m), int(os.environ.get("THETIS_AMD_FLOWX_CYCLES", "64"))))
        ends = [p.stage_range(g, depth=3*m) for g in range(3*m)]
        while full > 0:
            nc = min(per_launch, full)
            self._launch(('X', nc, m), lambda nc=nc: dev.solve_flow_exchange(nc, ends), graphed)
            full -= nc
        if rem:
            ends_r = [p.stage_range(g, depth=3*rem) for g in range(3*rem)]
            self._launch(('X', 1, rem), lambda: dev.solve_flow_exchange(1, ends_r), graphed)
        self._launch(('XU',), lambda: dev.flow_unpack_pending(), graphed)

    def _cycle_swe_flow(self, n_steps, graphed):
        dev, p = self.dev, self.part
        n = 3*n_steps
        ends = [p.stage_range(g, depth=n) for g in range(n)]
        if self.p2p is not None:
            def whole_cycle():
                dev.solve_flow(ends)
                self._receive(0, 0, self._send(0, 0))
            return self._launch(('W', n_steps), whole_cycle, graphed)
        self._launch(('WA', n_steps), lambda: dev.solve_flow(ends), graphed)
        self._receive(0, 0, self._send(0, 0))

    def set_tracer_global(self, i_tracer, nodal):
        self.dev.tracer_set_state(self.tids[i_tracer], np.asarray(nodal)[self.part.local_to_global])

    def get_tracer_owned(self, i_tracer):
# ... 583 lines not shown
```

Measured before the change: 31.06 billion.

## Add 384-lane two-ring tile option and cache facet lengths in LDS across stages

Templates the fused three-stage kernel on workgroup size and adds an option for 384-lane tiles with larger patches, which lowers the halo ring overhead per tile. By default it stays at 256 lanes. It also computes facet length and reciprocal length once in stage 1 and keeps them in LDS for stages 2 and 3, instead of recomputing sqrt and rsqrt each stage. Without sources it also takes the reciprocal of the area once rather than on every call. The geometry cache reuses the ghost-ring LDS region, so the LDS budget is sized to 24*WG, and it adds an extra LDS round-trip.

```diff
diff --git a/include/swe2d.h b/include/swe2d.h
--- a/include/swe2d.h
+++ b/include/swe2d.h
@@ -67,7 +67,8 @@
     SWE2D_OPT_P2P_TIMEOUT_MS = 12,
     SWE2D_OPT_P2P_ZONE = 13,
     SWE2D_OPT_ROCTX = 14,
-    SWE2D_OPT_COUNT = 15
+    SWE2D_OPT_TRIPLE_LANES = 15,
+    SWE2D_OPT_COUNT = 16
 } swe2d_option;
 
 typedef struct {
diff --git a/thetis_amd/_lib.py b/thetis_amd/_lib.py
--- a/thetis_amd/_lib.py
+++ b/thetis_amd/_lib.py
@@ -16,8 +16,8 @@
 SUM_LIMBS = 6
 ABI_VERSION = 12
 (OPT_FUSED_STAGES, OPT_FLOW, OPT_FLOW_WD, OPT_BND_INLINE, OPT_LDSX, OPT_ALTERNATE, OPT_COMPACT_IDX, OPT_VISC_FUSION, OPT_WALL_FAST,
- OPT_FLOW_POLL, OPT_FLOW_CAPACITY, OPT_FLOW_TIMEOUT_MS, OPT_P2P_TIMEOUT_MS, OPT_P2P_ZONE, OPT_ROCTX) = range(15)
-OPT_COUNT = 15
+ OPT_FLOW_POLL, OPT_FLOW_CAPACITY, OPT_FLOW_TIMEOUT_MS, OPT_P2P_TIMEOUT_MS, OPT_P2P_ZONE, OPT_ROCTX, OPT_TRIPLE_LANES) = range(16)
+OPT_COUNT = 16
 SNAPSHOT_SLOTS = 2
 MAX_FARMS, MAX_THRUST_TABLE = 8, 16
 PROBE_UV, PROBE_ELEV = -1, -2
@@ -39,6 +39,7 @@
     'THETIS_AMD_P2P_TIMEOUT_S': (OPT_P2P_TIMEOUT_MS, lambda v: max(1, int(round(1e3*float(v))))),
     'THETIS_AMD_P2P_ZONE': (OPT_P2P_ZONE, lambda v: {'uncached': 1, 'finegrained': 2, 'device': 3}[v]),
     'THETIS_AMD_ROCTX': (OPT_ROCTX, int),
+    'THETIS_AMD_TRIPLE_LANES': (OPT_TRIPLE_LANES, int),
 }
 
 
diff --git a/thetis_amd/csrc/swe2d_api.hip b/thetis_amd/csrc/swe2d_api.hip
--- a/thetis_amd/csrc/swe2d_api.hip
+++ b/thetis_amd/csrc/swe2d_api.hip
@@ -267,6 +267,10 @@
     if (!h) return SWE2D_ERR_INVALID_ARGUMENT;
     if (option < 0 || option >= SWE2D_OPT_COUNT) return fail(h, SWE2D_ERR_INVALID_ARGUMENT, "swe2d_set_option: unknown option");
     if (value < -1) return fail(h, SWE2D_ERR_INVALID_ARGUMENT, "swe2d_set_option: value must be >= -1 (-1: the library's own rule)");
+    if (option == SWE2D_OPT_TRIPLE_LANES) {
+        if (value != -1 && value != 256 && value != 384) return fail(h, SWE2D_ERR_INVALID_ARGUMENT, "swe2d_set_option: SWE2D_OPT_TRIPLE_LANES is 256 or 384");
+        if (int rc = fuse123_drop_tables(h)) return rc;
+    }
     h->opt[option] = value;
     if (option == SWE2D_OPT_FUSED_STAGES && h->fuse_state == -1) h->fuse_state = 0;
     if (option == SWE2D_OPT_FLOW_CAPACITY) h->flow_capacity = -1;
diff --git a/thetis_amd/csrc/swe2d_api_fuse.hip b/thetis_amd/csrc/swe2d_api_fuse.hip
--- a/thetis_amd/csrc/swe2d_api_fuse.hip
+++ b/thetis_amd/csrc/swe2d_api_fuse.hip
@@ -259,13 +259,30 @@
 
 namespace {
 typedef void (*fuse3_kernel_t)(const SweFuse3Args);
-template <bool SRC>
+template <bool SRC, int WG>
 fuse3_kernel_t pick_fuse3_src(bool nl, bool lf)
 {
-    if (nl) return lf ? swe_fuse123_kernel<true, true, SRC> : swe_fuse123_kernel<true, false, SRC>;
-    return lf ? swe_fuse123_kernel<false, true, SRC> : swe_fuse123_kernel<false, false, SRC>;
-}
-fuse3_kernel_t pick_fuse3_kernel(bool nl, bool lf, bool src) { return src ? pick_fuse3_src<true>(nl, lf) : pick_fuse3_src<false>(nl, lf); }
+    if (nl) return lf ? swe_fuse123_kernel<true, true, SRC, WG> : swe_fuse123_kernel<true, false, SRC, WG>;
+    return lf ? swe_fuse123_kernel<false, true, SRC, WG> : swe_fuse123_kernel<false, false, SRC, WG>;
+}
+fuse3_kernel_t pick_fuse3_kernel(bool nl, bool lf, bool src, int lanes)
+{
+    if (lanes == 384) return src ? pick_fuse3_src<true, 384>(nl, lf) : pick_fuse3_src<false, 384>(nl, lf);
+    return src ? pick_fuse3_src<true, 256>(nl, lf) : pick_fuse3_src<false, 256>(nl, lf);
+}
+int fuse3_lanes_wanted(const Handle *h) { return h->opt[SWE2D_OPT_TRIPLE_LANES] == 384 ? 384 : 256; }
+}
+
+int fuse123_drop_tables(Handle *h)
+{
+    if (!h->fuse3_tile && !h->fuse3_cnt) return SWE2D_OK;
+    if (stream_capturing(h)) return fail(h, SWE2D_ERR_UNSUPPORTED, "fused stages: the tile tables cannot be dropped inside a stream capture");
+    HIP_TRY(h, hipSetDevice(h->device));
+    HIP_TRY(h, hipStreamSynchronize(h->stream));
+    if (h->fuse3_tile) { (void)hipFree(h->fuse3_tile); h->fuse3_tile = nullptr; }
+    if (h->fuse3_cnt) { (void)hipFree(h->fuse3_cnt); h->fuse3_cnt = nullptr; }
+    h->fuse3_n_tiles = 0;
+    return SWE2D_OK;
 }
 
 int fuse123_build(Handle *h)
@@ -274,6 +291,8 @@
     const int n = h->n_cells;
     const size_t S = h->stride;
     const int *nbr = h->h_nbr.data();
+    const int lanes = fuse3_lanes_wanted(h);
+    const int max_out = lanes - 32;
     const int *order = (int)h->fuse3_order.size() == n ? h->fuse3_order.data() : ((int)h->fuse_order.size() == n ? h->fuse_order.data() : nullptr);
     const unsigned char *start = (int)h->fuse3_start.size() == n ? h->fuse3_start.data() : nullptr;
     std::vector<int2> tl, cnt;
@@ -308,7 +327,7 @@
                     }
                 }
             }
-            if (count[1] + count[2] + count[3] > SWE_FUSE_WG || 2*count[3] > SWE_FUSE3_MAX_OUT) {
+            if (count[1] + count[2] + count[3] > lanes || 2*count[3] > max_out) {
                 if (inner.empty()) return fail(h, SWE2D_ERR_UNSUPPORTED, "fused stages: a cell whose two rings do not fit a tile");
                 for (size_t i = undo.size(); i-- > 0;) { count[state[undo[i].first]]--; state[undo[i].first] = undo[i].second; count[undo[i].second]++; }
                 touched.resize(touched_before);
@@ -321,10 +340,10 @@
         for (int want = 2; want <= 3; want++)
             for (int c : touched) if (state[c] == want) cells.push_back(c);
         const int ni = (int)inner.size(), nm = ni + count[2], nt = (int)cells.size();
-        if (nt != count[1] + count[2] + count[3] || ni != count[1] || nt > SWE_FUSE_WG) return fail(h, SWE2D_ERR_UNSUPPORTED, "fused stages: tile bookkeeping");
+        if (nt != count[1] + count[2] + count[3] || ni != count[1] || nt > lanes) return fail(h, SWE2D_ERR_UNSUPPORTED, "fused stages: tile bookkeeping");
         for (int l = 0; l < nt; l++) lane_of[cells[l]] = l;
         const size_t base = tl.size();
-        tl.resize(base + SWE_FUSE_WG, int2{-1, 0});
+        tl.resize(base + lanes, int2{-1, 0});
         int n_out = 0;
         for (int l = 0; l < nt; l++) {
             const int c = cells[l];
@@ -335,7 +354,7 @@
                 if (code < 0) field = (unsigned)l;
                 else if (state[code >> 2] != 0) field = (unsigned)lane_of[code >> 2];
                 else {
-                    if (l < nm || n_out >= SWE_FUSE3_MAX_OUT) return fail(h, SWE2D_ERR_UNSUPPORTED, "fused stages: ring bookkeeping");
+                    if (l < nm || n_out >= max_out) return fail(h, SWE2D_ERR_UNSUPPORTED, "fused stages: ring bookkeeping");
                     field = 0x200u | (unsigned)n_out++;
                 }
                 w |= field << (SWE_FUSE_FBITS*f);
@@ -347,6 +366,7 @@
         for (int c : cells) { state[c] = 0; lane_of[c] = -1; }
     }
     h->fuse3_n_tiles = (int)cnt.size();
+    h->fuse3_lanes = lanes;
     HIP_TRY(h, hipMalloc(&h->fuse3_tile, tl.size()*sizeof(int2)));
     HIP_TRY(h, hipMalloc(&h->fuse3_cnt, cnt.size()*sizeof(int2)));
     HIP_TRY(h, hipMemcpy(h->fuse3_tile, tl.data(), tl.size()*sizeof(int2), hipMemcpyHostToDevice));
@@ -369,10 +389,10 @@
     q.cell_end = cell_end;
     for (int s = 0; s < 3; s++) { q.a0[s] = s ? kAlpha0[s] : 0.0; q.a1[s] = s ? kAlphaIn[s] : 1.0; q.beta[s] = kBeta[s]; }
     q.out = h->state[1];
-    fuse3_kernel_t kern = pick_fuse3_kernel(h->par.use_nonlinear_equations != 0, h->par.use_lax_friedrichs_velocity != 0, has_sources(h));
+    fuse3_kernel_t kern = pick_fuse3_kernel(h->par.use_nonlinear_equations != 0, h->par.use_lax_friedrichs_velocity != 0, has_sources(h), h->fuse3_lanes);
     const int grid = ((h->fuse3_n_tiles + 7)/8)*8;
     SWE_CHK_SYNC(h->stream);
-    hipLaunchKernelGGL(kern, dim3(grid), dim3(SWE_FUSE_WG), 0, h->stream, q);
+    hipLaunchKernelGGL(kern, dim3(grid), dim3(h->fuse3_lanes), 0, h->stream, q);
     HIP_TRY(h, hipGetLastError());
     std::swap(h->state[0], h->state[1]);
     h->stage_valid[0] = h->stage_valid[1] = false;
diff --git a/thetis_amd/csrc/swe2d_flow.h b/thetis_amd/csrc/swe2d_flow.h
--- a/thetis_amd/csrc/swe2d_flow.h
+++ b/thetis_amd/csrc/swe2d_flow.h
@@ -178,11 +178,13 @@
     }
 }
 
-template <bool NONLIN, bool LF, bool SRC, int NTR, bool WD = false, int XG = SWE_FLOW_XG, int PLANE = SWE_BLOCK, int NLDS = SWE_FLOW_LDS_DOUBLES>
+template <bool NONLIN, bool LF, bool SRC, int NTR, bool WD = false, int XG = SWE_FLOW_XG, int PLANE = SWE_BLOCK, int NLDS = SWE_FLOW_LDS_DOUBLES,
+          int GEO = 0, int GEO_N = 0>
 __device__ __forceinline__ void swe_flow_rhs_facets(const SweStageArgs &p, int k, const double u[3], const double v[3], const double e[3],
                                                     const double h[3], const double *lds, const unsigned tr[3][NTR], int bmarkers,
                                                     const double nx[3], const double ny[3], double twoA, double bu[3], double bv[3],
-                                                    double be[3], const double *Dn = nullptr, const double *al = nullptr)
+                                                    double be[3], const double *Dn = nullptr, const double *al = nullptr,
+                                                    double *geo = nullptr, unsigned geo_at = 0u)
 {
 #pragma clang fp contract(off)
     const double g = p.g;
@@ -199,7 +201,16 @@
         const double enb = lds[SWE_LDSI(ab2, NLDS)], ena = lds[SWE_LDSI(aa2, NLDS)];
         const double nxs = nx[f], nys = ny[f];
         double Lf, rLf;
-        swe_sqrt_rsqrt(swe_dot2(nxs, nxs, nys, nys), Lf, rLf);
+        if constexpr (GEO == 2) {
+            Lf = geo[SWE_LDSI(geo_at + (unsigned)(2*f*PLANE), GEO_N)];
+            rLf = geo[SWE_LDSI(geo_at + (unsigned)((2*f + 1)*PLANE), GEO_N)];
+        } else {
+            swe_sqrt_rsqrt(swe_dot2(nxs, nxs, nys, nys), Lf, rLf);
+            if constexpr (GEO == 1) {
+                geo[SWE_LDSI(geo_at + (unsigned)(2*f*PLANE), GEO_N)] = Lf;
+                geo[SWE_LDSI(geo_at + (unsigned)((2*f + 1)*PLANE), GEO_N)] = rLf;
+            }
+        }
         double Fau, Fbu, Fav, Fbv, Fae, Fbe;
         if constexpr (WD) {
             const double ena_ = swe_wd_eta(ena, h[a], al[a]), enb_ = swe_wd_eta(enb, h[b], al[b]);
@@ -225,7 +236,7 @@
     }
 }
 
-template <bool NONLIN, bool LF, bool WALLFAST, bool WD = false>
+template <bool NONLIN, bool LF, bool WALLFAST, bool WD = false, bool RCP = false>
 __device__ __forceinline__ void swe_flow_finish(const SweStageArgs &p, int k, double beta, const double u[3], const double v[3],
                                                 const double e[3], const double h[3], const double nx[3], const double ny[3],
                                                 double twoA, int bmarkers, int bkind1, const double bu[3], const double bv[3], const double be[3],
@@ -233,7 +244,7 @@
                                                 double ov[3], double oe[3], const double *Dn = nullptr, const double *al = nullptr)
 {
 #pragma clang fp contract(off)
-    const double s = 6.0*p.dt*beta*swe_rcp(twoA);
+    const double s = 6.0*p.dt*beta*(RCP ? twoA : swe_rcp(twoA));
     const double su = bu[0] + bu[1] + bu[2], sv = bv[0] + bv[1] + bv[2], se = be[0] + be[1] + be[2];
 #pragma unroll
     for (int i = 0; i < 3; i++) {
diff --git a/thetis_amd/csrc/swe2d_fuse.h b/thetis_amd/csrc/swe2d_fuse.h
--- a/thetis_amd/csrc/swe2d_fuse.h
+++ b/thetis_amd/csrc/swe2d_fuse.h
@@ -160,11 +160,9 @@
     }
 }
 
-#define SWE_FUSE3_XG (18*SWE_FUSE_WG)
-#ifndef SWE_FUSE3_MAX_OUT
-#define SWE_FUSE3_MAX_OUT 224
-#endif
-#define SWE_FUSE3_LDS (SWE_FUSE3_XG + 6*SWE_FUSE3_MAX_OUT)
+#define SWE_FUSE3_WG_MAX 384
+constexpr int swe_fuse3_xg(int wg) { return 18*wg; }
+constexpr int swe_fuse3_lds(int wg) { return 24*wg; }
 #ifndef SWE_FUSE3_SRC_MIN_WG
 #define SWE_FUSE3_SRC_MIN_WG 2
 #endif
@@ -179,22 +177,25 @@
     double *out;
 };
 
-template <bool NONLIN, bool LF, bool SRC = false>
-__global__ __launch_bounds__(SWE_FUSE_WG, SRC ? SWE_FUSE3_SRC_MIN_WG : SWE_FUSE_MIN_WG) void swe_fuse123_kernel(const SweFuse3Args q)
+template <bool NONLIN, bool LF, bool SRC = false, int WG = SWE_FUSE_WG>
+__global__ __launch_bounds__(WG, SRC ? SWE_FUSE3_SRC_MIN_WG : SWE_FUSE_MIN_WG) void swe_fuse123_kernel(const SweFuse3Args q)
 {
 #pragma clang fp contract(off)
-    __shared__ double lds[SWE_FUSE3_LDS];
+    static_assert(WG % 64 == 0 && WG <= 512 && WG <= SWE_FUSE3_WG_MAX && swe_fuse3_lds(WG) <= 65536, "lanes of a two-ring tile");
+    constexpr int XG3 = swe_fuse3_xg(WG), LDS3 = swe_fuse3_lds(WG);
+    __shared__ double lds[LDS3];
     const SweStageArgs &p = q.st;
     const int tile = swe_logical_block(blockIdx.x, gridDim.x);
     if (tile >= q.n_tiles) return;
     const int lane = (int)threadIdx.x;
-    const int2 tl = q.tile[(size_t)tile*SWE_FUSE_WG + lane];
+    const int2 tl = q.tile[(size_t)tile*WG + lane];
     const bool real = tl.x >= 0;
     const int k = real ? tl.x : 0;
     const int2 cnt = q.counts[tile];
     const size_t S = p.stride;
     const unsigned S8 = (unsigned)S*8u, k8 = (unsigned)k*8u;
-    double *const P1 = lds + 9*SWE_FUSE_WG;
+    double *const P1 = lds + 9*WG;
+    constexpr bool RCP = !SRC;
 
     int bmarkers = 0, bkind1 = 0;
     unsigned tr[3][1];
@@ -224,8 +225,8 @@
             const unsigned at = w & 0x1ffu;
             const int f2 = nbf >= 0 ? (nbf & 3) : f, f2a = f2 == 2 ? 0 : f2 + 1;
             {
-                const unsigned ab = outside[f] ? (unsigned)(SWE_FUSE3_XG + 6*at) : (unsigned)(f2*SWE_FUSE_WG + at);
-                const unsigned aa = outside[f] ? (unsigned)(SWE_FUSE3_XG + 6*at + 3) : (unsigned)(f2a*SWE_FUSE_WG + at);
+                const unsigned ab = outside[f] ? (unsigned)(XG3 + 6*at) : (unsigned)(f2*WG + at);
+                const unsigned aa = outside[f] ? (unsigned)(XG3 + 6*at + 3) : (unsigned)(f2a*WG + at);
                 tr[f][0] = ab | (aa << 16);
             }
             const int code = outside[f] ? nbf : ((k << 2) | f);
@@ -252,32 +253,43 @@
             ny[f] = px[f] - px[b];
         }
 #pragma unroll
-        for (int i = 0; i < 3; i++) { lds[i*SWE_FUSE_WG + lane] = u[i]; lds[(3 + i)*SWE_FUSE_WG + lane] = v[i]; lds[(6 + i)*SWE_FUSE_WG + lane] = e[i]; }
+        for (int i = 0; i < 3; i++) { lds[i*WG + lane] = u[i]; lds[(3 + i)*WG + lane] = v[i]; lds[(6 + i)*WG + lane] = e[i]; }
 #pragma unroll
         for (int f = 0; f < 3; f++) {
             if (outside[f]) {
                 const unsigned at = ((unsigned)tl.y >> (SWE_FUSE_FBITS*f)) & 0x1ffu;
 #pragma unroll
-                for (int j = 0; j < 6; j++) lds[SWE_LDSI(SWE_FUSE3_XG + 6*at + j, SWE_FUSE3_LDS)] = r0[f][j];
+                for (int j = 0; j < 6; j++) lds[SWE_LDSI(XG3 + 6*at + j, LDS3)] = r0[f][j];
             }
         }
     }
     __syncthreads();
     double twoA = 0.0;
+    double geo[6] = {0.0, 0.0, 0.0, 0.0, 0.0, 0.0};
     if (real) {
         twoA = fma(nx[0], ny[1], -(ny[0]*nx[1]));
         double bu[3], bv[3], be[3], wu[3], wv[3], we[3], ou[3], ov[3], oe[3];
         swe_flow_rhs_cell<NONLIN>(p, u, v, e, h, nx, ny, bu, bv, be);
-        swe_flow_rhs_facets<NONLIN, LF, SRC, 1, false, SWE_FUSE3_XG, SWE_FUSE_WG, SWE_FUSE3_LDS>(p, k, u, v, e, h, lds, tr, bmarkers, nx, ny, twoA, bu, bv, be);
+        swe_flow_rhs_facets<NONLIN, LF, SRC, 1, false, XG3, WG, LDS3, 1, 9*WG>(
+            p, k, u, v, e, h, lds, tr, bmarkers, nx, ny, twoA, bu, bv, be, nullptr, nullptr, P1, (unsigned)lane);
 #pragma unroll
         for (int i = 0; i < 3; i++) { wu[i] = 1.0*u[i]; wv[i] = 1.0*v[i]; we[i] = 1.0*e[i]; }
-        swe_flow_finish<NONLIN, LF, true>(p, k, q.beta[0], u, v, e, h, nx, ny, twoA, bmarkers, bkind1, bu, bv, be, wu, wv, we, ou, ov, oe);
+        if (RCP) twoA = swe_rcp(twoA);
+        swe_flow_finish<NONLIN, LF, true, false, RCP>(p, k, q.beta[0], u, v, e, h, nx, ny, twoA, bmarkers, bkind1, bu, bv, be, wu, wv, we, ou, ov, oe);
 #pragma unroll
         for (int i = 0; i < 3; i++) { u[i] = ou[i]; v[i] = ov[i]; e[i] = oe[i]; }
-#pragma unroll
-        for (int i = 0; i < 3; i++) { P1[i*SWE_FUSE_WG + lane] = u[i]; P1[(3 + i)*SWE_FUSE_WG + lane] = v[i]; P1[(6 + i)*SWE_FUSE_WG + lane] = e[i]; }
-    }
-    __syncthreads();
+        if (lane < cnt.y) {
+#pragma unroll
+            for (int j = 0; j < 6; j++) geo[j] = P1[SWE_LDSI(j*WG + lane, 9*WG)];
+        }
+#pragma unroll
+        for (int i = 0; i < 3; i++) { P1[i*WG + lane] = u[i]; P1[(3 + i)*WG + lane] = v[i]; P1[(6 + i)*WG + lane] = e[i]; }
+    }
+    __syncthreads();
+    if (lane < cnt.y) {
+#pragma unroll
+        for (int j = 0; j < 6; j++) lds[SWE_LDSI(XG3 + j*WG + lane, LDS3)] = geo[j];
+    }
 #pragma unroll 1
     for (int s = 1; s < 3; s++) {
         const bool act = lane < (s == 1 ? cnt.y : cnt.x) && (s == 1 || k < q.cell_end);
@@ -290,21 +302,22 @@
             asm volatile("" : "+v"(bmarkers), "+v"(twoA));
             double bu[3], bv[3], be[3], wu[3], wv[3], we[3];
             swe_flow_rhs_cell<NONLIN>(p, u, v, e, h, nx, ny, bu, bv, be);
-            swe_flow_rhs_facets<NONLIN, LF, SRC, 1, false, SWE_FUSE3_XG, SWE_FUSE_WG, 9*SWE_FUSE_WG>(p, k, u, v, e, h, P1, tr, bmarkers, nx, ny, twoA, bu, bv, be);
+            swe_flow_rhs_facets<NONLIN, LF, SRC, 1, false, XG3, WG, 9*WG, 2, LDS3>(
+                p, k, u, v, e, h, P1, tr, bmarkers, nx, ny, twoA, bu, bv, be, nullptr, nullptr, lds, (unsigned)(XG3 + lane));
             const double a0 = q.a0[s], a1 = q.a1[s];
 #pragma unroll
             for (int i = 0; i < 3; i++) {
-                wu[i] = fma(a0, lds[i*SWE_FUSE_WG + lane], a1*u[i]);
-                wv[i] = fma(a0, lds[(3 + i)*SWE_FUSE_WG + lane], a1*v[i]);
-                we[i] = fma(a0, lds[(6 + i)*SWE_FUSE_WG + lane], a1*e[i]);
-            }
-            swe_flow_finish<NONLIN, LF, true>(p, k, q.beta[s], u, v, e, h, nx, ny, twoA, bmarkers, bkind1, bu, bv, be, wu, wv, we, ou, ov, oe);
+                wu[i] = fma(a0, lds[i*WG + lane], a1*u[i]);
+                wv[i] = fma(a0, lds[(3 + i)*WG + lane], a1*v[i]);
+                we[i] = fma(a0, lds[(6 + i)*WG + lane], a1*e[i]);
+            }
+            swe_flow_finish<NONLIN, LF, true, false, RCP>(p, k, q.beta[s], u, v, e, h, nx, ny, twoA, bmarkers, bkind1, bu, bv, be, wu, wv, we, ou, ov, oe);
         }
         if (s == 1) {
             __syncthreads();
             if (act) {
 #pragma unroll
-                for (int i = 0; i < 3; i++) { P1[i*SWE_FUSE_WG + lane] = ou[i]; P1[(3 + i)*SWE_FUSE_WG + lane] = ov[i]; P1[(6 + i)*SWE_FUSE_WG + lane] = oe[i]; }
+                for (int i = 0; i < 3; i++) { P1[i*WG + lane] = ou[i]; P1[(3 + i)*WG + lane] = ov[i]; P1[(6 + i)*WG + lane] = oe[i]; }
 #pragma unroll
                 for (int i = 0; i < 3; i++) { u[i] = ou[i]; v[i] = ov[i]; e[i] = oe[i]; }
             }
diff --git a/thetis_amd/csrc/swe2d_handle.h b/thetis_amd/csrc/swe2d_handle.h
--- a/thetis_amd/csrc/swe2d_handle.h
+++ b/thetis_amd/csrc/swe2d_handle.h
@@ -130,6 +130,7 @@
     long long fuseq_ring_cells = 0;
     int2 *fuse3_tile = nullptr, *fuse3_cnt = nullptr;
     int fuse3_n_tiles = 0;
+    int fuse3_lanes = 0;
     long long fuse3_ring1 = 0, fuse3_ring2 = 0;
     std::vector<int> fuse_order;
     std::vector<int> fuse3_order;
@@ -316,6 +317,7 @@
 int launch_fuse12(Handle *h, int cell_end);
 bool fuse123_wanted(const Handle *h);
 int fuse123_build(Handle *h);
+int fuse123_drop_tables(Handle *h);
 int launch_fuse123(Handle *h, int cell_end);
 int capture_parity_check(Handle *h);
 bool stream_capturing(Handle *h, unsigned long long *id = nullptr);
diff --git a/thetis_amd/device.py b/thetis_amd/device.py
--- a/thetis_amd/device.py
+++ b/thetis_amd/device.py
@@ -129,7 +129,7 @@
         if (self.npc == 3 and isinstance(reorder, str) and self.n_owned == self.n_cells and 64 < self.n_cells <= 196608
                 and os.environ.get('THETIS_AMD_FLOW_BLOCKS', '1') != '0'):
             self.flow_set_order(ordering.flow_block_order(mesh))
-        tt = ordering.triple_tile_shape() if self.npc == 3 else None
+        tt = ordering.triple_tile_shape(self.triple_patch_default()) if self.npc == 3 else None
         if (self.npc == 3 and isinstance(reorder, str) and self.n_owned == self.n_cells and getattr(mesh, 'structured', False)
                 and self.n_cells > 131072 and tt is not None):
             self.fused_set_triple_tiles(*ordering.triple_tile_order(mesh, *tt))
@@ -388,6 +388,9 @@
         order = np.ascontiguousarray(order, dtype=np.int32)
         self._ck(self.lib.swe2d_fused_set_order(self.h, _iptr(order)))
 
+    def triple_patch_default(self):
+        return (16, 8) if self.get_option(_lib.OPT_TRIPLE_LANES) == 384 else (11, 8)
+
     def fused_set_triple_tiles(self, cells_in_tile_order, tile_starts=None):
         if cells_in_tile_order is None:
             self._ck(self.lib.swe2d_fused_set_triple_tiles(self.h, None, None, 0))
diff --git a/thetis_amd/distributed.py b/thetis_amd/distributed.py
--- a/thetis_amd/distributed.py
+++ b/thetis_amd/distributed.py
@@ -253,7 +253,7 @@
             if order is not None:
                 self.dev.fused_set_order(order)
             self.dev.fused_pair_info()
-            tt = ordering.triple_tile_shape()
+            tt = ordering.triple_tile_shape(self.dev.triple_patch_default() if hasattr(self.dev, 'triple_patch_default') else (11, 8))
             tiles = ordering.triple_tile_order(p, *tt) if tt is not None else None
             if tiles is not None:
                 self.dev.fused_set_triple_tiles(*tiles)
```

Result: faster. 31.84 billion (median of 6 runs) (+2.5%).
